# scenarios/VAE-2

Hardware: AMD Instinct MI355X
Metric: training frames/sec on 128x256 8-frame Cityscapes clips, 1/2/4/8 MI355X (higher is better)
Workload: dtype fp32; 1 GPU; VAE2 ELBO step (encz + encoder + 2 decoders fwd/bwd + Adam), HRNet-W18-small-v2, 128x256, 8 clips/GPU x 9 frames (CLIP_LENGTH=3); yaml=vae-2_amd/experiments/vae2_w18_small_v2_128x256.yaml, global_batch=8, frames_per_clip=9, parallelism=dp1, sync_bn=False, launch=hip_graph, mfma_operands=fp32

## Files before the change

### include/vae2_hip.h

```cpp
#ifndef VAE2_HIP_H
#define VAE2_HIP_H

#include <stdint.h>

#ifdef __cplusplus
extern "C" {
#endif

typedef struct vae2_act {
  int64_t n, h, w, c;
  int64_t ps;
} vae2_act;

#define VAE2_ABI_VERSION 15

int vae2_abi_version(void);
const char* vae2_last_error(void);

int vae2_kernel_log(int enable);
int64_t vae2_kernel_log_read(char* buf, int64_t len);


int64_t vae2_conv2d_fwd_stats_rows(const float* x, const vae2_act* xd, const vae2_act* yd,
                                   int k, int stride, int pad);

int vae2_conv2d_set_algo(int algo);
int vae2_conv2d_set_mfma_bf16(int on);
int vae2_conv2d_set_tune(int key, int value);
int vae2_wgrad_defer(int on);
int vae2_wgrad_flush(void* stream);
int vae2_wgrad_flush_stream(void* stream);

typedef struct vae2_conv_job {
  int32_t kind, k, stride, pad;
  const float* x;
  vae2_act xd;
  const float* wp;
  const float* bias;
  float* y;
  vae2_act yd;
  float beta;
  float* stats;
} vae2_conv_job;
int vae2_conv2d_multi(int n, const vae2_conv_job* jobs, void* stream);
int vae2_conv2d_set_grouping(int on);

int64_t vae2_conv2d_packed_size(int64_t cout, int64_t cin, int k, int mode);
int vae2_conv2d_pack_weight(const float* w, int64_t cout, int64_t cin, int k,
                            int mode, float* out, void* stream);
int vae2_conv2d_pack_weight_ld(const float* w, int64_t cout, int64_t cin, int k,
                               int mode, int64_t ld, float* out, void* stream);

typedef struct vae2_pack_job {
  const float* w;
  float* out;
  int32_t cout, cin, k, mode;
  int32_t ld;
  int32_t pad_;
} vae2_pack_job;
int vae2_conv2d_pack_weights(const vae2_pack_job* jobs, int64_t njobs, void* stream);

int vae2_conv2d_fwd(const float* x, const vae2_act* xd, const float* wp,
                    const float* bias, float* y, const vae2_act* yd, int k,
                    int stride, int pad, float beta, float* stats,
                    void* stream);

int vae2_conv2d_bnin_ok(const float* x, const vae2_act* xd, const vae2_act* yd, int k,
                        int stride, int pad);
int vae2_conv2d_fwd_bnin(const float* x, const vae2_act* xd, const float* bn_save, int relu,
                         const float* wp, const float* bias, float* y, const vae2_act* yd,
                         int k, int stride, int pad, float beta, float* stats, void* stream);
int vae2_conv2d_bwd_weight_bnin(const float* x, const vae2_act* xd, const float* bn_save,
                                int relu, const float* dy, const vae2_act* dyd, float* dw,
                                float* dbias, int k, int stride, int pad, int accumulate,
                                float* ws, int64_t ws_size, void* stream);
int64_t vae2_conv2d_bwd_data_bnpart_rows(const float* dy, const vae2_act* dyd,
                                         const vae2_act* dxd, int k, int stride, int pad);
int vae2_conv2d_bwd_data_bnpart(const float* dy, const vae2_act* dyd, const float* wp,
                                float* dx, const vae2_act* dxd, int k, int stride, int pad,
                                const float* bn_x, const vae2_act* bn_xd, const float* bn_save,
                                int relu, float* partials, void* stream);

int vae2_conv2d_fwd_kernel_name(const vae2_act* xd, const vae2_act* yd, int k, int stride,
                                int pad, char* buf, int64_t len);

int vae2_conv2d_bwd_data(const float* dy, const vae2_act* dyd, const float* wp,
                         float* dx, const vae2_act* dxd, int k, int stride,
                         int pad, float beta, void* stream);

int64_t vae2_conv2d_bwd_weight_ws_size(const vae2_act* xd, const vae2_act* dyd,
                                       int k);

int vae2_conv2d_bwd_weight(const float* x, const vae2_act* xd, const float* dy,
                           const vae2_act* dyd, float* dw, float* dbias, int k,
                           int stride, int pad, int accumulate, float* ws,
                           int64_t ws_size, void* stream);

int vae2_conv2d_bwd_weight_ld(const float* x, const vae2_act* xd, const float* dy,
                              const vae2_act* dyd, float* dw, int64_t dw_ld, float* dbias,
                              int k, int stride, int pad, int accumulate, float* ws,
                              int64_t ws_size, void* stream);


int64_t vae2_bn_partial_rows(const vae2_act* xd);

int vae2_bn_stats(const float* x, const vae2_act* xd, float* partials,
                  void* stream);

int vae2_bn_partials_reduce(const float* partials, int64_t rows, int64_t c,
                            double* sums, int accumulate, void* stream);

int vae2_bn_finalize(const double* sums, double count, const float* gamma,
                     const float* beta, float* running_mean, float* running_var,
                     int64_t* num_batches_tracked, float momentum, float eps,
                     int64_t c, float* save, void* stream);

int vae2_bn_reduce_finalize(const float* partials, int64_t rows, int64_t c,
                            double* sums, double count, const float* gamma,
                            const float* beta, float* running_mean, float* running_var,
                            int64_t* num_batches_tracked, float momentum, float eps,
                            float* save, void* stream);

int vae2_bn_reduce_finalize_shifted(const float* partials, int64_t rows, int64_t c,
                                    double* sums, double count, const float* mean_shift,
                                    const float* gamma, const float* beta,
                                    float* running_mean, float* running_var,
                                    int64_t* num_batches_tracked, float momentum, float eps,
                                    float* save, void* stream);
int vae2_bn_finalize_shifted(const double* sums, double count, const float* mean_shift,
                             const float* gamma, const float* beta, float* running_mean,
                             float* running_var, int64_t* num_batches_tracked, float momentum,
                             float eps, int64_t c, float* save, void* stream);

int vae2_bn_bwd_reduce_param_grads(const float* partials, int64_t rows, int64_t c,
                                   double* sums, float* dgamma, float* dbeta,
                                   void* stream);

int vae2_bn_eval_coeffs(const float* gamma, const float* beta,
                        const float* running_mean, const float* running_var,
                        float eps, int64_t c, float* save, void* stream);

int vae2_bn_apply(const float* x, const vae2_act* xd, const float* save,
                  const float* res, const vae2_act* rd, float* y,
                  const vae2_act* yd, int relu, void* stream);

int vae2_bn_relu_bwd_reduce(const float* dy, const vae2_act* dyd,
                            const float* y, const vae2_act* yd, const float* x,
                            const vae2_act* xd, const float* save, int relu,
                            float* partials, void* stream);

int vae2_bn_bwd_param_grads(const double* sums, int64_t c, float* dgamma,
                            float* dbeta, void* stream);

int vae2_bn_relu_bwd_apply(const float* dy, const vae2_act* dyd, const float* y,
                           const vae2_act* yd, const float* x,
                           const vae2_act* xd, const float* save,
                           const float* gamma, const double* sums, double count,
                           int relu, float* dx, const vae2_act* dxd,
                           float* dres, const vae2_act* dresd, void* stream);

typedef struct vae2_bn_layer {
  const float* x; vae2_act xd;
  const float* a; vae2_act ad;
  float* o; vae2_act od;
  const float* dy; vae2_act dyd;
  float* dres; vae2_act dresd;
  const float* save;
  const float* gamma;
  float* partials;
  const double* sums;
  const double* countp;
  double count;
  int relu;
  int dres_acc;
  const float* rx; vae2_act rxd;
  const float* rsave;
  const float* rgamma;
  float* rpartials;
  const double* rsums;
  float* rdx; vae2_act rdxd;
  unsigned char* mask;
} vae2_bn_layer;
int vae2_bn_multi_apply(int n, const vae2_bn_layer* layers, void* stream);
int vae2_bn_multi_bwd_reduce(int n, const vae2_bn_layer* layers, void* stream);
int vae2_bn_multi_bwd_apply(int n, const vae2_bn_layer* layers, void* stream);

typedef struct vae2_bn_fin {
  const float* partials; int64_t rows; int64_t c;
  double* sums;
  const double* countp;
  double count;
  const float* gamma; const float* beta;
  float* running_mean; float* running_var; int64_t* num_batches_tracked;
  float momentum, eps;
  float* save;
  float* dgamma; float* dbeta;
} vae2_bn_fin;
int vae2_bn_multi_reduce(int n, const vae2_bn_fin* fins, int mode, void* stream);
int vae2_bn_multi_finalize(int n, const vae2_bn_fin* fins, void* stream);

int64_t vae2_conv1x1_upsum_stats_rows(const vae2_act* yd);
int vae2_conv1x1_upsum_fwd(const float* x, const vae2_act* xd, const float* wp,
                           const float* bias, int nup, const float* const* ups,
                           const vae2_act* upds, float* y, const vae2_act* yd, float* stats,
                           void* stream);

int vae2_head_out_fwd(const float* y, const vae2_act* yd, const float* save, const float* w2,
                      const float* b2, int cout2, float* out, const vae2_act* outd,
                      void* stream);
int64_t vae2_head_out_bwd_ws_size(const vae2_act* yd, int cout2);
int vae2_head_out_bwd_reduce(const float* y, const vae2_act* yd, const float* save,
                             const float* w2, int cout2, const float* dout,
                             const vae2_act* doutd, double* sums, float* dgamma, float* dbeta,
                             float* dw2, float* db2, float* ws, int64_t ws_size, void* stream);
int vae2_head_out_bwd_apply(const float* y, const vae2_act* yd, const float* save,
                            const float* gamma, const float* w2, int cout2, const float* dout,
                            const vae2_act* doutd, const double* sums, double count, float* dy,
                            const vae2_act* dyd, float* dbias, float* ws, int64_t ws_size,
                            void* stream);


int vae2_upsample_bilinear_fwd(const float* x, const vae2_act* xd, float* y,
                               const vae2_act* yd, float beta, void* stream);
int vae2_upsample_bilinear_bwd(const float* dy, const vae2_act* dyd, float* dx,
                               const vae2_act* dxd, float beta, void* stream);

int vae2_fuse_sum_relu(int n, const float* const* xs, const vae2_act* xds,
                       float* y, const vae2_act* yd, void* stream);
int vae2_fuse_sum_relu_bn(int n, const float* const* xs, const vae2_act* xds,
                          const float* const* saves, float* y, const vae2_act* yd,
                          void* stream);

int vae2_heads_set_algo(int algo);

int64_t vae2_upsample_bilinear_bwd_multi_ws_size(const vae2_act* dyd, int n,
                                                 const vae2_act* dxds);
int vae2_upsample_bilinear_bwd_multi(const float* dy, const vae2_act* dyd, int n,
                                     float* const* dxs, const vae2_act* dxds, float* ws,
                                     int64_t ws_size, void* stream);

int64_t vae2_upsample_bilinear_bwd_pow2_ws_size(const vae2_act* dyd, int n,
                                                const vae2_act* dxds);
int vae2_upsample_bilinear_bwd_pow2(const float* dy, const vae2_act* dyd, int n,
                                    float* const* dxs, const vae2_act* dxds,
                                    const float* betas, float* ws, int64_t ws_size,
                                    void* stream);

int vae2_relu_bwd(const float* dy, const vae2_act* dyd, const float* y,
                  const vae2_act* yd, float* g, const vae2_act* gd,
                  void* stream);

int vae2_relu_bwd_dual(const float* dy, const vae2_act* dyd, const float* y,
                       const vae2_act* yd, float* g, const vae2_act* gd, float* g2,
                       const vae2_act* g2d, float beta2, void* stream);

int vae2_copy_act(const float* x, const vae2_act* xd, float* y,
                  const vae2_act* yd, float beta, void* stream);

int vae2_codemap_tile_fwd(const float* v, int64_t vs, float* y,
                          const vae2_act* yd, void* stream);
int64_t vae2_spatial_ws_size(const vae2_act* xd);
int vae2_codemap_tile_bwd(const float* dy, const vae2_act* dyd, float* dv,
                          int64_t vs, int accumulate, float* ws, int64_t ws_size,
                          void* stream);

int vae2_nchw_to_nhwc(const float* x, float* y, const vae2_act* yd,
                      float beta, void* stream);
int vae2_nhwc_to_nchw(const float* x, const vae2_act* xd, float* y,
                      float beta, void* stream);

int vae2_global_avgpool_fwd(const float* x, const vae2_act* xd, float* y,
                            const vae2_act* yd, float* ws, int64_t ws_size,
                            void* stream);
int vae2_global_avgpool_bwd(const float* dy, const vae2_act* dyd, float* dx,
                            const vae2_act* dxd, float beta, void* stream);
int vae2_weighted_avgpool_fwd(const float* x, const vae2_act* xd, const float* wr,
                              const float* wc, float scale, float* y, const vae2_act* yd,
                              float* ws, int64_t ws_size, void* stream);
int vae2_weighted_avgpool_bwd(const float* dy, const vae2_act* dyd, const float* wr,
                              const float* wc, float scale, float* dx, const vae2_act* dxd,
                              float beta, void* stream);


int64_t vae2_reduce_ws_size(int64_t n);
int vae2_l1_fwd(const float* p, const vae2_act* pd, const float* t,
                const vae2_act* td, float scale, float* ws, float* out,
                void* stream);
int vae2_l1_bwd(const float* p, const vae2_act* pd, const float* t,
                const vae2_act* td, const float* gout, float scale, float* dp,
                const vae2_act* dpd, float beta, void* stream);

int vae2_lsgan_fwd(const float* x, const vae2_act* xd, float target, float scale, float* ws,
                   float* out, void* stream);
int vae2_lsgan_bwd(const float* x, const vae2_act* xd, float target, const float* gout,
                   float scale, float* dx, const vae2_act* dxd, float beta, void* stream);

int64_t vae2_ssim_loss_ws_size(const vae2_act* pd);
int vae2_ssim_loss_fwd(const float* p, const vae2_act* pd, const float* t, const vae2_act* td,
                       const float* a, const float* b, float c1, float c2, float scale,
                       double* ws, float* out, void* stream);
int vae2_ssim_loss_bwd(const float* p, const vae2_act* pd, const float* t, const vae2_act* td,
                       const float* a, const float* b, float c1, float c2, const float* gout,
                       float scale, float* dp, const vae2_act* dpd, float beta, void* stream);

int vae2_reparam_kl_fwd(const float* muvar, const vae2_act* md,
                        const float* eps, const vae2_act* ed, float* z,
                        const vae2_act* zd, int prior, float scale,
                        float* kl_out, int accumulate, float* ws, void* stream);
int vae2_reparam_kl_bwd(const float* muvar, const vae2_act* md,
                        const float* eps, const vae2_act* ed, const float* dz,
                        const vae2_act* dzd, const float* gkl, float scale,
                        float* dmuvar, const vae2_act* dmd, void* stream);

int vae2_weighted_sum(int n, const float* const* terms, const float* lambdas,
                      float* total, void* stream);

int vae2_nonfinite_check(const float* x, int64_t n, int32_t* flag,
                         void* stream);


int vae2_clip_normalize_u8(const uint8_t* frames, int64_t n, int64_t nframes, int64_t h,
                           int64_t w, const float* lut, int nseg, float* const* outs,
                           void* stream);


int vae2_to_image(const float* x, float* y, int64_t n, int64_t c, int64_t h, int64_t w,
                  const double* mean3, const double* std3, void* stream);
int64_t vae2_metrics_ws_size(int64_t planes, int64_t h, int64_t w);
int vae2_absdiff_sqdiff_sum(const float* a, const float* b, int64_t n, double* ws,
                            double* out, void* stream);
int vae2_ssim(const float* x, const float* y, int64_t planes, int64_t h, int64_t w,
              const float* win, int win_size, float c1, float c2, double* ws, double* out,
              void* stream);
int vae2_avgpool2x2(const float* x, float* y, int64_t planes, int64_t h, int64_t w,
                    void* stream);


int vae2_adam_step(float* p, const float* g, float* m, float* v, int64_t n,
                   float lr, float beta1, float beta2, float eps,
                   float weight_decay, int64_t step, void* stream);

int vae2_adam_coeffs(double* state, float beta1, float beta2, float* coeffs,
                     void* stream);
int vae2_adam_step_dev(float* p, const float* g, float* m, float* v, int64_t n,
                       const float* coeffs, float beta1, float beta2, float eps,
                       float weight_decay, void* stream);

int vae2_sgd_step(float* p, const float* g, float* buf, int64_t n, float lr, float momentum,
                  float dampening, float weight_decay, int nesterov, int first_step,
                  void* stream);

int vae2_sgd_coeffs(double* state, float momentum, float dampening, int nesterov,
                    float* coeffs, void* stream);
int vae2_sgd_step_dev(float* p, const float* g, float* buf, int64_t n, const float* coeffs,
                      float momentum, float weight_decay, int nesterov, void* stream);

int64_t vae2_grad_norm_ws_size(int64_t n);
int vae2_grad_sumsq(const float* g, int64_t n, double* partials, void* stream);
int vae2_clip_coeffs(const double* partials, int64_t count, float max_norm, float* clip,
                     void* stream);
int vae2_sgd_step_dev_clip(float* p, const float* g, float* buf, int64_t n, const float* coeffs,
                           const float* clip, float momentum, float weight_decay, int nesterov,
                           void* stream);
int vae2_adam_step_dev_clip(float* p, const float* g, float* m, float* v, int64_t n,
                            const float* coeffs, const float* clip, float beta1, float beta2,
                            float eps, float weight_decay, void* stream);
int vae2_scale_dev(float* x, int64_t n, const float* clip, void* stream);

int vae2_ema_coeffs(double* state, float decay, float* coeffs, void* stream);
int vae2_ema_update_dev(float* ema, const float* p, int64_t n, const float* coeffs,
                        void* stream);
int vae2_ema_update(float* ema, const float* p, int64_t n, float decay, int first,
                    void* stream);

int vae2_scale(float* dst, const float* src, int64_t n, float scale,
               void* stream);


typedef struct vae2_syncbn_comm vae2_syncbn_comm;
int64_t vae2_syncbn_comm_bytes(int world, int64_t max_elems);
int vae2_syncbn_comm_init(int rank, int world, int64_t max_elems, void* handle_out,
                          vae2_syncbn_comm** out);
int vae2_syncbn_comm_connect(vae2_syncbn_comm* comm, const void* handles);
int vae2_syncbn_allreduce(vae2_syncbn_comm* comm, double* buf, int64_t n, void* stream);
int vae2_syncbn_comm_error(vae2_syncbn_comm* comm, int64_t* host_out);
int vae2_syncbn_comm_set_timeout(vae2_syncbn_comm* comm, double seconds);
int vae2_syncbn_comm_destroy(vae2_syncbn_comm* comm);

#ifdef __cplusplus
}
#endif

#endif
```

### vae-2_amd/csrc/conv.h

```cpp
#pragma once

#include "common.h"

namespace vae2 {

static inline int round_up(int a, int b) { return (a + b - 1) / b * b; }

struct IGemm {
  const float* a;
  int a_ps, a_c, a_c4, a_h, a_w;
  int g_n, g_h, g_w;
  int a_step;
  int nth, ntw;
  int dh0, dhs, dw0, dws;
  int kh0, khs, kw0, kws, ksz;
  const float* w;
  uint32_t a_bytes, w_bytes;
  int n;
  const float* bias;
  float* y;
  int y_ps, y_h, y_w, y_step, y_offh, y_offw;
  float beta;
  float* stats;
  int vec_out;
  FastDiv hw_div, w_div;
  int ktab;
  const float* bx;
  int bx_ps, brelu;
  const float* bsave;
  uint32_t bx_bytes;
  struct Cls {
    int g_h, g_w, nth, ntw, dh0, dw0, kh0, kw0, y_offh, y_offw;
    FastDiv hw_div, w_div;
  } cls[4];
};

struct Tile {
  int tm, tn, nblk;
  int ks = 1;
  int nr = 0;
};

struct IGemmPlan {
  Tile t;
  int64_t M;
  int max_taps;
  dim3 grid;
};
IGemmPlan igemm_plan(const IGemm& p, int ncls);

extern int g_wide_tiles, g_ksplit, g_bf16, g_conv_algo, g_dconv_nr, g_gemm1, g_vec_out,
    g_dconv_nr_wide, g_igemm_minblk, g_wgrad_cols, g_dconv_nw8, g_wgrad_nw8, g_gemm1_tn,
    g_gemm1_tm, g_igemm_nr, g_wgrad_narrow, g_igemm_tab, g_dconv_n16, g_dconv_split72,
    g_dconv_ksp, g_wgrad_wgs;
extern int g_dconv_stream, g_dconv_stream_wpc, g_dconv_stream_bl, g_dconv_stream_spb;
extern int g_wgrad_narrow_tps;
extern int g_bn_v2, g_bn_blocks, g_bn_apply_res;
extern int g_fuse_quad;

inline uint32_t packed_bytes(int64_t cout, int64_t cin, int k, int mode) {
  return (uint32_t)(vae2_conv2d_packed_size(cout, cin, k, mode) * 4);
}

inline bool vec_ok(const float* a, int ps) {
  return ((uintptr_t)a % 16 == 0) && (ps % 4 == 0);
}

inline bool conv_shapes_ok(const vae2_act* xd, const vae2_act* yd, int k, int stride, int pad) {
  if (!act_ok(xd) || !act_ok(yd)) return false;
  if (xd->n != yd->n) return false;
  if (k < 1 || stride < 1 || pad < 0) return false;
  int64_t oh = (xd->h + 2 * pad - k) / stride + 1;
  int64_t ow = (xd->w + 2 * pad - k) / stride + 1;
  return oh == yd->h && ow == yd->w;
}

inline bool fits32(const vae2_act* d) {
  return d->n * d->h * d->w * d->ps < (int64_t(1) << 29);
}

inline uint32_t act_bytes(const vae2_act* d) {
  int64_t tail = (d->ps % 4 == 0) ? ((d->c + 3) / 4 * 4) : d->c;
  int64_t last = ((d->n * d->h * d->w) - 1) * d->ps + tail;
  return (uint32_t)(last * 4);
}

struct G1Tile {
  int tm = 2, tn, nblk, grid_x;
  size_t lds;
};
int launch_igemm(IGemm& p, int role, hipStream_t s, const char* fn, int ncls = 1);
int launch_gemm1(const float* a, const vae2_act* ad, const float* wp, uint32_t w_bytes,
                 const float* bias, float* y, const vae2_act* yd, float beta, float* stats,
                 const G1Tile& t, hipStream_t s, const char* fn, const float* bx = nullptr,
                 int bx_ps = 0, int brelu = 0, const float* bsave = nullptr,
                 uint32_t bx_bytes = 0);

struct DTile {
  int tm, tn, nblk, cs4, tiles_h, tiles_w;
  int nr = 0;
  int nw = 4;
  int ks = 1;
};

struct BnSide {
  const float* isave = nullptr;
  int irelu = 0;
  const float* bx = nullptr;
  int bx_ps = 0, brelu = 0;
  const float* bsave = nullptr;
  uint32_t bx_bytes = 0;
};

int launch_dconv(const float* a, const vae2_act* ad, const float* wp, uint32_t w_bytes,
                 const float* bias, float* y, const vae2_act* yd, float beta,
                 float* stats, bool flip, hipStream_t s, const char* fn,
                 const BnSide& bn = BnSide{});

Tile pick_tile(int64_t M, int N, bool wide = false);
bool gemm1_pick(const vae2_act* ad, const vae2_act* yd, int k, int stride, int pad,
                const float* a, G1Tile* out);
DTile pick_dtile(const vae2_act* ad, const vae2_act* yd, bool remainder = true);
bool stream_use(const vae2_act* ad, const vae2_act* yd);
bool dconv_use(const vae2_act* ad, const vae2_act* yd, int k, int stride, int pad,
               const float* a);
int64_t dconv_rows(const vae2_act* ad, const vae2_act* yd);
bool wgrad3_shape_ok(const vae2_act* xd, const vae2_act* dyd, int k, int stride, int pad);

}
```

### vae-2_amd/csrc/conv_wgrad.hip

```cpp
#include <algorithm>
#include <mutex>
#include <vector>

#include "conv.h"

namespace vae2 {

struct WGrad {
  const float* x;
  int x_ps, cin, cin4, x_h, x_w;
  const float* dy;
  int dy_ps, cout, o_n, o_h, o_w;
  int k, stride, pad;
  int P, px_split;
  uint32_t x_bytes, dy_bytes;
  float* part;
  FastDiv ohw_div, ow_div, cin4_div;
};

template <int TM, int TN, bool BF = false, bool V4 = false>
__global__ __launch_bounds__(256, 2) void wgrad_kernel(WGrad p) {
  extern __shared__ __attribute__((aligned(16))) float wred[];
  const int lane = threadIdx.x & 63, wave = threadIdx.x >> 6;
  const int g = lane >> 4, r = lane & 15;
  const int ncol4 = p.k * p.k * p.cin4;
  const int co0 = blockIdx.y * 16 * TM;
  const int col0 = blockIdx.x * 16 * TN;
  const int pbeg = blockIdx.z * p.px_split;
  const int pend = min(pbeg + p.px_split, p.P);
  const __amdgpu_buffer_rsrc_t xr = make_rsrc(p.x, p.x_bytes);
  const __amdgpu_buffer_rsrc_t dr = make_rsrc(p.dy, p.dy_bytes);

  int aco[TM];
#pragma unroll
  for (int i = 0; i < TM; ++i) {
    const int co = co0 + i * 16 + r;
    aco[i] = co < p.cout ? co : -1;
  }
  int bkh[TN], bkw[TN], boff[TN];
  bool bok[TN];
  const int kq = r & 3;
#pragma unroll
  for (int j = 0; j < TN; ++j) {
    const int col = col0 + j * 16 + (V4 ? 4 * (r >> 2) : r);
    const int t = (int)p.cin4_div.div((uint32_t)col);
    const int ci = col - t * p.cin4;
    bkh[j] = t / p.k;
    bkw[j] = t - bkh[j] * p.k;
    bok[j] = col < ncol4 && ci < p.cin;
    boff[j] = (bkh[j] * p.x_w + bkw[j]) * p.x_ps + ci;
  }
  f4 acc[TM][TN];
#pragma unroll
  for (int i = 0; i < TM; ++i)
#pragma unroll
    for (int j = 0; j < TN; ++j) acc[i][j] = f4{0.f, 0.f, 0.f, 0.f};

  const int ohw = p.o_h * p.o_w;
  auto load = [&](int pc, f4* fa, f4* fb) {
    if constexpr (V4) {
      const int pix = pc + 4 * g + kq;
      const bool pv = pix < pend;
      const int pp = pv ? pix : pbeg;
      const int n = (int)p.ohw_div.div((uint32_t)pp);
      const int rem = pp - n * ohw;
      const int oh = (int)p.ow_div.div((uint32_t)rem);
      const int ow = rem - oh * p.o_w;
      const uint32_t drow = (uint32_t)(pp * p.dy_ps);
#pragma unroll
      for (int i = 0; i < TM; ++i) {
        const int co = co0 + i * 16 + 4 * (r >> 2);
        fa[i] = load4(dr, (pv && co < p.cout) ? (drow + co) * 4u : kOOB);
      }
      const int ih0 = oh * p.stride - p.pad, iw0 = ow * p.stride - p.pad;
      const int xc = ((n * p.x_h + ih0) * p.x_w + iw0) * p.x_ps;
#pragma unroll
      for (int j = 0; j < TN; ++j) {
        const int ih = ih0 + bkh[j], iw = iw0 + bkw[j];
        const bool ok = pv && bok[j] && (unsigned)ih < (unsigned)p.x_h &&
                        (unsigned)iw < (unsigned)p.x_w;
        fb[j] = load4(xr, ok ? (uint32_t)(xc + boff[j]) * 4u : kOOB);
      }
      return;
    }
#pragma unroll
    for (int s = 0; s < 4; ++s) {
      const int pix = pc + 4 * g + s;
      const bool pv = pix < pend;
      const int pp = pv ? pix : pbeg;
      const int n = (int)p.ohw_div.div((uint32_t)pp);
      const int rem = pp - n * ohw;
      const int oh = (int)p.ow_div.div((uint32_t)rem);
      const int ow = rem - oh * p.o_w;
      const uint32_t drow = (uint32_t)(pp * p.dy_ps);
#pragma unroll
      for (int i = 0; i < TM; ++i)
        fa[i][s] = load1(dr, (pv && aco[i] >= 0) ? (drow + aco[i]) * 4u : kOOB);
      const int ih0 = oh * p.stride - p.pad, iw0 = ow * p.stride - p.pad;
      const int xc = ((n * p.x_h + ih0) * p.x_w + iw0) * p.x_ps;
#pragma unroll
      for (int j = 0; j < TN; ++j) {
        const int ih = ih0 + bkh[j], iw = iw0 + bkw[j];
        const bool ok = pv && bok[j] && (unsigned)ih < (unsigned)p.x_h &&
                        (unsigned)iw < (unsigned)p.x_w;
        fb[j][s] = load1(xr, ok ? (uint32_t)(xc + boff[j]) * 4u : kOOB);
      }
    }
  };
  auto quads = [&](f4* fa, f4* fb) {
    if constexpr (V4) {
#pragma unroll
      for (int i = 0; i < TM; ++i) quad_transpose(fa[i], kq);
#pragma unroll
      for (int j = 0; j < TN; ++j) quad_transpose(fb[j], kq);
    }
  };
  auto mma = [&](f4* fa, f4* fb) {
    quads(fa, fb);
#pragma unroll
    for (int s = 0; s < 4; ++s)
#pragma unroll
      for (int i = 0; i < TM; ++i)
#pragma unroll
        for (int j = 0; j < TN; ++j)
          acc[i][j] = __builtin_amdgcn_mfma_f32_16x16x4f32(fa[i][s], fb[j][s], acc[i][j], 0, 0, 0);
  };
  {
    f4 fa0[TM], fb0[TN], fa1[TM], fb1[TN];
    int pc = pbeg + 16 * wave;
    if (!BF) {
      if (pc < pend) load(pc, fa0, fb0);
      for (; pc < pend; pc += 128) {
        load(pc + 64, fa1, fb1);
        mma(fa0, fb0);
        load(pc + 128, fa0, fb0);
        mma(fa1, fb1);
      }
    } else if (pc < pend) {
      load(pc, fa0, fb0);
      load(pc + 64, fa1, fb1);
      for (; pc < pend; pc += 128) {
        bf16x8 A[TM], B[TN];
        quads(fa0, fb0);
        quads(fa1, fb1);
#pragma unroll
        for (int i = 0; i < TM; ++i) A[i] = pack_bf16(fa0[i], fa1[i]);
#pragma unroll
        for (int j = 0; j < TN; ++j) B[j] = pack_bf16(fb0[j], fb1[j]);
        load(pc + 128, fa0, fb0);
        load(pc + 192, fa1, fb1);
#pragma unroll
        for (int i = 0; i < TM; ++i)
#pragma unroll
          for (int j = 0; j < TN; ++j)
            acc[i][j] = __builtin_amdgcn_mfma_f32_16x16x32_bf16(A[i], B[j], acc[i][j], 0, 0, 0);
      }
    }
  }

  constexpr int NV = TM * TN * 4;
  if (wave > 0) {
#pragma unroll
    for (int i = 0; i < TM; ++i)
#pragma unroll
      for (int j = 0; j < TN; ++j)
#pragma unroll
        for (int e = 0; e < 4; ++e)
          wred[((wave - 1) * NV + (i * TN + j) * 4 + e) * 64 + lane] = acc[i][j][e];
  }
  __syncthreads();
  if (wave != 0) return;
#pragma unroll
  for (int w = 0; w < 3; ++w)
#pragma unroll
    for (int i = 0; i < TM; ++i)
#pragma unroll
      for (int j = 0; j < TN; ++j)
#pragma unroll
        for (int e = 0; e < 4; ++e)
          acc[i][j][e] += wred[(w * NV + (i * TN + j) * 4 + e) * 64 + lane];

  float* out = p.part + (int64_t)blockIdx.z * p.cout * ncol4;
#pragma unroll
  for (int i = 0; i < TM; ++i)
#pragma unroll
    for (int e = 0; e < 4; ++e) {
      const int co = co0 + i * 16 + g * 4 + e;
      if (co >= p.cout) continue;
#pragma unroll
      for (int j = 0; j < TN; ++j) {
        const int col = col0 + j * 16 + r;
        if (col < ncol4) out[(int64_t)co * ncol4 + col] = acc[i][j][e];
      }
    }
}

struct WGrad3 {
  const float* x;
  int x_ps, cin, cin4, h, w;
  const float* dy;
  int dy_ps, cout;
  int tiles_h, tiles_w, ntiles, tiles_per_split;
  int csw, n_ci_slabs;
  uint32_t x_bytes, dy_bytes;
  float* part;
  const float* isave;
  int irelu;
};

template <int TM, int TN, int BH, bool PF, int KS, bool BF = false, int NR = 0, int NW = 4>
__global__ __launch_bounds__(64 * NW) void wgrad3_kernel(WGrad3 p) {
  constexpr int NT = 64 * NW;
  constexpr int HALO = KS / 2, TAPS = KS * KS;
  constexpr int LH = BH + KS - 1, LW = 32 + KS - 1, NPX = BH * 32, LPX = LH * LW;
  constexpr int QMAX = KS == 1 ? 16 : 9;
  constexpr int DYS = NPX + 4;
  constexpr int NRQ = (NR + 3) / 4;
  constexpr int NQ = 4 * TM + NRQ;
  static_assert(NR == 0 || (!BF && NR <= 4), "remainder shape");
  extern __shared__ __attribute__((aligned(16))) float sm[];
  float* dyt = sm;
  float* xt = sm + NQ * 4 * DYS;
  const int lane = threadIdx.x & 63, wave = threadIdx.x >> 6;
  const int g = lane >> 4, r = lane & 15;
  const int cis = blockIdx.y % p.n_ci_slabs, cos = blockIdx.y / p.n_ci_slabs;
  const int co0 = cos * (16 * TM + NR), c0 = cis * p.csw;
  const int csw_real = p.cin4 - c0 < p.csw ? p.cin4 - c0 : p.csw;
  const __amdgpu_buffer_rsrc_t xr = make_rsrc(p.x, p.x_bytes);
  const __amdgpu_buffer_rsrc_t dr = make_rsrc(p.dy, p.dy_bytes);

  int bbase[TN];
#pragma unroll
  for (int j = 0; j < TN; ++j) {
    const int n = (wave * TN + j) * 16 + r;
    const int t = n / p.csw;
    const int cl = n - t * p.csw;
    const bool ok = t < TAPS && cl < csw_real;
    bbase[j] = ok ? cl * LPX + (t / KS) * LW + (t % KS) : p.csw * LPX;
  }
  for (int i = threadIdx.x; i < LPX; i += NT) xt[p.csw * LPX + i] = 0.f;
  __shared__ float ibn[2][QMAX * 4];
  if (p.isave && threadIdx.x < QMAX * 4) {
    const int ch = c0 + (int)threadIdx.x < p.cin ? c0 + (int)threadIdx.x : p.cin - 1;
    ibn[0][threadIdx.x] = p.isave[2 * p.cin + ch];
    ibn[1][threadIdx.x] = p.isave[3 * p.cin + ch];
  }
  auto ibn_apply = [&](f4& v, int q) {
#pragma unroll
    for (int k = 0; k < 4; ++k) {
      const float t = __builtin_fmaf(v[k], ibn[0][4 * q + k], ibn[1][4 * q + k]);
      v[k] = (p.irelu && t < 0.f) ? 0.f : t;
    }
  };

  f4 acc[TM][TN];
#pragma unroll
  for (int i = 0; i < TM; ++i)
#pragma unroll
    for (int j = 0; j < TN; ++j) acc[i][j] = f4{0.f, 0.f, 0.f, 0.f};
  float racc[TN][NR > 0 ? NR : 1];
#pragma unroll
  for (int j = 0; j < TN; ++j)
#pragma unroll
    for (int q = 0; q < NR; ++q) racc[j][q] = 0.f;

  const int per_img = p.tiles_h * p.tiles_w;
  const int tb = blockIdx.x * p.tiles_per_split;
  const int te = tb + p.tiles_per_split < p.ntiles ? tb + p.tiles_per_split : p.ntiles;
  constexpr int NDY = NPX * NQ;
  constexpr int NI = (NDY + NT - 1) / NT;
  constexpr int NX = (LPX * QMAX + NT - 1) / NT;
  const int xtotal = LPX * (csw_real >> 2);
  f4 pdy[NI], pxx[NX];
  static_assert(NX <= 32, "x item mask");
  uint32_t xok = 0;
  auto fetch = [&](int tile) {
    const int img = tile / per_img;
    const int trem = tile - img * per_img;
    const int th = trem / p.tiles_w;
    const int oh0 = th * BH, ow0 = (trem - th * p.tiles_w) * 32;
    const int ibase = img * p.h;
#pragma unroll
    for (int u = 0; u < NI; ++u) {
      const int i = threadIdx.x + u * NT;
      const int q = i / NPX, px = i - q * NPX;
      const int oh = oh0 + px / 32, ow = ow0 + (px & 31);
      const int co = co0 + 4 * q;
      const bool ok = i < NDY && oh < p.h && ow < p.w && co < p.cout;
      pdy[u] = load4(dr, ok ? (uint32_t)(((ibase + oh) * p.w + ow) * p.dy_ps + co) * 4u : kOOB);
    }
#pragma unroll
    for (int u = 0; u < NX; ++u) {
      const int i = threadIdx.x + u * NT;
      const int q = i / LPX, hp = i - q * LPX;
      const int lr = hp / LW, lc = hp - lr * LW;
      const int ih = oh0 - HALO + lr, iw = ow0 - HALO + lc;
      const int c = c0 + 4 * q;
      const bool ok = i < xtotal && (unsigned)ih < (unsigned)p.h && (unsigned)iw < (unsigned)p.w;
      pxx[u] = load4(xr, ok ? (uint32_t)(((ibase + ih) * p.w + iw) * p.x_ps + c) * 4u : kOOB);
      xok = u == 0 ? (uint32_t)ok : (xok | ((uint32_t)ok << u));
    }
  };
  auto store = [&]() {
#pragma unroll
    for (int u = 0; u < NI; ++u) {
      const int i = threadIdx.x + u * NT;
      if (NDY % NT != 0 && i >= NDY) break;
      const int q = i / NPX, px = i - q * NPX;
      const int co = co0 + 4 * q;
#pragma unroll
      for (int k = 0; k < 4; ++k) dyt[(4 * q + k) * DYS + px] = co + k < p.cout ? pdy[u][k] : 0.f;
    }
#pragma unroll
    for (int u = 0; u < NX; ++u) {
      const int i = threadIdx.x + u * NT;
      if (i < xtotal) {
        const int q = i / LPX, hp = i - q * LPX;
        const int c = c0 + 4 * q;
        if (p.isave && ((xok >> u) & 1u)) ibn_apply(pxx[u], q);
#pragma unroll
        for (int k = 0; k < 4; ++k) xt[(4 * q + k) * LPX + hp] = c + k < p.cin ? pxx[u][k] : 0.f;
      }
    }
  };
  if (PF && tb < te) fetch(tb);
  for (int tile = tb; tile < te; ++tile) {
    __syncthreads();
    if (PF) {
      store();
    } else {
      const int img = tile / per_img;
      const int trem = tile - img * per_img;
      const int th = trem / p.tiles_w;
      const int oh0 = th * BH, ow0 = (trem - th * p.tiles_w) * 32;
      const int ibase = img * p.h;
      {
        f4 v[NI];
#pragma unroll
        for (int u = 0; u < NI; ++u) {
          const int i = threadIdx.x + u * NT;
          const int q = i / NPX, px = i - q * NPX;
          const int oh = oh0 + px / 32, ow = ow0 + (px & 31);
          const int co = co0 + 4 * q;
          const bool ok = i < NDY && oh < p.h && ow < p.w && co < p.cout;
          v[u] = load4(dr, ok ? (uint32_t)(((ibase + oh) * p.w + ow) * p.dy_ps + co) * 4u : kOOB);
        }
#pragma unroll
        for (int u = 0; u < NI; ++u) {
          const int i = threadIdx.x + u * NT;
          if (NDY % NT != 0 && i >= NDY) break;
          const int q = i / NPX, px = i - q * NPX;
          const int co = co0 + 4 * q;
#pragma unroll
          for (int k = 0; k < 4; ++k)
            dyt[(4 * q + k) * DYS + px] = co + k < p.cout ? v[u][k] : 0.f;
        }
      }
      for (int i0 = threadIdx.x; i0 < xtotal; i0 += 4 * NT) {
        f4 v[4];
        bool okv[4];
#pragma unroll
        for (int u = 0; u < 4; ++u) {
          const int i = i0 + u * NT;
          const int q = i / LPX, hp = i - q * LPX;
          const int lr = hp / LW, lc = hp - lr * LW;
          const int ih = oh0 - HALO + lr, iw = ow0 - HALO + lc;
          const int c = c0 + 4 * q;
          const bool ok =
              i < xtotal && (unsigned)ih < (unsigned)p.h && (unsigned)iw < (unsigned)p.w;
          okv[u] = ok;
          v[u] = load4(xr, ok ? (uint32_t)(((ibase + ih) * p.w + iw) * p.x_ps + c) * 4u : kOOB);
        }
#pragma unroll
        for (int u = 0; u < 4; ++u) {
          const int i = i0 + u * NT;
          if (i >= xtotal) break;
          const int q = i / LPX, hp = i - q * LPX;
          const int c = c0 + 4 * q;
          if (p.isave && okv[u]) ibn_apply(v[u], q);
#pragma unroll
          for (int k = 0; k < 4; ++k) xt[(4 * q + k) * LPX + hp] = c + k < p.cin ? v[u][k] : 0.f;
        }
      }
    }
    __syncthreads();
    if (PF && tile + 1 < te) fetch(tile + 1);
    auto frag = [&](int ch, f4* fa, f4* fb) {
      const int px0 = ch * 16 + 4 * g;
      const int poff = (px0 >> 5) * LW + (px0 & 31);
#pragma unroll
      for (int i = 0; i < TM; ++i)
        fa[i] = *reinterpret_cast<const f4*>(&dyt[(i * 16 + r) * DYS + px0]);
#pragma unroll
      for (int j = 0; j < TN; ++j) {
        const float* b = &xt[bbase[j] + poff];
        if (KS == 1) fb[j] = *reinterpret_cast<const f4*>(b);
        else fb[j] = f4{b[0], b[1], b[2], b[3]};
      }
    };
    if (!BF) {
#pragma unroll 2
      for (int ch = 0; ch < NPX / 16; ++ch) {
        f4 fa[TM], fb[TN];
        frag(ch, fa, fb);
#pragma unroll
        for (int s2 = 0; s2 < 4; ++s2)
#pragma unroll
          for (int i = 0; i < TM; ++i)
#pragma unroll
            for (int j = 0; j < TN; ++j)
              acc[i][j] = __builtin_amdgcn_mfma_f32_16x16x4f32(fa[i][s2], fb[j][s2], acc[i][j], 0, 0, 0);
        if constexpr (NR > 0) {
          const int px0 = ch * 16 + 4 * g;
#pragma unroll
          for (int q = 0; q < NR; ++q) {
            const f4 d = *reinterpret_cast<const f4*>(&dyt[(16 * TM + q) * DYS + px0]);
#pragma unroll
            for (int j = 0; j < TN; ++j) {
              racc[j][q] = __builtin_fmaf(d[0], fb[j][0], racc[j][q]);
              racc[j][q] = __builtin_fmaf(d[1], fb[j][1], racc[j][q]);
              racc[j][q] = __builtin_fmaf(d[2], fb[j][2], racc[j][q]);
              racc[j][q] = __builtin_fmaf(d[3], fb[j][3], racc[j][q]);
            }
          }
        }
      }
    } else {
#pragma unroll 2
      for (int ch = 0; ch < NPX / 16; ch += 2) {
        f4 fa0[TM], fb0[TN], fa1[TM], fb1[TN];
        frag(ch, fa0, fb0);
        frag(ch + 1, fa1, fb1);
#pragma unroll
        for (int i = 0; i < TM; ++i)
#pragma unroll
          for (int j = 0; j < TN; ++j)
            acc[i][j] = __builtin_amdgcn_mfma_f32_16x16x32_bf16(
                pack_bf16(fa0[i], fa1[i]), pack_bf16(fb0[j], fb1[j]), acc[i][j], 0, 0, 0);
      }
    }
  }

  const int ncol4 = TAPS * p.cin4;
  float* out = p.part + (int64_t)blockIdx.x * p.cout * ncol4;
#pragma unroll
  for (int j = 0; j < TN; ++j) {
    const int n = (wave * TN + j) * 16 + r;
    const int t = n / p.csw;
    const int cl = n - t * p.csw;
    if (t >= TAPS || cl >= csw_real) continue;
    const int col = t * p.cin4 + c0 + cl;
#pragma unroll
    for (int i = 0; i < TM; ++i)
#pragma unroll
      for (int e = 0; e < 4; ++e) {
        const int co = co0 + i * 16 + g * 4 + e;
        if (co < p.cout) out[(int64_t)co * ncol4 + col] = acc[i][j][e];
      }
  }
  if constexpr (NR > 0) {
#pragma unroll
    for (int j = 0; j < TN; ++j) {
      const int n = (wave * TN + j) * 16 + r;
      const int t = n / p.csw;
      const int cl = n - t * p.csw;
#pragma unroll
      for (int q = 0; q < NR; ++q) {
        float v = racc[j][q];
        v += __shfl_xor(v, 16, 64);
        v += __shfl_xor(v, 32, 64);
        if (g == 0 && t < TAPS && cl < csw_real)
          out[(int64_t)(co0 + 16 * TM + q) * ncol4 + t * p.cin4 + c0 + cl] = v;
      }
    }
  }
}

__global__ __launch_bounds__(256) void wgrad_reduce_kernel(const float* __restrict__ part,
                                                           int splits, int cout, int cin,
                                                           int cin4, int k,
                                                           float* __restrict__ dw, int64_t ld,
                                                           int accumulate) {
  __shared__ float red[8][32];
  const int kk = k * k;
  const int ncol4 = kk * cin4;
  const int total = cout * ncol4;
  const int cl = threadIdx.x & 31, sg = threadIdx.x >> 5;
  const int idx = blockIdx.x * 32 + cl;
  float s = 0.f;
  if (idx < total) {
    const float* src = part + idx;
    const int64_t stride = (int64_t)total;
#pragma unroll 8
    for (int sp = sg; sp < splits; sp += 8) s += src[sp * stride];
  }
  red[sg][cl] = s;
  __syncthreads();
  if (sg != 0 || idx >= total) return;
  s = red[0][cl];
#pragma unroll
  for (int j = 1; j < 8; ++j) s += red[j][cl];
  const int co = idx / ncol4;
  const int col = idx - co * ncol4;
  const int t = col / cin4;
  const int ci = col - t * cin4;
  if (ci >= cin) return;
  const int64_t o = (int64_t)co * ld + ci * kk + t;
  dw[o] = accumulate ? dw[o] + s : s;
}

struct WRJob {
  const float* part;
  float* dw;
  int64_t ld;
  int splits, cout, cin, cin4, k, accumulate, blk0;
};
constexpr int kWrMaxJobs = 32;
struct WRMulti {
  WRJob j[kWrMaxJobs];
  int n;
};

__global__ __launch_bounds__(256) void wgrad_reduce_multi_kernel(WRMulti m) {
  int i = 0;
  while (i + 1 < m.n && (int)blockIdx.x >= m.j[i + 1].blk0) ++i;
  const WRJob& J = m.j[i];
  __shared__ float red[8][32];
  const int kk = J.k * J.k;
  const int ncol4 = kk * J.cin4;
  const int total = J.cout * ncol4;
  const int cl = threadIdx.x & 31, sg = threadIdx.x >> 5;
  const int idx = ((int)blockIdx.x - J.blk0) * 32 + cl;
  float s = 0.f;
  if (idx < total) {
    const float* src = J.part + idx;
    const int64_t stride = (int64_t)total;
#pragma unroll 8
    for (int sp = sg; sp < J.splits; sp += 8) s += src[sp * stride];
  }
  red[sg][cl] = s;
  __syncthreads();
  if (sg != 0 || idx >= total) return;
  s = red[0][cl];
#pragma unroll
  for (int q = 1; q < 8; ++q) s += red[q][cl];
  const int co = idx / ncol4;
  const int col = idx - co * ncol4;
  const int t = col / J.cin4;
  const int ci = col - t * J.cin4;
  if (ci >= J.cin) return;
  const int64_t o = (int64_t)co * J.ld + ci * kk + t;
  J.dw[o] = J.accumulate ? J.dw[o] + s : s;
}


struct WRQueued {
  WRJob job;
  hipStream_t stream;
};
static thread_local bool g_wr_defer = false;
static std::vector<WRQueued> g_wr_queue;
static std::mutex g_wr_mu;

struct WTile {
  int tm, tn, gx, gy, splits, px_split;
};

static WTile pick_wtile(int64_t P, int cout, int ncol4) {
  WTile t;
  int mt = (cout + 15) / 16;
  t.tm = mt <= 4 ? mt : 4;
  t.gy = (int)ceil_div(cout, 16 * t.tm);
  int ct = (ncol4 + 15) / 16;
  if (g_wgrad_cols && t.tm == 4 && ct == 4) {
    t.tm = 2;
    t.gy = (int)ceil_div(cout, 32);
  }
  const int tn_max = t.tm == 4 ? 3 : 4;
  t.tn = ct <= tn_max ? ct : tn_max;
  t.gx = (int)ceil_div(ncol4, 16 * t.tn);
  int64_t tiles = (int64_t)t.gx * t.gy;
  int64_t want = ceil_div(g_wgrad_wgs, tiles);
  int64_t maxs = ceil_div(P, 256);
  int64_t s = want < maxs ? want : maxs;
  if (s < 1) s = 1;
  t.px_split = (int)(ceil_div(ceil_div(P, s), 64) * 64);
  t.splits = (int)ceil_div(P, t.px_split);
  return t;
}

template <int TM, bool V4>
static void launch_wgrad_tn_v(const WGrad& p, int tn, dim3 grid, hipStream_t s) {
  const size_t lds = (size_t)3 * TM * 4 * 4 * 64 * sizeof(float) / 4 * tn;
  switch (tn) {
#define CASE(T) \
  case T: \
    if (g_bf16) VAE2_LAUNCH((wgrad_kernel<TM, T, true, V4>), grid, dim3(256), lds, s, p); \
    else VAE2_LAUNCH((wgrad_kernel<TM, T, false, V4>), grid, dim3(256), lds, s, p); \
    break;
    CASE(1) CASE(2) CASE(3)
    default: CASE(4)
#undef CASE
  }
}

template <int TM>
static void launch_wgrad_tn(const WGrad& p, int tn, dim3 grid, hipStream_t s, bool v4) {
  if (v4) launch_wgrad_tn_v<TM, true>(p, tn, grid, s);
  else launch_wgrad_tn_v<TM, false>(p, tn, grid, s);
}


struct W3Tile {
  int ks, tm, tn, bh, csw, n_ci_slabs, n_co_slabs, tiles_h, tiles_w, ntiles, tps, splits;
  bool pf;
  int nr = 0;
  int nw = 4;
};

int wgrad3_blocks_per_cu(const W3Tile& t, size_t lds);
static size_t wgrad3_lds(const W3Tile& t);

bool wgrad3_shape_ok(const vae2_act* xd, const vae2_act* dyd, int k, int stride, int pad) {
  return k == 3 && pad == 1 && stride == 1 && xd->h == dyd->h &&
         xd->w == dyd->w && xd->ps % 4 == 0 && dyd->ps % 4 == 0 && dyd->w >= 16;
}

static W3Tile pick_w3tile(const vae2_act* xd, const vae2_act* dyd, int k) {
  W3Tile t;
  t.ks = k;
  const int cin4 = round_up((int)xd->c, 4);
  const int maxc = k == 1 ? 64 : 36;
  int nsl = (cin4 + maxc - 1) / maxc;
  t.csw = round_up((int)ceil_div(cin4, nsl), 4);
  t.n_ci_slabs = (int)ceil_div(cin4, t.csw);
  const int nt = (k * k * t.csw + 15) / 16;
  t.tn = (nt + 3) / 4;
  const int mt = (int)((dyd->c + 15) / 16);
  t.n_co_slabs = (mt + 3) / 4;
  t.tm = (mt + t.n_co_slabs - 1) / t.n_co_slabs;
  if (k == 3 && g_dconv_nr && !g_bf16 && (dyd->c == 18 || dyd->c == 36 || dyd->c == 72)) {
    t.tm = dyd->c == 18 ? 1 : 2;
    t.nr = dyd->c == 18 ? 2 : 4;
    t.n_co_slabs = (int)(dyd->c / (16 * t.tm + t.nr));
  }
  if (g_wgrad_nw8 && t.nr && !g_bf16) {
    const int tn2 = (nt + 7) / 8;
    if ((t.tm == 1 && tn2 == 2) || (t.tm == 2 && tn2 == 3)) {
      t.tn = tn2;
      t.nw = 8;
    }
  }
  t.bh = (t.tm <= 2 && t.csw <= 24 && k == 3) ? 8 : 4;
  t.tiles_h = (int)ceil_div(dyd->h, t.bh);
  t.tiles_w = (int)ceil_div(dyd->w, 32);
  t.ntiles = (int)(dyd->n * t.tiles_h * t.tiles_w);
  const int gy = t.n_ci_slabs * t.n_co_slabs;
  int64_t want = ceil_div(1024, gy);
  const int64_t slab = (int64_t)dyd->c * k * k * cin4 * 4;
  const int64_t cap = 48ll << 20;
  if (want * slab > cap) want = cap / slab > 0 ? cap / slab : 1;
  if (want > t.ntiles) want = t.ntiles;
  t.tps = (int)ceil_div(t.ntiles, want);
  t.pf = (int64_t)t.ntiles * gy >= 1024;
  if (t.pf) {
    const int64_t resident = 256 * (int64_t)wgrad3_blocks_per_cu(t, wgrad3_lds(t));
    int64_t w2 = resident / gy > 0 ? resident / gy : 1;
    if (w2 * slab > cap) w2 = cap / slab > 0 ? cap / slab : 1;
    t.tps = (int)ceil_div(t.ntiles, w2);
    if (t.tps < 2) t.tps = 2;
  }
  if (t.tps < 2) t.tps = 2;
  t.splits = (int)ceil_div(t.ntiles, t.tps);
  return t;
}

static size_t wgrad3_lds(const W3Tile& t) {
  const int npx = t.bh * 32, lpx = (t.bh + t.ks - 1) * (32 + t.ks - 1);
  const int rows = 16 * t.tm + 4 * ((t.nr + 3) / 4);
  return ((size_t)rows * (npx + 4) + (size_t)(t.csw + 1) * lpx) * sizeof(float);
}

struct W3Probe {
  bool on = false;
  const void* fn = nullptr;
  unsigned threads = 0;
};
static thread_local W3Probe g_w3probe;
#define W3_LAUNCH(K, GRID, BLOCK, SHM, S, ...)                         \
  do {                                                                \
    if (g_w3probe.on) {                                               \
      g_w3probe.fn = reinterpret_cast<const void*>(K);                \
      g_w3probe.threads = dim3(BLOCK).x;                              \
    } else {                                                          \
      VAE2_LAUNCH(K, GRID, BLOCK, SHM, S, __VA_ARGS__);               \
    }                                                                 \
  } while (0)

template <int TM, int BH, bool PF>
static void wgrad3_launch_tn(const WGrad3& p, int tn, int ks, dim3 grid, size_t shm,
                             hipStream_t s, int nr = 0, int nw = 4) {
  if constexpr (TM == 1 || TM == 2) {
    if (nr && nw == 8) {
      constexpr int R = TM == 1 ? 2 : 4, T8 = TM == 1 ? 2 : 3;
      W3_LAUNCH((wgrad3_kernel<TM, T8, BH, PF, 3, false, R, 8>), grid, dim3(512), shm, s, p);
      return;
    }
    if (nr) {
      constexpr int R = TM == 1 ? 2 : 4;
      switch (tn) {
#define CASE(T) \
  case T: W3_LAUNCH((wgrad3_kernel<TM, T, BH, PF, 3, false, R>), grid, dim3(256), shm, s, p); break;
        CASE(1) CASE(2) CASE(3) CASE(4) CASE(5) CASE(6)
#undef CASE
      }
      return;
    }
  }
  if (ks == 1) {
    if (g_bf16) W3_LAUNCH((wgrad3_kernel<TM, 1, BH, PF, 1, true>), grid, dim3(256), shm, s, p);
    else W3_LAUNCH((wgrad3_kernel<TM, 1, BH, PF, 1>), grid, dim3(256), shm, s, p);
    return;
  }
  switch (tn) {
#define CASE(T) \
  case T:                                                                         \
    if (g_bf16) W3_LAUNCH((wgrad3_kernel<TM, T, BH, PF, 3, true>), grid, dim3(256), shm, s, p); \
    else W3_LAUNCH((wgrad3_kernel<TM, T, BH, PF, 3>), grid, dim3(256), shm, s, p);   \
    break;
    CASE(1) CASE(2) CASE(3) CASE(4) CASE(5) CASE(6)
#undef CASE
  }
}

template <int BH, bool PF>
static void wgrad3_launch_tm(const WGrad3& p, const W3Tile& t, dim3 grid, size_t shm,
                             hipStream_t s) {
  switch (t.tm) {
    case 1: wgrad3_launch_tn<1, BH, PF>(p, t.tn, t.ks, grid, shm, s, t.nr, t.nw); break;
    case 2: wgrad3_launch_tn<2, BH, PF>(p, t.tn, t.ks, grid, shm, s, t.nr, t.nw); break;
    case 3: wgrad3_launch_tn<3, BH, PF>(p, t.tn, t.ks, grid, shm, s); break;
    default: wgrad3_launch_tn<4, BH, PF>(p, t.tn, t.ks, grid, shm, s); break;
  }
}

template <int BH>
static void wgrad3_launch(const WGrad3& p, const W3Tile& t, dim3 grid, size_t shm,
                          hipStream_t s) {
  if (t.pf) wgrad3_launch_tm<BH, true>(p, t, grid, shm, s);
  else wgrad3_launch_tm<BH, false>(p, t, grid, shm, s);
}

int wgrad3_blocks_per_cu(const W3Tile& t, size_t lds) {
  struct Key {
    int tm, tn, bh, ks, nr, nw, pf, bf;
    size_t lds;
    int n;
  };
  static Key cache[32];
  static int ncache = 0;
  const int bf = g_bf16;
  for (int i = 0; i < ncache; ++i) {
    const Key& k = cache[i];
    if (k.tm == t.tm && k.tn == t.tn && k.bh == t.bh && k.ks == t.ks && k.nr == t.nr &&
        k.nw == t.nw && k.pf == (int)t.pf && k.bf == bf && k.lds == lds)
      return k.n;
  }
  WGrad3 p{};
  g_w3probe = W3Probe{};
  g_w3probe.on = true;
  if (t.bh == 8) wgrad3_launch<8>(p, t, dim3(1), lds, nullptr);
  else wgrad3_launch<4>(p, t, dim3(1), lds, nullptr);
  g_w3probe.on = false;
  int n = 0;
  if (!g_w3probe.fn || hipOccupancyMaxActiveBlocksPerMultiprocessor(
                           &n, g_w3probe.fn, (int)g_w3probe.threads, lds) != hipSuccess ||
      n < 1) {
    (void)hipGetLastError();
    n = 1;
  }
  if (ncache < 32) cache[ncache++] = Key{t.tm, t.tn, t.bh, t.ks, t.nr, t.nw, (int)t.pf, bf, lds, n};
  return n;
}

}

using namespace vae2;

extern "C" {

int vae2_wgrad_defer(int on) {
  const int prev = g_wr_defer ? 1 : 0;
  g_wr_defer = on != 0;
  return prev;
}

static int wgrad_flush_impl(void* stream, bool own_only) {
  const char* fn = "vae2_wgrad_flush";
  hipStream_t want = as_stream(stream);
  std::vector<WRQueued> q;
  {
    std::lock_guard<std::mutex> lk(g_wr_mu);
    if (own_only) {
      std::vector<WRQueued> keep;
      for (const WRQueued& j : g_wr_queue) (j.stream == want ? q : keep).push_back(j);
      g_wr_queue.swap(keep);
    } else {
      q.swap(g_wr_queue);
    }
  }
  size_t i = 0;
  while (i < q.size()) {
    WRMulti m{};
    hipStream_t st = want;
    int blocks = 0;
    while (i < q.size() && m.n < kWrMaxJobs) {
      WRJob j = q[i].job;
      const float* lo = j.dw;
      const float* hi = j.dw + (int64_t)(j.cout - 1) * j.ld + (int64_t)j.cin * j.k * j.k;
      bool clash = false;
      for (int u = 0; u < m.n; ++u) {
        const float* lo2 = m.j[u].dw;
        const float* hi2 = m.j[u].dw + (int64_t)(m.j[u].cout - 1) * m.j[u].ld +
                           (int64_t)m.j[u].cin * m.j[u].k * m.j[u].k;
        if (lo < hi2 && lo2 < hi) clash = true;
      }
      if (clash) break;
      j.blk0 = blocks;
      blocks += (int)ceil_div((int64_t)j.cout * j.k * j.k * j.cin4, 32);
      m.j[m.n++] = j;
      ++i;
    }
    VAE2_LAUNCH(wgrad_reduce_multi_kernel, dim3((unsigned)blocks), dim3(256), 0, st, m);
    const int rc = check_launch(fn);
    if (rc) return rc;
  }
  return 0;
}

int vae2_wgrad_flush(void* stream) { return wgrad_flush_impl(stream, false); }

int vae2_wgrad_flush_stream(void* stream) { return wgrad_flush_impl(stream, true); }


struct WgradWs {
  int64_t part, total;
};
static WgradWs wgrad_ws(const vae2_act* xd, const vae2_act* dyd, int k) {
  const int ncol4 = k * k * round_up((int)xd->c, 4);
  const WTile t = pick_wtile(act_pixels(dyd), (int)dyd->c, ncol4);
  int64_t splits = t.splits;
  if ((k == 3 || k == 1) && xd->h == dyd->h && xd->w == dyd->w) {
    splits = std::max<int64_t>(splits, pick_w3tile(xd, dyd, k).splits);
    splits = std::max<int64_t>(splits, wgrad3n_splits(xd, dyd));
  }
  const int64_t part = splits * dyd->c * ncol4;
  return WgradWs{part, part + 2 * vae2_bn_partial_rows(dyd) * dyd->c + 4};
}

int64_t vae2_conv2d_bwd_weight_ws_size(const vae2_act* xd, const vae2_act* dyd, int k) {
  if (!act_ok(xd) || !act_ok(dyd)) return 0;
  return wgrad_ws(xd, dyd, k).total;
}

static int bwd_weight_impl(const float* x, const vae2_act* xd, const float* dy,
                           const vae2_act* dyd, float* dw, int64_t dw_ld, float* dbias,
                           int k, int stride, int pad, int accumulate, float* ws,
                           int64_t ws_size, void* stream, const float* isave, int irelu,
                           const char* fn) {
  VAE2_REQUIRE(xd && dw_ld >= xd->c * k * k, fn, "bad dW row stride");
  VAE2_REQUIRE(x && dy && dw && ws, fn, "null pointer");
  VAE2_REQUIRE(conv_shapes_ok(xd, dyd, k, stride, pad), fn, "inconsistent conv shapes");
  VAE2_REQUIRE(fits32(xd) && fits32(dyd), fn, "tensor too large for 32-bit indexing");
  const WgradWs wsl = wgrad_ws(xd, dyd, k);
  VAE2_REQUIRE(ws_size >= wsl.total, fn, "workspace too small");
  hipStream_t s = as_stream(stream);
  const int cin4 = round_up((int)xd->c, 4);
  const int ncol4 = k * k * cin4;
  int splits = 0;
  const bool direct = g_conv_algo != 1 && wgrad3_shape_ok(xd, dyd, k, stride, pad) &&
                      vec_ok(x, (int)xd->ps) && vec_ok(dy, (int)dyd->ps);
  VAE2_REQUIRE(direct || !isave, fn,
               "input BatchNorm needs the direct 3x3 weight-gradient kernel (vae2_conv2d_bnin_ok)");
  if (direct && k == 3) {
    splits = wgrad3n_launch(x, xd, dy, dyd, ws, isave, irelu, act_bytes(xd), act_bytes(dyd), s);
    if (splits < 0) return check_launch(fn);
  }
  if (direct && !splits) {
    W3Tile t3 = pick_w3tile(xd, dyd, k);
    WGrad3 q{};
    q.x = x; q.x_ps = (int)xd->ps; q.cin = (int)xd->c; q.cin4 = cin4;
    q.h = (int)xd->h; q.w = (int)xd->w;
    q.dy = dy; q.dy_ps = (int)dyd->ps; q.cout = (int)dyd->c;
    q.tiles_h = t3.tiles_h; q.tiles_w = t3.tiles_w; q.ntiles = t3.ntiles;
    q.tiles_per_split = t3.tps;
    q.csw = t3.csw; q.n_ci_slabs = t3.n_ci_slabs;
    q.x_bytes = act_bytes(xd); q.dy_bytes = act_bytes(dyd);
    q.part = ws;
    q.isave = isave;
    q.irelu = irelu ? 1 : 0;
    dim3 grid((unsigned)t3.splits, (unsigned)(t3.n_ci_slabs * t3.n_co_slabs));
    const size_t shm = wgrad3_lds(t3);
    if (t3.bh == 8) wgrad3_launch<8>(q, t3, grid, shm, s);
    else wgrad3_launch<4>(q, t3, grid, shm, s);
    int rc = check_launch(fn);
    if (rc) return rc;
    splits = t3.splits;
  }
  WTile t = pick_wtile(act_pixels(dyd), (int)dyd->c, ncol4);
  if (splits) goto reduce;
  {
  WGrad p{};
  p.x = x; p.x_ps = (int)xd->ps; p.cin = (int)xd->c; p.cin4 = cin4;
  p.x_h = (int)xd->h; p.x_w = (int)xd->w;
  p.dy = dy; p.dy_ps = (int)dyd->ps; p.cout = (int)dyd->c;
  p.o_n = (int)dyd->n; p.o_h = (int)dyd->h; p.o_w = (int)dyd->w;
  p.k = k; p.stride = stride; p.pad = pad;
  p.P = (int)act_pixels(dyd);
  p.px_split = t.px_split;
  p.part = ws;
  p.x_bytes = act_bytes(xd);
  p.dy_bytes = act_bytes(dyd);
  p.ohw_div = FastDiv((uint32_t)(dyd->h * dyd->w));
  p.ow_div = FastDiv((uint32_t)dyd->w);
  p.cin4_div = FastDiv((uint32_t)cin4);
  dim3 grid(t.gx, t.gy, (unsigned)t.splits);
  const bool v4 = g_vec_out && vec_ok(x, (int)xd->ps) && vec_ok(dy, (int)dyd->ps);
  switch (t.tm) {
    case 1: launch_wgrad_tn<1>(p, t.tn, grid, s, v4); break;
    case 2: launch_wgrad_tn<2>(p, t.tn, grid, s, v4); break;
    case 3: launch_wgrad_tn<3>(p, t.tn, grid, s, v4); break;
    default: launch_wgrad_tn<4>(p, t.tn, grid, s, v4); break;
  }
  int rc = check_launch(fn);
  if (rc) return rc;
  splits = t.splits;
  }
reduce:
  int64_t slab = dyd->c * (int64_t)ncol4;
  int rc = 0;
  if (g_wr_defer) {
    WRJob j{ws, dw, dw_ld, splits, (int)dyd->c, (int)xd->c, cin4, k, accumulate, 0};
    std::lock_guard<std::mutex> lk(g_wr_mu);
    g_wr_queue.push_back(WRQueued{j, s});
  } else {
    VAE2_LAUNCH(wgrad_reduce_kernel, dim3((unsigned)ceil_div(slab, 32)), dim3(256), 0, s,
                (const float*)ws, splits, (int)dyd->c, (int)xd->c, cin4, k, dw, dw_ld,
                accumulate);
    rc = check_launch(fn);
    if (rc) return rc;
  }
  if (dbias) {
    float* bp = ws + wsl.part;
    rc = vae2_bn_stats(dy, dyd, bp, stream);
    if (rc) return rc;
    rc = bias_grad_from_partials(bp, vae2_bn_partial_rows(dyd), dyd->c, dbias, accumulate,
                                 stream);
    if (rc) return rc;
  }
  return 0;
}

int vae2_conv2d_bwd_weight_ld(const float* x, const vae2_act* xd, const float* dy,
                              const vae2_act* dyd, float* dw, int64_t dw_ld, float* dbias,
                              int k, int stride, int pad, int accumulate, float* ws,
                              int64_t ws_size, void* stream) {
  return bwd_weight_impl(x, xd, dy, dyd, dw, dw_ld, dbias, k, stride, pad, accumulate, ws,
                         ws_size, stream, nullptr, 0, "vae2_conv2d_bwd_weight");
}

int vae2_conv2d_bwd_weight_bnin(const float* x, const vae2_act* xd, const float* bn_save,
                                int relu, const float* dy, const vae2_act* dyd, float* dw,
                                float* dbias, int k, int stride, int pad, int accumulate,
                                float* ws, int64_t ws_size, void* stream) {
  const char* fn = "vae2_conv2d_bwd_weight_bnin";
  if (!xd || !bn_save) return fail(fn, "null pointer");
  return bwd_weight_impl(x, xd, dy, dyd, dw, xd->c * k * k, dbias, k, stride, pad, accumulate,
                         ws, ws_size, stream, bn_save, relu, fn);
}

int vae2_conv2d_bwd_weight(const float* x, const vae2_act* xd, const float* dy,
                           const vae2_act* dyd, float* dw, float* dbias, int k,
                           int stride, int pad, int accumulate, float* ws,
                           int64_t ws_size, void* stream) {
  if (!xd) return fail("vae2_conv2d_bwd_weight", "null descriptor");
  return vae2_conv2d_bwd_weight_ld(x, xd, dy, dyd, dw, xd->c * k * k, dbias, k, stride, pad,
                                   accumulate, ws, ws_size, stream);
}

}
```

### vae-2_amd/csrc/wgrad_narrow.hip

```cpp
#include "conv.h"

namespace vae2 {

int g_wgrad_narrow_tps = 2;

constexpr int kTH = 4;
constexpr int kTW = 32;
constexpr int kLW = kTW + 2;
constexpr int kNPX = kTH * kTW;

struct WGN {
  const float* x;
  int x_ps, cin, cin4, h, w;
  const float* dy;
  int dy_ps, cout;
  int tiles_h, tiles_w, ntiles, tps;
  int n_ci_slabs;
  FastDiv per_img_div, tiles_w_div;
  uint32_t x_bytes, dy_bytes;
  float* part;
  const float* isave;
  int irelu;
};

template <int CQ, int TM, int NR, int WPIX, bool PF, int NW = 4>
__global__ __launch_bounds__(64 * NW) void wgrad3n_kernel(WGN p) {
  constexpr int CSW = 4 * CQ;
  constexpr int CO = 16 * TM + NR;
  constexpr int COQ = (CO + 3) / 4;
  constexpr int DP = 4 * COQ;
  constexpr int XP = CSW;
  constexpr int LPX = (kTH + 2) * kLW;
  constexpr int RS = kLW * XP + ((CSW - kLW * XP) % 16 + 16) % 16;
  constexpr int G = (3 * CSW + 15) / 16;
  constexpr int WCOL = NW / WPIX;
  constexpr int NT = 64 * NW;
  constexpr int GW = (G + WCOL - 1) / WCOL;
  static_assert(NR <= 4 && (NR == 0 || COQ == 4 * TM + 1), "one remainder quad");
  static_assert(WCOL * WPIX == NW && (WCOL == 1 || WCOL == 2 || WCOL == 4), "waves per tile");
  extern __shared__ __attribute__((aligned(16))) float sm[];
  float* xs = sm;
  float* ds = sm + (kTH + 2) * RS;

  const int lane = threadIdx.x & 63, wave = threadIdx.x >> 6;
  const int g = lane >> 4, r = lane & 15;
  const int wc = wave % WCOL, wp = wave / WCOL;
  const int cis = blockIdx.y % p.n_ci_slabs, cos = blockIdx.y / p.n_ci_slabs;
  const int c0 = cis * CSW, co0 = cos * CO;
  const __amdgpu_buffer_rsrc_t xr = make_rsrc(p.x, p.x_bytes);
  const __amdgpu_buffer_rsrc_t dr = make_rsrc(p.dy, p.dy_bytes);

  int xoff[GW];
  bool colok[GW];
#pragma unroll
  for (int j = 0; j < GW; ++j) {
    const int n = (wc * GW + j) * 16 + r;
    const int nc = n < 3 * CSW ? n : 3 * CSW - 1;
    const int dh = nc / CSW, ci = nc - dh * CSW;
    colok[j] = wc * GW + j < G && n < 3 * CSW && c0 + ci < p.cin;
    xoff[j] = dh * RS + ci;
  }
  __shared__ f4 ibn_tab[2][CQ];
  if (p.isave && threadIdx.x < 2 * CSW) {
    const int k = threadIdx.x % CSW, which = threadIdx.x / CSW;
    const int ch = c0 + k < p.cin ? c0 + k : p.cin - 1;
    reinterpret_cast<float*>(&ibn_tab[which][0])[k] = p.isave[(2 + which) * p.cin + ch];
  }
  auto ibn = [&](f4& v, int q) {
    const f4 sc = ibn_tab[0][q], sh = ibn_tab[1][q];
#pragma unroll
    for (int k = 0; k < 4; ++k) {
      const float t = __builtin_fmaf(v[k], sc[k], sh[k]);
      v[k] = (p.irelu && t < 0.f) ? 0.f : t;
    }
  };

  f4 acc[TM][GW][3];
#pragma unroll
  for (int i = 0; i < TM; ++i)
#pragma unroll
    for (int j = 0; j < GW; ++j)
#pragma unroll
      for (int d = 0; d < 3; ++d) acc[i][j][d] = f4{0.f, 0.f, 0.f, 0.f};
  float racc[GW][3][NR > 0 ? NR : 1];
#pragma unroll
  for (int j = 0; j < GW; ++j)
#pragma unroll
    for (int d = 0; d < 3; ++d)
#pragma unroll
      for (int q = 0; q < NR; ++q) racc[j][d][q] = 0.f;

  const int per_img = p.tiles_h * p.tiles_w;
  const int tb = blockIdx.x * p.tps;
  const int te = tb + p.tps < p.ntiles ? tb + p.tps : p.ntiles;
  constexpr int XPU = NT / CQ, DPU = NT / COQ;
  constexpr int NXI = (LPX + XPU - 1) / XPU, NDI = (kNPX + DPU - 1) / DPU;
  const int xq = threadIdx.x % CQ, xb = threadIdx.x / CQ;
  const int dq = threadIdx.x % COQ, db = threadIdx.x / COQ;
  const bool xact = xb < XPU, dact = db < DPU;
  const int xc = c0 + 4 * xq;
  const bool xcok = xc < p.cin4;
  const bool dcok = co0 + 4 * dq < p.cout;
  f4 px[NXI], pd[NDI];
  uint32_t xin = 0;
  auto fetch = [&](int tile) {
    const int img = (int)p.per_img_div.div((uint32_t)tile);
    const int trem = tile - img * per_img;
    const int th = (int)p.tiles_w_div.div((uint32_t)trem);
    const int oh0 = th * kTH, ow0 = (trem - th * p.tiles_w) * kTW;
    const int ibase = img * p.h;
#pragma unroll
    for (int u = 0; u < NXI; ++u) {
      const int hp = xb + u * XPU;
      const int lr = hp / kLW, lc = hp - lr * kLW;
      const int ih = oh0 - 1 + lr, iw = ow0 - 1 + lc;
      const bool ok = xact && hp < LPX && xcok && (unsigned)ih < (unsigned)p.h &&
                      (unsigned)iw < (unsigned)p.w;
      px[u] = load4(xr, ok ? (uint32_t)(((ibase + ih) * p.w + iw) * p.x_ps + xc) * 4u : kOOB);
      xin = u == 0 ? (uint32_t)ok : (xin | ((uint32_t)ok << u));
    }
#pragma unroll
    for (int u = 0; u < NDI; ++u) {
      const int pp = db + u * DPU;
      const int oh = oh0 + pp / kTW, ow = ow0 + (pp & (kTW - 1));
      const bool ok = dact && pp < kNPX && dcok && oh < p.h && ow < p.w;
      pd[u] = load4(dr, ok ? (uint32_t)(((ibase + oh) * p.w + ow) * p.dy_ps + co0 + 4 * dq) * 4u : kOOB);
    }
  };
  auto store = [&]() {
#pragma unroll
    for (int u = 0; u < NXI; ++u) {
      const int hp = xb + u * XPU;
      if (!xact || hp >= LPX) break;
      f4 v = px[u];
      if (p.isave && ((xin >> u) & 1u)) ibn(v, xq);
#pragma unroll
      for (int k = 0; k < 4; ++k) v[k] = xc + k < p.cin ? v[k] : 0.f;
      const int lr = hp / kLW, lc = hp - lr * kLW;
      *reinterpret_cast<f4*>(&xs[lr * RS + lc * XP + 4 * xq]) = v;
    }
#pragma unroll
    for (int u = 0; u < NDI; ++u) {
      const int pp = db + u * DPU;
      if (!dact || pp >= kNPX) break;
      f4 v = pd[u];
#pragma unroll
      for (int k = 0; k < 4; ++k) v[k] = (co0 + 4 * dq + k < p.cout && 4 * dq + k < CO) ? v[k] : 0.f;
      *reinterpret_cast<f4*>(&ds[pp * DP + 4 * dq]) = v;
    }
  };

  if (PF && tb < te) fetch(tb);
  for (int tile = tb; tile < te; ++tile) {
    __syncthreads();
    if (!PF) fetch(tile);
    store();
    __syncthreads();
    if (PF && tile + 1 < te) fetch(tile + 1);
#pragma unroll 1
    for (int ch = wp; ch < kTH * 2; ch += WPIX) {
      const int orow = ch >> 1, cb = (ch & 1) * 16;
      const int dpx = orow * kTW + cb + 4 * g;
      float a[TM][4];
#pragma unroll
      for (int i = 0; i < TM; ++i)
#pragma unroll
        for (int s = 0; s < 4; ++s) a[i][s] = ds[(dpx + s) * DP + 16 * i + r];
      f4 rq[4];
      if constexpr (NR > 0) {
#pragma unroll
        for (int s = 0; s < 4; ++s) rq[s] = *reinterpret_cast<const f4*>(&ds[(dpx + s) * DP + 16 * TM]);
      }
      const int xb = orow * RS + (cb + 4 * g) * XP;
#pragma unroll
      for (int j = 0; j < GW; ++j) {
        float xv[6];
#pragma unroll
        for (int t = 0; t < 6; ++t) xv[t] = xs[xb + xoff[j] + t * XP];
#pragma unroll
        for (int d = 0; d < 3; ++d) {
#pragma unroll
          for (int s = 0; s < 4; ++s)
#pragma unroll
            for (int i = 0; i < TM; ++i)
              acc[i][j][d] = __builtin_amdgcn_mfma_f32_16x16x4f32(a[i][s], xv[d + s], acc[i][j][d], 0, 0, 0);
          if constexpr (NR > 0) {
#pragma unroll
            for (int q = 0; q < NR; ++q)
#pragma unroll
              for (int s = 0; s < 4; ++s) racc[j][d][q] = __builtin_fmaf(rq[s][q], xv[d + s], racc[j][d][q]);
          }
        }
      }
    }
  }

#pragma unroll
  for (int j = 0; j < GW; ++j)
#pragma unroll
    for (int d = 0; d < 3; ++d)
#pragma unroll
      for (int q = 0; q < NR; ++q) {
        float v = racc[j][d][q];
        v += __shfl_xor(v, 16, 64);
        v += __shfl_xor(v, 32, 64);
        racc[j][d][q] = v;
      }
  const int ncol4 = 9 * p.cin4;
  const uint32_t slab = (uint32_t)(p.cout * ncol4);
  const __amdgpu_buffer_rsrc_t orr = make_rsrc(p.part + (int64_t)blockIdx.x * slab, slab * 4u);
  int colb[GW];
#pragma unroll
  for (int j = 0; j < GW; ++j) {
    const int n = (wc * GW + j) * 16 + r;
    const int dh = n / CSW, ci = n - dh * CSW;
    colb[j] = colok[j] ? dh * 3 * p.cin4 + c0 + ci : -1;
  }
  auto write = [&](int j, int d, int i, int e, float v) {
    const int co = co0 + 16 * i + 4 * g + e;
    const bool ok = colb[j] >= 0 && co < p.cout;
    store1(orr, ok ? (uint32_t)(co * ncol4 + colb[j] + d * p.cin4) * 4u : kOOB, v);
  };
  auto write_r = [&](int j, int d, int q, float v) {
    const int co = co0 + 16 * TM + q;
    const bool ok = g == 0 && colb[j] >= 0 && co < p.cout;
    store1(orr, ok ? (uint32_t)(co * ncol4 + colb[j] + d * p.cin4) * 4u : kOOB, v);
  };
  if constexpr (WPIX == 1) {
#pragma unroll
    for (int j = 0; j < GW; ++j)
#pragma unroll
      for (int d = 0; d < 3; ++d) {
#pragma unroll
        for (int i = 0; i < TM; ++i)
#pragma unroll
          for (int e = 0; e < 4; ++e) write(j, d, i, e, acc[i][j][d][e]);
#pragma unroll
        for (int q = 0; q < NR; ++q) write_r(j, d, q, racc[j][d][q]);
      }
  } else {
    constexpr int NV = TM * GW * 3 * 4 + GW * 3 * NR;
    __syncthreads();
    float* red = sm;
    if (wp > 0) {
      float* o = red + ((wp - 1) * WCOL + wc) * NV * 64 + lane;
      int k = 0;
#pragma unroll
      for (int i = 0; i < TM; ++i)
#pragma unroll
        for (int j = 0; j < GW; ++j)
#pragma unroll
          for (int d = 0; d < 3; ++d)
#pragma unroll
            for (int e = 0; e < 4; ++e) o[64 * k++] = acc[i][j][d][e];
#pragma unroll
      for (int j = 0; j < GW; ++j)
#pragma unroll
        for (int d = 0; d < 3; ++d)
#pragma unroll
          for (int q = 0; q < NR; ++q) o[64 * k++] = racc[j][d][q];
    }
    __syncthreads();
    if (wp == 0) {
#pragma unroll 1
      for (int w = 1; w < WPIX; ++w) {
        const float* o = red + ((w - 1) * WCOL + wc) * NV * 64 + lane;
        int k = 0;
#pragma unroll
        for (int i = 0; i < TM; ++i)
#pragma unroll
          for (int j = 0; j < GW; ++j)
#pragma unroll
            for (int d = 0; d < 3; ++d)
#pragma unroll
              for (int e = 0; e < 4; ++e) acc[i][j][d][e] += o[64 * k++];
#pragma unroll
        for (int j = 0; j < GW; ++j)
#pragma unroll
          for (int d = 0; d < 3; ++d)
#pragma unroll
            for (int q = 0; q < NR; ++q) racc[j][d][q] += o[64 * k++];
      }
#pragma unroll
      for (int j = 0; j < GW; ++j)
#pragma unroll
        for (int d = 0; d < 3; ++d) {
#pragma unroll
          for (int i = 0; i < TM; ++i)
#pragma unroll
            for (int e = 0; e < 4; ++e) write(j, d, i, e, acc[i][j][d][e]);
#pragma unroll
          for (int q = 0; q < NR; ++q) write_r(j, d, q, racc[j][d][q]);
        }
    }
  }
}

namespace {

struct Cfg {
  int cq, tm, nr, wpix, ci_slabs, co_slabs;
  int pf = 0;
  int nw = 4;
};

bool pick(const vae2_act* xd, const vae2_act* dyd, Cfg& c) {
  if (xd->c != dyd->c) return false;
  if (dyd->c == 18) c = Cfg{5, 1, 2, 2, 1, 1};
  else if (dyd->c == 36) c = Cfg{9, 2, 4, 1, 1, 1};
  else if (dyd->c == 72) c = Cfg{9, 2, 4, 1, 2, 2};
  else return false;
  c.pf = g_wgrad_narrow == 2;
  if (g_wgrad_narrow == 3) {
    c.nw = 8;
    c.wpix *= 2;
  }
  return true;
}

size_t lds_bytes(const Cfg& c) {
  const int CO = 16 * c.tm + c.nr, DP = 4 * ((CO + 3) / 4);
  const int csw = 4 * c.cq, rs = kLW * csw + ((csw - kLW * csw) % 16 + 16) % 16;
  const size_t stage = ((size_t)(kTH + 2) * rs + (size_t)kNPX * DP) * sizeof(float);
  const int G = (3 * 4 * c.cq + 15) / 16, wcol = c.nw / c.wpix, gw = (G + wcol - 1) / wcol;
  const size_t nv = (size_t)c.tm * gw * 12 + (size_t)gw * 3 * c.nr;
  const size_t red = c.wpix > 1 ? (size_t)(c.wpix - 1) * wcol * nv * 64 * sizeof(float) : 0;
  return stage > red ? stage : red;
}

const void* kernel_of(const Cfg& c) {
  if (c.nw == 8)
    return c.cq == 5 ? reinterpret_cast<const void*>(wgrad3n_kernel<5, 1, 2, 4, false, 8>)
                     : reinterpret_cast<const void*>(wgrad3n_kernel<9, 2, 4, 2, false, 8>);
  if (c.cq == 5) return c.pf ? reinterpret_cast<const void*>(wgrad3n_kernel<5, 1, 2, 2, true>)
                             : reinterpret_cast<const void*>(wgrad3n_kernel<5, 1, 2, 2, false>);
  return c.pf ? reinterpret_cast<const void*>(wgrad3n_kernel<9, 2, 4, 1, true>)
              : reinterpret_cast<const void*>(wgrad3n_kernel<9, 2, 4, 1, false>);
}

int resident_per_cu(const Cfg& c) {
  static int cache[6] = {0, 0, 0, 0, 0, 0};
  const int k = (c.cq == 5 ? 0 : 1) + (c.nw == 8 ? 4 : 2 * c.pf);
  if (!cache[k]) {
    int n = 0;
    if (hipOccupancyMaxActiveBlocksPerMultiprocessor(&n, kernel_of(c), 64 * c.nw, lds_bytes(c)) !=
            hipSuccess || n < 1) {
      (void)hipGetLastError();
      n = 1;
    }
    cache[k] = n;
  }
  return cache[k];
}

struct Plan {
  Cfg c;
  int tiles_h, tiles_w, ntiles, tps, splits;
};

bool plan(const vae2_act* xd, const vae2_act* dyd, Plan& pl) {
  if (g_bf16 || !g_wgrad_narrow || !pick(xd, dyd, pl.c)) return false;
  pl.tiles_h = (int)ceil_div(dyd->h, kTH);
  pl.tiles_w = (int)ceil_div(dyd->w, kTW);
  pl.ntiles = (int)(dyd->n * pl.tiles_h * pl.tiles_w);
  const int gy = pl.c.ci_slabs * pl.c.co_slabs;
  int64_t want = (int64_t)256 * resident_per_cu(pl.c) / gy;
  if (want < 1) want = 1;
  pl.tps = (int)ceil_div(pl.ntiles, want);
  if (pl.tps < g_wgrad_narrow_tps) pl.tps = g_wgrad_narrow_tps;
  pl.splits = (int)ceil_div(pl.ntiles, pl.tps);
  return true;
}

}

int64_t wgrad3n_splits(const vae2_act* xd, const vae2_act* dyd) {
  Plan pl;
  return plan(xd, dyd, pl) ? pl.splits : 0;
}

int wgrad3n_launch(const float* x, const vae2_act* xd, const float* dy, const vae2_act* dyd,
                   float* part, const float* isave, int irelu, uint32_t x_bytes,
                   uint32_t dy_bytes, hipStream_t s) {
  Plan pl;
  if (!plan(xd, dyd, pl)) return 0;
  WGN p{};
  p.x = x; p.x_ps = (int)xd->ps; p.cin = (int)xd->c; p.cin4 = (int)((xd->c + 3) / 4 * 4);
  p.h = (int)xd->h; p.w = (int)xd->w;
  p.dy = dy; p.dy_ps = (int)dyd->ps; p.cout = (int)dyd->c;
  p.tiles_h = pl.tiles_h; p.tiles_w = pl.tiles_w; p.ntiles = pl.ntiles; p.tps = pl.tps;
  p.n_ci_slabs = pl.c.ci_slabs;
  p.per_img_div = FastDiv((uint32_t)(pl.tiles_h * pl.tiles_w));
  p.tiles_w_div = FastDiv((uint32_t)pl.tiles_w);
  p.x_bytes = x_bytes; p.dy_bytes = dy_bytes;
  p.part = part;
  p.isave = isave; p.irelu = irelu ? 1 : 0;
  dim3 grid((unsigned)pl.splits, (unsigned)(pl.c.ci_slabs * pl.c.co_slabs));
  const size_t shm = lds_bytes(pl.c);
  if (pl.c.cq == 5) {
    if (pl.c.nw == 8) VAE2_LAUNCH((wgrad3n_kernel<5, 1, 2, 4, false, 8>), grid, dim3(512), shm, s, p);
    else if (pl.c.pf) VAE2_LAUNCH((wgrad3n_kernel<5, 1, 2, 2, true>), grid, dim3(256), shm, s, p);
    else VAE2_LAUNCH((wgrad3n_kernel<5, 1, 2, 2, false>), grid, dim3(256), shm, s, p);
  } else {
    if (pl.c.nw == 8) VAE2_LAUNCH((wgrad3n_kernel<9, 2, 4, 2, false, 8>), grid, dim3(512), shm, s, p);
    else if (pl.c.pf) VAE2_LAUNCH((wgrad3n_kernel<9, 2, 4, 1, true>), grid, dim3(256), shm, s, p);
    else VAE2_LAUNCH((wgrad3n_kernel<9, 2, 4, 1, false>), grid, dim3(256), shm, s, p);
  }
  const hipError_t e = hipGetLastError();
  return e == hipSuccess ? pl.splits : -(int)e;
}

}
```

### vae-2_amd/vae2/_lib.py

```python
import ctypes
import os

import torch

_HERE = os.path.dirname(os.path.abspath(__file__))
LIB_PATH = os.environ.get("VAE2_LIB", os.path.join(_HERE, "libvae2_hip.so"))

c_i64 = ctypes.c_int64
c_int = ctypes.c_int
c_f32 = ctypes.c_float
c_f64 = ctypes.c_double
c_vp = ctypes.c_void_p


class Act(ctypes.Structure):

    _fields_ = [("n", c_i64), ("h", c_i64), ("w", c_i64), ("c", c_i64), ("ps", c_i64)]


P_ACT = ctypes.POINTER(Act)


class BnLayer(ctypes.Structure):
    _fields_ = [("x", c_vp), ("xd", Act), ("a", c_vp), ("ad", Act), ("o", c_vp), ("od", Act),
                ("dy", c_vp), ("dyd", Act), ("dres", c_vp), ("dresd", Act),
                ("save", c_vp), ("gamma", c_vp), ("partials", c_vp), ("sums", c_vp),
                ("countp", c_vp), ("count", c_f64), ("relu", c_int), ("dres_acc", c_int),
                ("rx", c_vp), ("rxd", Act), ("rsave", c_vp), ("rgamma", c_vp),
                ("rpartials", c_vp), ("rsums", c_vp), ("rdx", c_vp), ("rdxd", Act),
                ("mask", c_vp)]


class BnFin(ctypes.Structure):
    _fields_ = [("partials", c_vp), ("rows", c_i64), ("c", c_i64), ("sums", c_vp),
                ("countp", c_vp), ("count", c_f64), ("gamma", c_vp), ("beta", c_vp),
                ("running_mean", c_vp), ("running_var", c_vp), ("num_batches_tracked", c_vp),
                ("momentum", c_f32), ("eps", c_f32), ("save", c_vp), ("dgamma", c_vp),
                ("dbeta", c_vp)]

_SIGS = {
    "vae2_abi_version": (c_int, []),
    "vae2_last_error": (ctypes.c_char_p, []),
    "vae2_kernel_log": (c_int, [c_int]),
    "vae2_kernel_log_read": (c_i64, [ctypes.c_char_p, c_i64]),
    "vae2_conv2d_packed_size": (c_i64, [c_i64, c_i64, c_int, c_int]),
    "vae2_conv2d_pack_weight": (c_int, [c_vp, c_i64, c_i64, c_int, c_int, c_vp, c_vp]),
    "vae2_conv2d_pack_weight_ld": (c_int, [c_vp, c_i64, c_i64, c_int, c_int, c_i64, c_vp, c_vp]),
    "vae2_conv2d_pack_weights": (c_int, [c_vp, c_i64, c_vp]),
    "vae2_conv2d_fwd_stats_rows": (c_i64, [c_vp, P_ACT, P_ACT, c_int, c_int, c_int]),
    "vae2_conv2d_set_mfma_bf16": (c_int, [c_int]),
    "vae2_conv2d_set_tune": (c_int, [c_int, c_int]),
    "vae2_wgrad_defer": (c_int, [c_int]),
    "vae2_wgrad_flush": (c_int, [c_vp]),
    "vae2_wgrad_flush_stream": (c_int, [c_vp]),
    "vae2_conv2d_set_algo": (c_int, [c_int]),
    "vae2_conv2d_fwd": (c_int, [c_vp, P_ACT, c_vp, c_vp, c_vp, P_ACT, c_int, c_int, c_int,
                                c_f32, c_vp, c_vp]),
    "vae2_conv2d_fwd_kernel_name": (c_int, [P_ACT, P_ACT, c_int, c_int, c_int, ctypes.c_char_p,
                                            c_i64]),
    "vae2_conv2d_bwd_data": (c_int, [c_vp, P_ACT, c_vp, c_vp, P_ACT, c_int, c_int, c_int,
                                     c_f32, c_vp]),
    "vae2_conv2d_bnin_ok": (c_int, [c_vp, P_ACT, P_ACT, c_int, c_int, c_int]),
    "vae2_conv2d_fwd_bnin": (c_int, [c_vp, P_ACT, c_vp, c_int, c_vp, c_vp, c_vp, P_ACT, c_int,
                                     c_int, c_int, c_f32, c_vp, c_vp]),
    "vae2_conv2d_bwd_weight_bnin": (c_int, [c_vp, P_ACT, c_vp, c_int, c_vp, P_ACT, c_vp, c_vp,
                                            c_int, c_int, c_int, c_int, c_vp, c_i64, c_vp]),
    "vae2_conv2d_bwd_data_bnpart_rows": (c_i64, [c_vp, P_ACT, P_ACT, c_int, c_int, c_int]),
    "vae2_conv2d_bwd_data_bnpart": (c_int, [c_vp, P_ACT, c_vp, c_vp, P_ACT, c_int, c_int, c_int,
                                            c_vp, P_ACT, c_vp, c_int, c_vp, c_vp]),
    "vae2_conv2d_bwd_weight_ws_size": (c_i64, [P_ACT, P_ACT, c_int]),
    "vae2_conv2d_bwd_weight": (c_int, [c_vp, P_ACT, c_vp, P_ACT, c_vp, c_vp, c_int, c_int,
                                       c_int, c_int, c_vp, c_i64, c_vp]),
    "vae2_conv2d_bwd_weight_ld": (c_int, [c_vp, P_ACT, c_vp, P_ACT, c_vp, c_i64, c_vp, c_int,
                                          c_int, c_int, c_int, c_vp, c_i64, c_vp]),
    "vae2_conv1x1_upsum_stats_rows": (c_i64, [P_ACT]),
    "vae2_conv1x1_upsum_fwd": (c_int, [c_vp, P_ACT, c_vp, c_vp, c_int, ctypes.POINTER(c_vp), P_ACT,
                                       c_vp, P_ACT, c_vp, c_vp]),
    "vae2_upsample_bilinear_bwd_multi_ws_size": (c_i64, [P_ACT, c_int, P_ACT]),
    "vae2_upsample_bilinear_bwd_multi": (c_int, [c_vp, P_ACT, c_int, ctypes.POINTER(c_vp), P_ACT,
                                                 c_vp, c_i64, c_vp]),
    "vae2_upsample_bilinear_bwd_pow2_ws_size": (c_i64, [P_ACT, c_int, P_ACT]),
    "vae2_upsample_bilinear_bwd_pow2": (c_int, [c_vp, P_ACT, c_int, ctypes.POINTER(c_vp), P_ACT,
                                                c_vp, c_vp, c_i64, c_vp]),
    "vae2_head_out_fwd":(c_int, [c_vp, P_ACT, c_vp, c_vp, c_vp, c_int, c_vp, P_ACT, c_vp]),
    "vae2_head_out_bwd_ws_size": (c_i64, [P_ACT, c_int]),
    "vae2_head_out_bwd_reduce": (c_int, [c_vp, P_ACT, c_vp, c_vp, c_int, c_vp, P_ACT, c_vp, c_vp,
                                         c_vp, c_vp, c_vp, c_vp, c_i64, c_vp]),
    "vae2_head_out_bwd_apply": (c_int, [c_vp, P_ACT, c_vp, c_vp, c_vp, c_int, c_vp, P_ACT, c_vp,
                                        c_f64, c_vp, P_ACT, c_vp, c_vp, c_i64, c_vp]),
    "vae2_bn_reduce_finalize_shifted": (c_int, [c_vp, c_i64, c_i64, c_vp, c_f64, c_vp, c_vp, c_vp,
                                                c_vp, c_vp, c_vp, c_f32, c_f32, c_vp, c_vp]),
    "vae2_bn_finalize_shifted": (c_int, [c_vp, c_f64, c_vp, c_vp, c_vp, c_vp, c_vp, c_vp,
                                         c_f32, c_f32, c_i64, c_vp, c_vp]),
    "vae2_bn_partial_rows": (c_i64, [P_ACT]),
    "vae2_bn_stats": (c_int, [c_vp, P_ACT, c_vp, c_vp]),
    "vae2_bn_partials_reduce": (c_int, [c_vp, c_i64, c_i64, c_vp, c_int, c_vp]),
    "vae2_bn_finalize": (c_int, [c_vp, c_f64, c_vp, c_vp, c_vp, c_vp, c_vp, c_f32, c_f32,
                                 c_i64, c_vp, c_vp]),
    "vae2_bn_reduce_finalize": (c_int, [c_vp, c_i64, c_i64, c_vp, c_f64, c_vp, c_vp, c_vp, c_vp,
                                        c_vp, c_f32, c_f32, c_vp, c_vp]),
    "vae2_bn_bwd_reduce_param_grads": (c_int, [c_vp, c_i64, c_i64, c_vp, c_vp, c_vp, c_vp]),
    "vae2_bn_eval_coeffs": (c_int, [c_vp, c_vp, c_vp, c_vp, c_f32, c_i64, c_vp, c_vp]),
    "vae2_bn_apply": (c_int, [c_vp, P_ACT, c_vp, c_vp, P_ACT, c_vp, P_ACT, c_int, c_vp]),
    "vae2_bn_relu_bwd_reduce": (c_int, [c_vp, P_ACT, c_vp, P_ACT, c_vp, P_ACT, c_vp, c_int,
                                        c_vp, c_vp]),
    "vae2_bn_bwd_param_grads": (c_int, [c_vp, c_i64, c_vp, c_vp, c_vp]),
    "vae2_bn_relu_bwd_apply": (c_int, [c_vp, P_ACT, c_vp, P_ACT, c_vp, P_ACT, c_vp, c_vp,
                                       c_vp, c_f64, c_int, c_vp, P_ACT, c_vp, P_ACT, c_vp]),
    "vae2_upsample_bilinear_fwd": (c_int, [c_vp, P_ACT, c_vp, P_ACT, c_f32, c_vp]),
    "vae2_upsample_bilinear_bwd": (c_int, [c_vp, P_ACT, c_vp, P_ACT, c_f32, c_vp]),
    "vae2_fuse_sum_relu": (c_int, [c_int, ctypes.POINTER(c_vp), P_ACT, c_vp, P_ACT, c_vp]),
    "vae2_fuse_sum_relu_bn": (c_int, [c_int, ctypes.POINTER(c_vp), P_ACT, ctypes.POINTER(c_vp),
                                      c_vp, P_ACT, c_vp]),
    "vae2_relu_bwd_dual": (c_int, [c_vp, P_ACT, c_vp, P_ACT, c_vp, P_ACT, c_vp, P_ACT, c_f32,
                                   c_vp]),
    "vae2_relu_bwd": (c_int, [c_vp, P_ACT, c_vp, P_ACT, c_vp, P_ACT, c_vp]),
    "vae2_copy_act": (c_int, [c_vp, P_ACT, c_vp, P_ACT, c_f32, c_vp]),
    "vae2_codemap_tile_fwd": (c_int, [c_vp, c_i64, c_vp, P_ACT, c_vp]),
    "vae2_spatial_ws_size": (c_i64, [P_ACT]),
    "vae2_codemap_tile_bwd": (c_int, [c_vp, P_ACT, c_vp, c_i64, c_int, c_vp, c_i64, c_vp]),
    "vae2_nchw_to_nhwc": (c_int, [c_vp, c_vp, P_ACT, c_f32, c_vp]),
    "vae2_nhwc_to_nchw": (c_int, [c_vp, P_ACT, c_vp, c_f32, c_vp]),
    "vae2_global_avgpool_fwd": (c_int, [c_vp, P_ACT, c_vp, P_ACT, c_vp, c_i64, c_vp]),
    "vae2_global_avgpool_bwd": (c_int, [c_vp, P_ACT, c_vp, P_ACT, c_f32, c_vp]),
    "vae2_reduce_ws_size": (c_i64, [c_i64]),
    "vae2_l1_fwd": (c_int, [c_vp, P_ACT, c_vp, P_ACT, c_f32, c_vp, c_vp, c_vp]),
    "vae2_l1_bwd": (c_int, [c_vp, P_ACT, c_vp, P_ACT, c_vp, c_f32, c_vp, P_ACT, c_f32, c_vp]),
    "vae2_ssim_loss_ws_size": (c_i64, [P_ACT]),
    "vae2_ssim_loss_fwd": (c_int, [c_vp, P_ACT, c_vp, P_ACT, c_vp, c_vp, c_f32, c_f32, c_f32,
                                   c_vp, c_vp, c_vp]),
    "vae2_ssim_loss_bwd": (c_int, [c_vp, P_ACT, c_vp, P_ACT, c_vp, c_vp, c_f32, c_f32, c_vp,
                                   c_f32, c_vp, P_ACT, c_f32, c_vp]),
    "vae2_bn_multi_apply": (c_int, [c_int, c_vp, c_vp]),
    "vae2_bn_multi_bwd_reduce": (c_int, [c_int, c_vp, c_vp]),
    "vae2_bn_multi_bwd_apply": (c_int, [c_int, c_vp, c_vp]),
    "vae2_bn_multi_reduce": (c_int, [c_int, c_vp, c_int, c_vp]),
    "vae2_bn_multi_finalize": (c_int, [c_int, c_vp, c_vp]),
    "vae2_lsgan_fwd": (c_int, [c_vp, P_ACT, c_f32, c_f32, c_vp, c_vp, c_vp]),
    "vae2_lsgan_bwd": (c_int, [c_vp, P_ACT, c_f32, c_vp, c_f32, c_vp, P_ACT, c_f32, c_vp]),
    "vae2_reparam_kl_fwd": (c_int, [c_vp, P_ACT, c_vp, P_ACT, c_vp, P_ACT, c_int, c_f32, c_vp,
                                    c_int, c_vp, c_vp]),
    "vae2_reparam_kl_bwd": (c_int, [c_vp, P_ACT, c_vp, P_ACT, c_vp, P_ACT, c_vp, c_f32, c_vp,
                                    P_ACT, c_vp]),
    "vae2_weighted_sum": (c_int, [c_int, ctypes.POINTER(c_vp), ctypes.POINTER(c_f32), c_vp,
                                  c_vp]),
    "vae2_nonfinite_check": (c_int, [c_vp, c_i64, c_vp, c_vp]),
    "vae2_adam_coeffs": (c_int, [c_vp, c_f32, c_f32, c_vp, c_vp]),
    "vae2_adam_step_dev": (c_int, [c_vp, c_vp, c_vp, c_vp, c_i64, c_vp, c_f32, c_f32, c_f32,
                                   c_f32, c_vp]),
    "vae2_adam_step": (c_int, [c_vp, c_vp, c_vp, c_vp, c_i64, c_f32, c_f32, c_f32, c_f32, c_f32,
                               c_i64, c_vp]),
    "vae2_sgd_coeffs": (c_int, [c_vp, c_f32, c_f32, c_int, c_vp, c_vp]),
    "vae2_sgd_step_dev": (c_int, [c_vp, c_vp, c_vp, c_i64, c_vp, c_f32, c_f32, c_int, c_vp]),
    "vae2_sgd_step": (c_int, [c_vp, c_vp, c_vp, c_i64, c_f32, c_f32, c_f32, c_f32, c_int, c_int,
                              c_vp]),
    "vae2_grad_norm_ws_size": (c_i64, [c_i64]),
    "vae2_grad_sumsq": (c_int, [c_vp, c_i64, c_vp, c_vp]),
    "vae2_clip_coeffs": (c_int, [c_vp, c_i64, c_f32, c_vp, c_vp]),
    "vae2_sgd_step_dev_clip": (c_int, [c_vp, c_vp, c_vp, c_i64, c_vp, c_vp, c_f32, c_f32, c_int,
                                       c_vp]),
    "vae2_adam_step_dev_clip": (c_int, [c_vp, c_vp, c_vp, c_vp, c_i64, c_vp, c_vp, c_f32, c_f32,
                                        c_f32, c_f32, c_vp]),
    "vae2_scale_dev": (c_int, [c_vp, c_i64, c_vp, c_vp]),
    "vae2_ema_coeffs": (c_int, [c_vp, c_f32, c_vp, c_vp]),
    "vae2_ema_update_dev": (c_int, [c_vp, c_vp, c_i64, c_vp, c_vp]),
    "vae2_ema_update": (c_int, [c_vp, c_vp, c_i64, c_f32, c_int, c_vp]),
    "vae2_scale": (c_int, [c_vp, c_vp, c_i64, c_f32, c_vp]),
    "vae2_syncbn_comm_bytes": (c_i64, [c_int, c_i64]),
    "vae2_syncbn_comm_init": (c_int, [c_int, c_int, c_i64, c_vp, ctypes.POINTER(c_vp)]),
    "vae2_syncbn_comm_connect": (c_int, [c_vp, c_vp]),
    "vae2_syncbn_allreduce": (c_int, [c_vp, c_vp, c_i64, c_vp]),
    "vae2_syncbn_comm_error": (c_int, [c_vp, ctypes.POINTER(c_i64)]),
    "vae2_syncbn_comm_set_timeout": (c_int, [c_vp, ctypes.c_double]),
    "vae2_syncbn_comm_destroy": (c_int, [c_vp]),
    "vae2_clip_normalize_u8": (c_int, [c_vp, c_i64, c_i64, c_i64, c_i64, c_vp, c_int,
                                       ctypes.POINTER(c_vp), c_vp]),
    "vae2_to_image": (c_int, [c_vp, c_vp, c_i64, c_i64, c_i64, c_i64,
                              ctypes.POINTER(c_f64), ctypes.POINTER(c_f64), c_vp]),
    "vae2_metrics_ws_size": (c_i64, [c_i64, c_i64, c_i64]),
    "vae2_absdiff_sqdiff_sum": (c_int, [c_vp, c_vp, c_i64, c_vp, c_vp, c_vp]),
    "vae2_ssim": (c_int, [c_vp, c_vp, c_i64, c_i64, c_i64, c_vp, c_int, c_f32, c_f32, c_vp,
                          c_vp, c_vp]),
    "vae2_avgpool2x2": (c_int, [c_vp, c_vp, c_i64, c_i64, c_i64, c_vp]),
    "vae2_heads_set_algo": (c_int, [c_int]),
    "vae2_conv2d_multi": (c_int, [c_int, c_vp, c_vp]),
    "vae2_weighted_avgpool_fwd": (c_int, [c_vp, P_ACT, c_vp, c_vp, c_f32, c_vp, P_ACT, c_vp,
                                          c_i64, c_vp]),
    "vae2_weighted_avgpool_bwd": (c_int, [c_vp, P_ACT, c_vp, c_vp, c_f32, c_vp, P_ACT, c_f32,
                                          c_vp]),
    "vae2_conv2d_set_grouping": (c_int, [c_int]),
}

ABI_VERSION = 15
_lib = None


def load():
    global _lib
    if _lib is not None:
        return _lib
    if not os.path.exists(LIB_PATH):
        raise RuntimeError(
            f"libvae2_hip.so not found at {LIB_PATH}: build it with "
            "`python -c 'import __graft_entry__ as g; g.build()'` "
            "(there is no fallback compute path)")
    lib = ctypes.CDLL(LIB_PATH)
    for name, (res, args) in _SIGS.items():
        fn = getattr(lib, name)
        fn.restype = res
        fn.argtypes = args
    if lib.vae2_abi_version() != ABI_VERSION:
        raise RuntimeError("libvae2_hip.so ABI version mismatch; rebuild it")
    _lib = lib
    return lib


def exported_symbols():
    return sorted(_SIGS)


class PackJob(ctypes.Structure):
    _fields_ = [("w", c_vp), ("out", c_vp), ("cout", ctypes.c_int32), ("cin", ctypes.c_int32),
                ("k", ctypes.c_int32), ("mode", ctypes.c_int32), ("ld", ctypes.c_int32),
                ("pad_", ctypes.c_int32)]


class ConvJob(ctypes.Structure):
    _fields_ = [("kind", ctypes.c_int32), ("k", ctypes.c_int32), ("stride", ctypes.c_int32),
                ("pad", ctypes.c_int32), ("x", c_vp), ("xd", Act), ("wp", c_vp), ("bias", c_vp),
                ("y", c_vp), ("yd", Act), ("beta", c_f32), ("stats", c_vp)]


class HipError(RuntimeError):
    pass


def check(rc):
    if rc != 0:
        msg = load().vae2_last_error()
        raise HipError(f"libvae2_hip error {rc}: {msg.decode() if msg else ''}")


CALL_HOOK = None


def call(name, *args):
    fn = getattr(load(), name)
    if CALL_HOOK is not None:
        check(CALL_HOOK(name, fn, args))
    else:
        check(fn(*args))
```

### vae-2_amd/vae2/ops.py

```python
import collections
import ctypes
import functools
import itertools

import torch
import torch.distributed as dist

from . import _lib, prof, streams
from ._lib import Act, call

_F32 = torch.float32


def stream_ptr():
    return ctypes.c_void_p(torch.cuda.current_stream().cuda_stream)


def act_of(t):
    if t.dim() != 4 or t.dtype != _F32 or not t.is_cuda:
        raise ValueError(f"expected a 4-D float32 device tensor (N,H,W,C), got {tuple(t.shape)} "
                         f"{t.dtype} on {t.device}")
    n, h, w, c = t.shape
    s0, s1, s2, s3 = t.stride()
    if c > 1 and s3 != 1:
        raise ValueError("channel axis must be contiguous")
    if w > 1:
        ps = s2
    elif h > 1:
        ps = s1
    elif n > 1:
        ps = s0
    else:
        ps = c
    if (w > 1 and s2 != ps) or (h > 1 and s1 != w * ps) or (n > 1 and s0 != h * w * ps) or ps < c:
        raise ValueError(f"not a uniform NHWC view: shape {tuple(t.shape)} strides {t.stride()}")
    return ctypes.c_void_p(t.data_ptr()), Act(n, h, w, c, ps)


def as_act(t):
    try:
        act_of(t)
        return t
    except ValueError:
        return t.contiguous()


def ptr(t):
    return ctypes.c_void_p(t.data_ptr()) if t is not None else None


def _empty(shape, like, dtype=_F32):
    return torch.empty(shape, dtype=dtype, device=like.device)


def new_act(shape, like):
    n, h, w, c = shape
    cp = (c + 3) // 4 * 4
    buf = torch.empty((n, h, w, cp), dtype=_F32, device=like.device)
    return buf if cp == c else buf[..., :c]


def _grad_sink(p, need=True):
    if p is None or not need or not p.requires_grad:
        return None, None
    mg = getattr(p, "main_grad", None)
    if mg is not None:
        return mg, None
    g = torch.zeros_like(p)
    return g, g


def _bn_group():
    from . import dist as vdist
    return vdist.sync_bn_group()


def _all_reduce_sums(sums, count, group):
    if group is None:
        return sums, count
    from . import dist as vdist
    vdist.syncbn_all_reduce_(sums, group=group)
    return sums, count * dist.get_world_size(group)


class GradLink:

    __slots__ = ("n", "buf", "done")

    def __init__(self, n=2):
        self.n, self.buf, self.done = n, None, 0

    def finish(self):
        self.done += 1
        if self.done < self.n:
            return None
        buf, self.buf = self.buf, None
        return buf

    def hand_over(self, g, before_add=None):
        if self.buf is None:
            self.buf = g
        elif self.buf is not g:
            if before_add is not None:
                before_add(self.buf)
            self.buf.add_(g)
        return self.finish()


class _BNMarker:

    __slots__ = ("save", "relu", "part", "rows", "r", "claimed")

    def __init__(self):
        self.claimed = False
        self.publish(None, False)

    def claim(self):
        if self.claimed:
            raise RuntimeError("one consumer per marked BatchNorm output: already claimed")
        self.claimed = True

    def publish(self, save, relu, r=None):
        self.save, self.relu, self.r, self.part, self.rows = save, relu, r, None, 0

    def put_partials(self, part, rows):
        self.part, self.rows = part, rows

    def take_partials(self):
        part, self.part = self.part, None
        return part, self.rows


def _claim(markers):
    for m in markers or ():
        if isinstance(m, _BNMarker):
            m.claim()


class LazyBN(_BNMarker):
    __slots__ = ()


LAZY_BN = True


class PartBN(_BNMarker):
    __slots__ = ()


PART_BN = True


class ResBN:
    __slots__ = ()


RES_BN = True
MASK_BYTES = True
FUSE_LAZY = True


def lazy_bn_ok(shape, conv):
    if not LAZY_BN or not torch.cuda.is_available():
        return False
    n, h, w, c = shape
    k, st, pad = conv.kernel_size[0], conv.stride[0], conv.padding[0]
    if conv.in_channels != c:
        return False
    oh, ow = (h + 2 * pad - k) // st + 1, (w + 2 * pad - k) // st + 1
    xa = Act(n, h, w, c, (c + 3) // 4 * 4)
    ya = Act(n, oh, ow, conv.out_channels, (conv.out_channels + 3) // 4 * 4)
    return bool(_lib.load().vae2_conv2d_bnin_ok(ctypes.c_void_p(256), ctypes.byref(xa),
                                                ctypes.byref(ya), k, st, pad))


class ConvSpec:

    __slots__ = ("k", "stride", "pad", "relu", "bn", "momentum", "eps", "training", "x_link",
                 "res_link", "bn_in", "bn_out", "res_bn", "bn_part")

    def __init__(self, conv, bn=None, relu=False):
        kh, kw = conv.kernel_size
        if kh != kw or conv.stride[0] != conv.stride[1] or conv.padding[0] != conv.padding[1]:
            raise ValueError("only square kernels / strides / paddings are used by the model")
        if conv.groups != 1 or conv.dilation != (1, 1):
            raise ValueError("grouped / dilated convs are not used by the model")
        self.k, self.stride, self.pad = kh, conv.stride[0], conv.padding[0]
        self.relu = relu
        self.bn = bn
        self.x_link = self.res_link = None
        self.bn_in = self.bn_out = None
        self.bn_part = None
        self.res_bn = None
        if bn is not None:
            if bn.momentum is None:
                raise ValueError("cumulative-average BatchNorm (momentum=None) is not supported")
            self.momentum = float(bn.momentum)
            self.eps = float(bn.eps)
            self.training = bn.training or not bn.track_running_stats
        else:
            self.momentum = self.eps = 0.0
            self.training = False

    def out_hw(self, h, w):
        return ((h + 2 * self.pad - self.k) // self.stride + 1,
                (w + 2 * self.pad - self.k) // self.stride + 1)


class PackPlan:

    def __init__(self, module):
        lib = _lib.load()
        seen, self.weights, self.splits = set(), [], []
        for m in module.modules():
            if isinstance(m, torch.nn.Conv2d) and id(m.weight) not in seen:
                seen.add(id(m.weight))
                self.weights.append(m.weight)
                self.splits.append(getattr(m, "_vae2_col_split", None))
        self._blocks, total = [], 0
        for w, split in zip(self.weights, self.splits):
            cout, cin, k, _ = w.shape
            blocks, c0 = [], 0
            for cb in (split if split is not None else (cin,)):
                sizes = [lib.vae2_conv2d_packed_size(cout, cb, k, mode) for mode in (0, 1)]
                blocks.append((c0, cb, total, sizes[0], total + sizes[0], sizes[1]))
                total += sizes[0] + sizes[1]
                c0 += cb
            if c0 != cin:
                raise ValueError(f"column split {split} does not cover {cin} input channels")
            self._blocks.append(blocks)
        self.buf = torch.empty((total,), dtype=_F32,
                               device=self.weights[0].device if self.weights else None)
        self._views = [[(self.buf[a:a + na], self.buf[b:b + nb]) for _, _, a, na, b, nb in bl]
                       for bl in self._blocks]
        self._build_jobs()
        self.run()

    def _build_jobs(self):
        if not self.weights:
            self.njobs = 0
            return
        self._ptrs = [w.data_ptr() for w in self.weights]
        jobs = []
        for w, split, blocks, views in zip(self.weights, self.splits, self._blocks, self._views):
            cout, cin, k, _ = w.shape
            ld = cin * k * k if split is not None else 0
            for (c0, cb, *_), vv in zip(blocks, views):
                for mode in (0, 1):
                    jobs.append(_lib.PackJob(w.data_ptr() + 4 * c0 * k * k, vv[mode].data_ptr(),
                                             cout, cb, k, mode, ld, 0))
        arr = (_lib.PackJob * len(jobs))(*jobs)
        host = torch.frombuffer(bytearray(bytes(arr)), dtype=torch.uint8)
        self.jobs = host.to(self.buf.device)
        self.njobs = len(jobs)

    @torch.no_grad()
    def run(self):
        if not self.weights:
            return
        if any(w.data_ptr() != p for w, p in zip(self.weights, self._ptrs)):
            self._build_jobs()
        call("vae2_conv2d_pack_weights", ptr(self.jobs), self.njobs, stream_ptr())
        for w, split, views in zip(self.weights, self.splits, self._views):
            if split is None:
                w._vae2_packed = (views[0][0], views[0][1], w._version, w.data_ptr())
            else:
                w._vae2_packed_cols = (tuple(split), views, w._version, w.data_ptr())

    def bump_versions(self):
        torch.autograd.graph.increment_version(self.weights)
        self.run()


def packed_weight(weight, mode):
    cached = getattr(weight, "_vae2_packed", None)
    if cached is not None and cached[2] == weight._version and cached[3] == weight.data_ptr():
        return cached[mode]
    cout, cin, k, _ = weight.shape
    out = torch.empty((_lib.load().vae2_conv2d_packed_size(cout, cin, k, mode),),
                      dtype=_F32, device=weight.device)
    call("vae2_conv2d_pack_weight", ptr(weight), cout, cin, k, mode, ptr(out), stream_ptr())
    return out


def packed_weight_cols(weight, split, j, mode):
    split = tuple(split)
    cached = getattr(weight, "_vae2_packed_cols", None)
    if (cached is not None and cached[0] == split and cached[2] == weight._version and
            cached[3] == weight.data_ptr()):
        return cached[1][j][mode]
    cout, cin, k, _ = weight.shape
    c0, cb = sum(split[:j]), split[j]
    out = torch.empty((_lib.load().vae2_conv2d_packed_size(cout, cb, k, mode),),
                      dtype=_F32, device=weight.device)
    call("vae2_conv2d_pack_weight_ld", ctypes.c_void_p(weight.data_ptr() + 4 * c0 * k * k),
         cout, cb, k, mode, cin * k * k, ptr(out), stream_ptr())
    return out


def _conv_work(kind, xa, yshape, k, stride):
    n, oh, ow, cout = yshape
    prof.note(2.0 * n * oh * ow * cout * xa.c * k * k,
              4.0 * (xa.n * xa.h * xa.w * xa.c + n * oh * ow * cout + cout * xa.c * k * k),
              prof.conv_label(kind, xa.c, cout, k, stride, xa.h, xa.w))


class ConvGroup:

    def __init__(self):
        self.jobs, self.hold, self.outs, self.notes = [], [], set(), []

    def add(self, kind, x, xa, wp, bias, y, ya, spec, beta=0.0, stats=None):
        self.jobs.append(_lib.ConvJob(kind, spec.k, spec.stride, spec.pad, x, xa, ptr(wp),
                                      ptr(bias), y, ya, beta, ptr(stats)))
        self.hold.append((wp, bias, stats))
        self.outs.add(y.value if isinstance(y, ctypes.c_void_p) else int(y))
        self.notes.append(prof.take())

    def pending(self, t):
        return t is not None and t.data_ptr() in self.outs

    def flush(self):
        if not self.jobs:
            return
        if prof.active() and not _lib.load().vae2_conv2d_set_grouping(0):
            for job, work in zip(self.jobs, self.notes):
                prof.put(work)
                call("vae2_conv2d_multi", 1, (_lib.ConvJob * 1)(job), stream_ptr())
        else:
            if prof.active():
                _lib.load().vae2_conv2d_set_grouping(1)
                prof.put(_merge(self.notes))
            arr = (_lib.ConvJob * len(self.jobs))(*self.jobs)
            call("vae2_conv2d_multi", len(self.jobs), arr, stream_ptr())
        self.jobs, self.hold, self.outs, self.notes = [], [], set(), []


def _merge(notes):
    notes = [n for n in notes if n is not None]
    if not notes:
        return None
    return (sum(n[0] for n in notes), sum(n[1] for n in notes),
            " + ".join(n[2] for n in notes if n[2]))


def _conv_fwd(x, weight, bias, spec, stats=None, group=None, sp=None):
    sp = stream_ptr() if sp is None else sp
    xp, xa = act_of(x)
    n, h, w, _ = x.shape
    oh, ow = spec.out_hw(h, w)
    cout = weight.shape[0]
    y = new_act((n, oh, ow, cout), x)
    yp, ya = act_of(y)
    wp, lz = packed_weight(weight, 0), spec.bn_in
    if prof.active():
        _conv_work("fwd", xa, (n, oh, ow, cout), spec.k, spec.stride)
    if lz is not None:
        call("vae2_conv2d_fwd_bnin", xp, ctypes.byref(xa), ptr(lz.save), int(lz.relu), ptr(wp),
             ptr(bias), yp, ctypes.byref(ya), spec.k, spec.stride, spec.pad, 0.0, ptr(stats), sp)
    elif group is None:
        call("vae2_conv2d_fwd", xp, ctypes.byref(xa), ptr(wp), ptr(bias), yp, ctypes.byref(ya),
             spec.k, spec.stride, spec.pad, 0.0, ptr(stats), sp)
    else:
        group.add(0, xp, xa, wp, bias, yp, ya, spec, 0.0, stats)
    return y


_WGRAD_BATCH = [0]
_WS_HOLD = []
_WGRAD_CB = [False, -1]


def flush_wgrad(own_stream=False):
    cur = torch.cuda.current_stream() if torch.cuda.is_available() else None
    if own_stream:
        key = cur.cuda_stream if cur is not None else None
        if _FLUSH_EV[0] is not None and cur is not None:
            cur.wait_event(_FLUSH_EV[0])
        call("vae2_wgrad_flush_stream", stream_ptr())
        keep = [(k, t_) for k, t_ in _WS_HOLD if k != key]
        _WS_HOLD[:] = keep
        return
    streams.join_all()
    try:
        call("vae2_wgrad_flush", stream_ptr())
    finally:
        if cur is not None:
            for _, t_ in _WS_HOLD:
                if t_.is_cuda:
                    t_.record_stream(cur)
            ev = torch.cuda.Event()
            ev.record(cur)
            _FLUSH_EV[0] = ev
        _WS_HOLD.clear()


_FLUSH_EV = [None]


def _end_of_backward():
    _WGRAD_CB[0] = False
    flush_wgrad()
    _FLUSH_EV[0] = None


def _graph_task():
    try:
        return torch._C._current_graph_task_id()
    except (AttributeError, RuntimeError):
        return -1


class wgrad_batch:

    def __enter__(self):
        if _WGRAD_BATCH[0] == 0 and _WGRAD_CB[0] and _WGRAD_CB[1] != _graph_task():
            _end_of_backward()
        _lib.load().vae2_wgrad_defer(1)
        _WGRAD_BATCH[0] += 1
        return self

    def __exit__(self, *exc):
        _WGRAD_BATCH[0] -= 1
        if _WGRAD_BATCH[0] == 0:
            _lib.load().vae2_wgrad_defer(0)
            if not _WGRAD_CB[0]:
                try:
                    torch.autograd.Variable._execution_engine.queue_callback(_end_of_backward)
                    _WGRAD_CB[0], _WGRAD_CB[1] = True, _graph_task()
                except RuntimeError:
                    flush_wgrad()
        return False


class _defer_off:

    __slots__ = ("on", "prev")

    def __init__(self, on=True):
        self.on = on

    def __enter__(self):
        if self.on:
            self.prev = _lib.load().vae2_wgrad_defer(0)
        return self

    def __exit__(self, *exc):
        if self.on:
            _lib.load().vae2_wgrad_defer(self.prev)
        return False


def _conv_bwd(x, weight, bias, dy, spec, need_dx, need_w=True, need_b=True, group=None,
              sp=None, hold=None):
    s = stream_ptr() if sp is None else sp
    xv, dyv = act_of(x), act_of(dy)
    wret, bret, ws = _conv_wgrad(x, xv, weight, bias, dy, dyv, spec, need_w, need_b, s=s,
                                 lane=sp is not None, hold=hold)
    if not need_dx or getattr(x, "_vae2_no_dx", False):
        return None, wret, bret
    return _conv_dgrad(x, xv, weight, dy, dyv, spec, group=group, s=s, hold=hold), wret, bret


def _conv_wgrad(x, xv, weight, bias, dy, dyv, spec, need_w, need_b, *, s, lane, hold):
    (xp, xa), (dyp, dya) = xv, dyv
    wsink, wret = _grad_sink(weight, need_w)
    bsink, bret = _grad_sink(bias, need_b)
    if wsink is None and bsink is None:
        return wret, bret, None
    tmp_w = wsink is None
    if tmp_w:
        wsink = torch.zeros_like(weight)
    size = _lib.load().vae2_conv2d_bwd_weight_ws_size(ctypes.byref(xa), ctypes.byref(dya), spec.k)
    ws = _empty((max(size, 1),), x)
    if prof.active():
        _conv_work("wgrad", xa, tuple(dy.shape), spec.k, spec.stride)
    lz = spec.bn_in
    now = wret is not None or tmp_w or lane
    if lane and hold is not None:
        hold.append(ws)
    with _defer_off(now and _WGRAD_BATCH[0] > 0):
        if lz is not None:
            call("vae2_conv2d_bwd_weight_bnin", xp, ctypes.byref(xa), ptr(lz.save),
                 int(lz.relu), dyp, ctypes.byref(dya), ptr(wsink), ptr(bsink), spec.k,
                 spec.stride, spec.pad, 1, ptr(ws), size, s)
        else:
            call("vae2_conv2d_bwd_weight", xp, ctypes.byref(xa), dyp, ctypes.byref(dya),
                 ptr(wsink), ptr(bsink), spec.k, spec.stride, spec.pad, 1, ptr(ws), size, s)
    if _WGRAD_BATCH[0] and not now:
        _WS_HOLD.append((torch.cuda.current_stream().cuda_stream, ws))
    return wret, bret, ws


def _conv_dgrad(x, xv, weight, dy, dyv, spec, *, group, s, hold):
    (xp, xa), (dyp, dya) = xv, dyv
    link, beta = spec.x_link, 0.0
    if link is not None and link.buf is not None:
        dx, beta = link.buf, 1.0
    else:
        dx = new_act(tuple(x.shape), x)
        if link is not None:
            link.buf = dx
    (dxp, dxa), wp = act_of(dx), packed_weight(weight, 1)
    if prof.active():
        _conv_work("dgrad", xa, tuple(dy.shape), spec.k, spec.stride)
    lz, src = spec.bn_in, spec.bn_in if spec.bn_in is not None else spec.bn_part
    if lz is None and src is not None and (src.r is None or src.save is None or
                                           link is not None):
        src = None
    rows = 0
    if src is not None and beta == 0.0:
        rows = _lib.load().vae2_conv2d_bwd_data_bnpart_rows(
            dyp, ctypes.byref(dya), ctypes.byref(dxa), spec.k, spec.stride, spec.pad)
    if rows > 0:
        part = _empty((2 * rows * xa.c,), x)
        if hold is not None:
            hold.append(part)
        bxp, bxa = (xp, xa) if lz is not None else act_of(src.r)
        call("vae2_conv2d_bwd_data_bnpart", dyp, ctypes.byref(dya), ptr(wp), dxp,
             ctypes.byref(dxa), spec.k, spec.stride, spec.pad, bxp, ctypes.byref(bxa),
             ptr(src.save), int(src.relu), ptr(part), s)
        src.put_partials(part, rows)
    elif group is not None:
        group.add(1, dyp, dya, wp, None, dxp, dxa, spec, beta)
    else:
        call("vae2_conv2d_bwd_data", dyp, ctypes.byref(dya), ptr(wp), dxp,
             ctypes.byref(dxa), spec.k, spec.stride, spec.pad, beta, s)
    return link.finish() if link is not None else dx


_In = collections.namedtuple("_In", "x weight bias gamma beta residual")


def _layer_needs(need, i):
    k = len(_In._fields)
    return _In(*need[1 + k * i:1 + k * (i + 1)])


def _level_grads(per_layer):
    return (None, *itertools.chain.from_iterable(per_layer))


def _running_ptrs(bn):
    if bn.track_running_stats and bn.running_mean is not None:
        return ptr(bn.running_mean), ptr(bn.running_var), ptr(bn.num_batches_tracked)
    return None, None, None


class _ConvBN(torch.autograd.Function):

    @staticmethod
    def forward(ctx, x, weight, bias, gamma, beta, residual, spec):
        s = stream_ptr()
        bn, group = spec.bn, None
        L = _Layer(spec, _In(x, weight, bias, gamma, beta, residual))
        r, stats, cout, count, rows = L.conv(stats=spec.training), L.stats, L.cout, L.count, L.rows
        if spec.training:
            sums = _empty((2 * cout,), x, torch.float64)
            group = _bn_group()
            save = _empty((4 * cout,), x)
            stat_ptrs = _running_ptrs(bn)
            if group is None:
                if count <= 1:
                    raise ValueError("Expected more than 1 value per channel when training, "
                                     f"got input size {(x.shape[0], cout, *r.shape[1:3])}")
                call("vae2_bn_reduce_finalize", ptr(stats), rows, cout, ptr(sums), count,
                     ptr(gamma), ptr(beta), *stat_ptrs, spec.momentum, spec.eps, ptr(save), s)
            else:
                call("vae2_bn_partials_reduce", ptr(stats), rows, cout, ptr(sums), 0, s)
                sums, count = _all_reduce_sums(sums, count, group)
                if count <= 1:
                    raise ValueError("Expected more than 1 value per channel when training")
                call("vae2_bn_finalize", ptr(sums), count, ptr(gamma), ptr(beta), *stat_ptrs,
                     spec.momentum, spec.eps, cout, ptr(save), s)
        else:
            save = _empty((4 * cout,), x)
            call("vae2_bn_eval_coeffs", ptr(gamma), ptr(beta), ptr(bn.running_mean),
                 ptr(bn.running_var), spec.eps, cout, ptr(save), s)
        y = new_act(tuple(r.shape), x)
        rp, ra = act_of(r)
        yp, ya = act_of(y)
        resp, resa = act_of(residual) if residual is not None else (None, ya)
        if prof.active():
            prof.note(0, 4.0 * r.numel() * (3 if residual is not None else 2))
        call("vae2_bn_apply", rp, ctypes.byref(ra), ptr(save), resp, ctypes.byref(resa), yp,
             ctypes.byref(ya), int(spec.relu), s)
        ctx.spec, ctx.count, ctx.group, ctx.has_res = spec, count, group, residual is not None
        ctx.params = (weight, bias, gamma, beta)
        ctx.save_for_backward(x, r, y, save)
        return y

    @staticmethod
    def backward(ctx, dy):
        if not ctx.spec.training:
            raise RuntimeError("backward through an eval-mode BatchNorm is not supported")
        s = stream_ptr()
        x, r, y, save = ctx.saved_tensors
        (weight, bias, gamma, beta), spec = ctx.params, ctx.spec
        need = _In(*ctx.needs_input_grad[:len(_In._fields)])
        dy, cout = as_act(dy), r.shape[3]
        (dyp, dya), (rp, ra), (yp, ya) = act_of(dy), act_of(r), act_of(y)
        if not ctx.has_res:
            yp = None
        rows = _lib.load().vae2_bn_partial_rows(ctypes.byref(ra))
        part = _empty((2 * rows * cout,), r)
        if prof.active():
            prof.note(0, 4.0 * r.numel() * (3 if yp is not None else 2))
        call("vae2_bn_relu_bwd_reduce", dyp, ctypes.byref(dya), yp, ctypes.byref(ya), rp,
             ctypes.byref(ra), ptr(save), int(spec.relu), ptr(part), s)
        lsums = _empty((2 * cout,), r, torch.float64)
        gsink, gret = _grad_sink(gamma, need.gamma)
        bsink, bret = _grad_sink(beta, need.beta)
        call("vae2_bn_bwd_reduce_param_grads", ptr(part), rows, cout, ptr(lsums), ptr(gsink),
             ptr(bsink), s)
        gsums, _ = _all_reduce_sums(lsums, ctx.count, ctx.group)
        dr = new_act(tuple(r.shape), r)
        drp, dra = act_of(dr)
        dres = new_act(tuple(r.shape), r) if ctx.has_res and need.residual else None
        dresp, dresa = act_of(dres) if dres is not None else (None, dra)
        if prof.active():
            prof.note(0, 4.0 * r.numel() * (3 + (1 if yp is not None else 0) +
                                             (1 if dres is not None else 0)))
        call("vae2_bn_relu_bwd_apply", dyp, ctypes.byref(dya), yp, ctypes.byref(ya), rp,
             ctypes.byref(ra), ptr(save), ptr(gamma), ptr(gsums), ctx.count, int(spec.relu), drp,
             ctypes.byref(dra), dresp, ctypes.byref(dresa), s)
        if dres is not None and spec.res_link is not None:
            dres = spec.res_link.hand_over(dres)
        dx, wret, bret_conv = _conv_bwd(x, weight, bias, dr, spec, need.x, need.weight, need.bias)
        return (*_In(dx, wret, bret_conv, gret, bret, dres), None)


def conv_bn(x, conv, bn, relu, residual=None, x_link=None, res_link=None, bn_part=None):
    _claim((bn_part,))
    spec = ConvSpec(conv, bn, relu)
    spec.x_link, spec.res_link = x_link, res_link
    spec.bn_part = bn_part if PART_BN else None
    if spec.training and (residual is None or _bn_quad_ok(residual)):
        return _ConvBNMulti.apply((spec,), x, conv.weight, conv.bias, bn.weight, bn.bias,
                                  residual)[0]
    return _ConvBN.apply(x, conv.weight, conv.bias, bn.weight, bn.bias, residual, spec)


def _bn_quad_ok(t):
    p_, a = act_of(t)
    return p_.value % 16 == 0 and a.ps % 4 == 0 and a.c <= 1024


@functools.lru_cache(maxsize=None)
def _counts_dev(counts, device):
    return torch.tensor(counts, dtype=torch.float64).to(device)


LEVEL_LANES = 0
LEVEL_LANES_BWD = True


class _Lanes:

    def __init__(self, specs, enabled=True):
        self.on = False
        self.lane = [0] * len(specs)
        if (not enabled or LEVEL_LANES <= 1 or len(specs) < 2 or not torch.cuda.is_available()
                or prof.active()):
            return
        keys = []
        for i, sp in enumerate(specs):
            key = id(sp.x_link) if sp.x_link is not None else ("solo", i)
            if key not in keys:
                keys.append(key)
            self.lane[i] = keys.index(key) % LEVEL_LANES
        if max(self.lane) == 0:
            return
        self.parent = torch.cuda.current_stream()
        if streams.role_of(self.parent) != "main":
            return
        self.streams = {k: streams.side_stream(self.parent.device, ("lane", "main", k))
                        for k in sorted(set(self.lane) - {0})}
        self.on = torch.cuda.is_current_stream_capturing()
        if not self.on:
            return
        for st in self.streams.values():
            st.wait_stream(self.parent)
            streams._FORKED.add(st)

    def ptr(self, i):
        if not self.on or self.lane[i] == 0:
            return None
        return ctypes.c_void_p(self.streams[self.lane[i]].cuda_stream)

    def join(self):
        if self.on:
            for st in self.streams.values():
                self.parent.wait_stream(st)

    def sync(self):
        if self.on:
            self.join()
            for st in self.streams.values():
                st.wait_stream(self.parent)


class _Layer:
    __slots__ = _In._fields + ("spec", "has_res", "cout", "count", "rows", "stats", "r", "save",
                               "y", "mask", "dy", "dr", "dres", "acc", "gret", "bret")

    def __init__(self, spec, ins):
        self.cout = self.count = self.rows = self.stats = self.r = self.save = self.y = None
        self.mask = self.dy = self.dr = self.dres = self.acc = self.gret = self.bret = None
        self.spec, self.has_res = spec, ins.residual is not None
        self.x, self.weight, self.bias, self.gamma, self.beta, self.residual = ins

    def conv(self, group=None, sp=None, stats=True):
        x, spec = self.x, self.spec
        n, h, w, _ = x.shape
        oh, ow = spec.out_hw(h, w)
        cout, self.count = self.weight.shape[0], float(n * oh * ow)
        self.cout = cout
        if stats:
            xp, xa = act_of(x)
            self.rows = _lib.load().vae2_conv2d_fwd_stats_rows(
                xp, ctypes.byref(xa), ctypes.byref(Act(n, oh, ow, cout, cout)), spec.k,
                spec.stride, spec.pad)
            self.stats = _empty((2 * self.rows * cout,), x)
        self.r = _conv_fwd(x, self.weight, self.bias, spec, self.stats, group, sp)
        return self.r


def _sums_layout(layers, group):
    n, tot = len(layers), 2 * sum(L.cout for L in layers)
    buf = _empty((tot + n,), layers[0].r, torch.float64)
    if group is not None:
        buf[tot:].copy_(_counts_dev(tuple(L.count for L in layers), buf.device))
    base, off, ptrs = buf.data_ptr(), 0, []
    for i, L in enumerate(layers):
        ptrs.append((base + 8 * off, base + 8 * (tot + i) if group is not None else None))
        off += 2 * L.cout
    return buf, ptrs


def _bn_fin(L, sums_p, countp=None, gamma=None, beta=None, running=(None, None, None),
            momentum=0.0, eps=0.0, save=None, dgamma=None, dbeta=None):
    return _lib.BnFin(L.stats.data_ptr(), L.rows, L.cout, sums_p, countp, L.count, ptr(gamma),
                      ptr(beta), *running, momentum, eps, ptr(save), ptr(dgamma), ptr(dbeta))


def _ride_shortcut(layer, S, rsums_p=None):
    layer.rx, layer.rxd, layer.rsave = S.r.data_ptr(), act_of(S.r)[1], S.save.data_ptr()
    if rsums_p is not None:
        layer.rgamma, layer.rpartials, layer.rsums = ptr(S.gamma), S.stats.data_ptr(), rsums_p
        layer.rdx, layer.rdxd = S.dr.data_ptr(), act_of(S.dr)[1]


def _bn_note(kind, Ls, passes):
    if prof.active():
        prof.note(0, sum(4.0 * L.r.numel() * passes(L) for L in Ls),
                  f"{kind} " + " + ".join("%d@%dx%d" % (L.r.shape[3], *L.r.shape[1:3]) for L in Ls))


def _level_convs(layers):
    lanes = _Lanes([L.spec for L in layers])
    cg = None if lanes.on else ConvGroup()
    for i, L in enumerate(layers):
        L.conv(cg, lanes.ptr(i))
        L.save = _empty((4 * L.cout,), L.x)
    if cg is not None:
        cg.flush()
    lanes.join()


def _level_stats(layers, group, s):
    n = len(layers)
    buf, sp = _sums_layout(layers, group)
    world = dist.get_world_size(group) if group is not None else 1
    arr = (_lib.BnFin * n)()
    for i, L in enumerate(layers):
        if L.count * world <= 1:
            raise ValueError("Expected more than 1 value per channel when training, "
                             f"got input size {(L.count, L.cout)}")
        arr[i] = _bn_fin(L, *sp[i], L.gamma, L.beta, _running_ptrs(L.spec.bn), L.spec.momentum,
                         L.spec.eps, L.save)
    if group is None:
        call("vae2_bn_multi_reduce", n, arr, 0, s)
    else:
        call("vae2_bn_multi_reduce", n, arr, 2, s)
        from . import dist as vdist
        vdist.syncbn_all_reduce_(buf, group=group)
        call("vae2_bn_multi_finalize", n, arr, s)
    return buf


def _level_apply(layers, s):
    lay = []
    for L in layers:
        spec, lz, res = L.spec, L.spec.bn_out, L.residual
        if isinstance(lz, PartBN):
            lz.publish(L.save, spec.relu, L.r if res is None and spec.res_bn is None else None)
        elif lz is not None:
            if not isinstance(lz, ResBN):
                lz.publish(L.save, spec.relu)
            L.y = L.r
            continue
        L.y = new_act(tuple(L.r.shape), L.r)
        layer = _bn_layer(L.r, res, L.y, None, None, L.save, None, None, None, None, 0.0,
                          spec.relu)
        if MASK_BYTES and spec.relu and (res is not None or spec.res_bn is not None):
            _, ya_ = act_of(L.y)
            L.mask = torch.empty((ya_.n * ya_.h * ya_.w * ((ya_.c + 3) // 4),),
                                 dtype=torch.uint8, device=L.y.device)
            layer.mask = L.mask.data_ptr()
        if spec.res_bn is not None:
            _ride_shortcut(layer, layers[spec.res_bn])
        lay.append(layer)
    if lay:
        _bn_note("bn apply", [L for L in layers if L.spec.bn_out is None],
                 lambda L: 3 if L.has_res or L.spec.res_bn is not None else 2)
        call("vae2_bn_multi_apply", len(lay), (_lib.BnLayer * len(lay))(*lay), s)


def _resbn_buffers(layers):
    for L in layers:
        if isinstance(L.spec.bn_out, ResBN):
            L.rows = _lib.load().vae2_bn_partial_rows(ctypes.byref(act_of(L.r)[1]))
            L.stats = _empty((2 * L.rows * L.cout,), L.r)
            L.dr = new_act(tuple(L.r.shape), L.r)


def _bn_bwd_descs(ctx, layers, dys, sp):
    n = len(layers)
    lay, fins, red, act = (_lib.BnLayer * n)(), (_lib.BnFin * n)(), [], []
    for i, L in enumerate(layers):
        spec, r, lz, need = L.spec, L.r, L.spec.bn_out, _layer_needs(ctx.needs_input_grad, i)
        own = not isinstance(lz, ResBN)
        if own:
            act.append(i)
            dy = as_act(dys[i]) if dys[i] is not None else torch.zeros_like(L.y)
            L.dy = dy if _bn_quad_ok(dy) else _aligned_copy(dy)
            L.stats, L.rows = (lz.take_partials() if lz is not None and dys[i] is not None
                               else (None, 0))
            if L.stats is None:
                L.rows = _lib.load().vae2_bn_partial_rows(ctypes.byref(act_of(r)[1]))
                L.stats = _empty((2 * L.rows * L.cout,), r)
                red.append(i)
            L.dr, L.acc, link = new_act(tuple(r.shape), r), 0, spec.res_link
            if L.has_res and need.residual:
                if (link is not None and link.buf is not None and
                        tuple(link.buf.shape) == tuple(r.shape) and _bn_quad_ok(link.buf)):
                    L.dres, L.acc = link.buf, 1
                else:
                    L.dres = new_act(tuple(r.shape), r)
        gsink, L.gret = _grad_sink(L.gamma, need.gamma)
        bsink, L.bret = _grad_sink(L.beta, need.beta)
        fins[i] = _bn_fin(L, sp[i][0], dgamma=gsink, dbeta=bsink)
        if own:
            y = L.y if (L.has_res or spec.res_bn is not None) and L.mask is None else None
            layer = _bn_layer(r, y, L.dr, L.dy, L.dres, L.save, L.gamma, L.stats, *sp[i],
                              L.count, spec.relu, L.acc)
            if L.mask is not None:
                layer.mask = L.mask.data_ptr()
            if spec.res_bn is not None:
                _ride_shortcut(layer, layers[spec.res_bn], sp[spec.res_bn][0])
            lay[i] = layer
    return lay, fins, red, act


def _bn_bwd_launch(layers, descs, buf, group, s):
    lay, fins, red, act = descs
    if red:
        _bn_note("bn bwd reduce", [layers[i] for i in red],
                 lambda L: 2 + _y_reads(L) + (1 if L.spec.res_bn is not None else 0))
        call("vae2_bn_multi_bwd_reduce", len(red),
             (_lib.BnLayer * len(red))(*[lay[i] for i in red]), s)
    call("vae2_bn_multi_reduce", len(layers), fins, 1, s)
    if group is not None:
        from . import dist as vdist
        vdist.syncbn_all_reduce_(buf, group=group)
    _bn_note("bn bwd apply", [layers[i] for i in act],
             lambda L: (3 + _y_reads(L) + (1 if L.dres is not None else 0) +
                        (2 if L.spec.res_bn is not None else 0)))
    call("vae2_bn_multi_bwd_apply", len(act), (_lib.BnLayer * len(act))(*[lay[i] for i in act]),
         s)


def _level_conv_grads(ctx, layers):
    grads, hold = [], []
    lanes = _Lanes([L.spec for L in layers], LEVEL_LANES_BWD)
    cg = None if lanes.on else ConvGroup()

    def settle(buf):
        if cg is not None and cg.pending(buf):
            cg.flush()
        lanes.sync()

    with wgrad_batch():
        for i, L in enumerate(layers):
            need, dres = _layer_needs(ctx.needs_input_grad, i), L.dres
            if dres is not None and L.spec.res_link is not None:
                dres = L.spec.res_link.hand_over(dres, settle)
            dx, wret, bret_conv = _conv_bwd(L.x, L.weight, L.bias, L.dr, L.spec, need.x,
                                            need.weight, need.bias, group=cg, sp=lanes.ptr(i),
                                            hold=hold)
            grads.append(_In(dx, wret, bret_conv, L.gret, L.bret, dres))
        if cg is not None:
            cg.flush()
        lanes.join()
    del hold
    return _level_grads(grads)


class _ConvBNMulti(torch.autograd.Function):

    @staticmethod
    def forward(ctx, specs, *flat):
        s = stream_ptr()
        ctx.group = _bn_group()
        ins = map(_In._make, zip(*[iter(flat)] * len(_In._fields)))
        layers = [_Layer(spec, i_) for spec, i_ in zip(specs, ins)]
        _level_convs(layers)
        sums = _level_stats(layers, ctx.group, s)
        _level_apply(layers, s)
        ys = tuple(L.y for L in layers)
        ctx.save_for_backward(*[t for L in layers for t in (L.x, L.r, L.y, L.save)])
        for L in layers:
            L.x = L.r = L.y = L.save = L.residual = L.stats = None
        ctx.layers = layers
        del sums
        return ys

    @staticmethod
    def backward(ctx, *dys):
        s = stream_ptr()
        layers = ctx.layers
        for L, saved in zip(layers, zip(*[iter(ctx.saved_tensors)] * 4)):
            L.x, L.r, L.y, L.save = saved
        buf, sp = _sums_layout(layers, ctx.group)
        _resbn_buffers(layers)
        descs = _bn_bwd_descs(ctx, layers, dys, sp)
        _bn_bwd_launch(layers, descs, buf, ctx.group, s)
        grads = _level_conv_grads(ctx, layers)
        for L in layers:
            L.x = L.r = L.y = L.save = L.stats = L.dy = L.dr = L.dres = L.gret = L.bret = None
        return grads


def _y_reads(L):
    if L.mask is not None:
        return 1.0 / 16.0
    return 1 if L.has_res or L.spec.res_bn is not None else 0


def _aligned_copy(t):
    out = new_act(tuple(t.shape), t)
    (tp, ta), (op, oa) = act_of(t), act_of(out)
    call("vae2_copy_act", tp, ctypes.byref(ta), op, ctypes.byref(oa), 0.0, stream_ptr())
    return out


def _bn_layer(x, a, o, dy, dres, save, gamma, part, sums_p, countp, count, relu, dres_acc=0):
    def d(t):
        return act_of(t)[1] if t is not None else Act(0, 0, 0, 0, 0)
    return _lib.BnLayer(ptr(x), d(x), ptr(a), d(a), ptr(o), d(o), ptr(dy), d(dy), ptr(dres),
                        d(dres), ptr(save), ptr(gamma), ptr(part), sums_p, countp, float(count),
                        int(relu), int(dres_acc))


BN_BATCH = True


def _check_res_bns(res_bns, xs, convs, specs, residuals, bn_outs):
    for i, j in enumerate(res_bns):
        if j is None:
            continue
        if (residuals[i] is not None or residuals[j] is not None or specs[j].relu or
                res_bns[j] is not None or bn_outs[i] is not None or bn_outs[j] is not None):
            raise ValueError("res_bns: the shortcut layer must be a plain conv + BN")
        shp = [(xs[k].shape[0], *specs[k].out_hw(xs[k].shape[1], xs[k].shape[2]),
                convs[k].out_channels) for k in (i, j)]
        if shp[0] != shp[1]:
            raise ValueError(f"res_bns: shortcut output {shp[1]} != layer output {shp[0]}")
        specs[i].res_bn = j
        specs[j].bn_out = ResBN()


def conv_bn_multi(xs, convs, bns, relu, residuals=None, x_links=None, res_links=None,
                  bn_outs=None, bn_ins=None, res_bns=None):
    n = len(xs)
    nones = [None] * n
    residuals, x_links, res_links = residuals or nones, x_links or nones, res_links or nones
    outs_, ins_, res_bns = bn_outs or nones, bn_ins or nones, res_bns or nones
    relus = relu if isinstance(relu, (list, tuple)) else [relu] * n
    _claim(ins_)
    specs = []
    for i in range(n):
        spec = ConvSpec(convs[i], bns[i], relus[i])
        spec.x_link, spec.res_link, spec.bn_out = x_links[i], res_links[i], outs_[i]
        if isinstance(ins_[i], PartBN):
            spec.bn_part = ins_[i] if PART_BN else None
        else:
            spec.bn_in = ins_[i]
        specs.append(spec)
    _check_res_bns(res_bns, xs, convs, specs, residuals, outs_)
    if (not BN_BATCH or not RES_BN and any(j is not None for j in res_bns)
            or not all(sp.training for sp in specs) or
            not all(r is None or _bn_quad_ok(r) for r in residuals)):
        if any(sp.bn_in is not None for sp in specs):
            raise RuntimeError("a LazyBN input needs the batched training path")
        if bn_outs is not None:
            bn_outs[:] = nones
        outs = [None] * n
        order = [j for j in range(n) if j in res_bns]
        order += [i for i in range(n) if i not in order]
        for i in order:
            res = outs[res_bns[i]] if res_bns[i] is not None else residuals[i]
            outs[i] = conv_bn(xs[i], convs[i], bns[i], relus[i], res, x_links[i], res_links[i])
        return outs
    flat = [t for i in range(n) for t in _In(xs[i], convs[i].weight, convs[i].bias,
                                             bns[i].weight, bns[i].bias, residuals[i])]
    return list(_ConvBNMulti.apply(tuple(specs), *flat))


class _Conv(torch.autograd.Function):
    @staticmethod
    def forward(ctx, x, weight, bias, spec):
        y = _conv_fwd(x, weight, bias, spec)
        ctx.spec, ctx.params = spec, (weight, bias)
        ctx.save_for_backward(x)
        return y

    @staticmethod
    def backward(ctx, dy):
        (x,) = ctx.saved_tensors
        weight, bias = ctx.params
        dx, wret, bret = _conv_bwd(x, weight, bias, as_act(dy), ctx.spec, ctx.needs_input_grad[0],
                                   ctx.needs_input_grad[1], ctx.needs_input_grad[2])
        return dx, wret, bret, None


def conv(x, conv_mod):
    return _Conv.apply(x, conv_mod.weight, conv_mod.bias, ConvSpec(conv_mod))


def _up_bwd(g, shape):
    dx = new_act(shape, g)
    gp, ga = act_of(g)
    dxp, dxa = act_of(dx)
    call("vae2_upsample_bilinear_bwd", gp, ctypes.byref(ga), dxp, ctypes.byref(dxa), 0.0,
         stream_ptr())
    return dx


UP_POW2 = True


def _up_bwd_pow2(g, shapes):
    if not UP_POW2 or len(shapes) > 3:
        return None
    lib = _lib.load()
    gp, ga = act_of(g)
    dxs = [new_act(shp, g) for shp in shapes]
    views = [act_of(d) for d in dxs]
    acts = (Act * len(dxs))(*[a for _, a in views])
    wsz = lib.vae2_upsample_bilinear_bwd_pow2_ws_size(ctypes.byref(ga), len(dxs), acts)
    if wsz < 0 or ga.ps % 4 or g.data_ptr() % 16:
        return None
    ptrs = (ctypes.c_void_p * len(dxs))(*[p for p, _ in views])
    ws = _empty((max(wsz, 1),), g)
    call("vae2_upsample_bilinear_bwd_pow2", gp, ctypes.byref(ga), len(dxs), ptrs, acts, None,
         ptr(ws), wsz, stream_ptr())
    return dxs


class _FuseSum(torch.autograd.Function):
    @staticmethod
    def forward(ctx, out_hw, links, lazies, *terms):
        ref = terms[0]
        n, c = ref.shape[0], ref.shape[3]
        y = new_act((n, out_hw[0], out_hw[1], c), ref)
        ptrs = (ctypes.c_void_p * len(terms))()
        acts = (Act * len(terms))()
        for i, t in enumerate(terms):
            p_, a_ = act_of(t)
            ptrs[i] = p_
            acts[i] = a_
        yp, ya = act_of(y)
        if lazies is not None and any(lz is not None for lz in lazies):
            sv = (ctypes.c_void_p * len(terms))(*[ptr(lz.save) if lz is not None else None
                                                  for lz in lazies])
            call("vae2_fuse_sum_relu_bn", len(terms), ptrs, acts, sv, yp, ctypes.byref(ya),
                 stream_ptr())
        else:
            call("vae2_fuse_sum_relu", len(terms), ptrs, acts, yp, ctypes.byref(ya),
                 stream_ptr())
        ctx.shapes = [tuple(t.shape) for t in terms]
        ctx.links = links
        ctx.save_for_backward(y)
        return y

    @staticmethod
    def backward(ctx, dy):
        (y,) = ctx.saved_tensors
        dy = as_act(dy)
        g = new_act(tuple(y.shape), y)
        dyp, dya = act_of(dy)
        yp, ya = act_of(y)
        gp, ga = act_of(g)
        links = ctx.links or (None,) * len(ctx.shapes)
        lk = next((i for i, l in enumerate(links) if l is not None), None)
        if lk is not None and ctx.needs_input_grad[lk + 3]:
            link = links[lk]
            beta = 0.0
            if link.buf is None:
                link.buf = new_act(tuple(y.shape), y)
            else:
                beta = 1.0
            bp, ba = act_of(link.buf)
            call("vae2_relu_bwd_dual", dyp, ctypes.byref(dya), yp, ctypes.byref(ya), gp,
                 ctypes.byref(ga), bp, ctypes.byref(ba), beta, stream_ptr())
        else:
            lk = None
            call("vae2_relu_bwd", dyp, ctypes.byref(dya), yp, ctypes.byref(ya), gp,
                 ctypes.byref(ga), stream_ptr())
        grads = []
        ups = [i for i, shp in enumerate(ctx.shapes)
               if ctx.needs_input_grad[i + 3] and i != lk and shp[1:3] != tuple(y.shape[1:3])]
        upg = _up_bwd_pow2(g, [ctx.shapes[i] for i in ups]) if ups else None
        for i, shp in enumerate(ctx.shapes):
            if not ctx.needs_input_grad[i + 3]:
                grads.append(None)
            elif i == lk:
                grads.append(links[i].finish())
            elif shp[1:3] == tuple(y.shape[1:3]):
                grads.append(g)
            elif upg is not None:
                grads.append(upg[ups.index(i)])
            else:
                grads.append(_up_bwd(g, shp))
        return (None, None, None, *grads)


def fuse_sum_relu(terms, out_hw, links=None, lazies=None):
    _claim(lazies)
    return _FuseSum.apply(tuple(out_hw), tuple(links) if links else None,
                          tuple(lazies) if lazies else None, *terms)


class _UpCat(torch.autograd.Function):

    @staticmethod
    def forward(ctx, *xs):
        x0 = xs[0]
        n, h, w, _ = x0.shape
        ctot = sum(t.shape[3] for t in xs)
        y = new_act((n, h, w, ctot), x0)
        s = stream_ptr()
        off = 0
        for t in xs:
            c = t.shape[3]
            dst = y[..., off:off + c]
            tp, ta = act_of(t)
            dp_, da = act_of(dst)
            if t.shape[1:3] == x0.shape[1:3]:
                call("vae2_copy_act", tp, ctypes.byref(ta), dp_, ctypes.byref(da), 0.0, s)
            else:
                call("vae2_upsample_bilinear_fwd", tp, ctypes.byref(ta), dp_, ctypes.byref(da), 0.0,
                     s)
            off += c
        ctx.shapes = [tuple(t.shape) for t in xs]
        return y

    @staticmethod
    def backward(ctx, dy):
        dy = as_act(dy)
        grads = []
        off = 0
        for i, shp in enumerate(ctx.shapes):
            c = shp[3]
            sl = dy[..., off:off + c]
            off += c
            if not ctx.needs_input_grad[i]:
                grads.append(None)
            elif shp[1:3] == tuple(dy.shape[1:3]):
                grads.append(sl)
            else:
                grads.append(_up_bwd(sl, shp))
        return tuple(grads)


def up_cat(xs):
    return _UpCat.apply(*xs)


class _Cat(torch.autograd.Function):

    @staticmethod
    def forward(ctx, out_hw, tiles, *parts):
        ref = parts[0]
        n = ref.shape[0]
        ctot = sum(p_.shape[3] for p_ in parts)
        y = new_act((n, out_hw[0], out_hw[1], ctot), ref)
        s = stream_ptr()
        off = 0
        for p_, tile in zip(parts, tiles):
            c = p_.shape[3]
            dst = y[..., off:off + c]
            dp_, da = act_of(dst)
            pp, pa = act_of(p_)
            if tile:
                call("vae2_codemap_tile_fwd", pp, pa.ps, dp_, ctypes.byref(da), s)
            else:
                call("vae2_copy_act", pp, ctypes.byref(pa), dp_, ctypes.byref(da), 0.0, s)
            off += c
        ctx.tiles = tiles
        ctx.shapes = [tuple(p_.shape) for p_ in parts]
        return y

    @staticmethod
    def backward(ctx, dy):
        dy = as_act(dy)
        grads = []
        off = 0
        lib = _lib.load()
        for i, (shp, tile) in enumerate(zip(ctx.shapes, ctx.tiles)):
            c = shp[3]
            sl = dy[..., off:off + c]
            off += c
            if not ctx.needs_input_grad[i + 2]:
                grads.append(None)
            elif tile:
                g = _empty(shp, dy)
                sp, sa = act_of(sl)
                wsz = lib.vae2_spatial_ws_size(ctypes.byref(sa))
                ws = _empty((max(wsz, 1),), dy)
                gp, ga = act_of(g)
                call("vae2_codemap_tile_bwd", sp, ctypes.byref(sa), gp, ga.ps, 0, ptr(ws), wsz,
                     stream_ptr())
                grads.append(g)
            else:
                grads.append(sl)
        return (None, None, *grads)


def cat(parts, out_hw, tiles=None):
    tiles = tuple(tiles) if tiles is not None else (False,) * len(parts)
    return _Cat.apply(tuple(out_hw), tiles, *parts)


class _AvgPool(torch.autograd.Function):
    @staticmethod
    def forward(ctx, x):
        n, h, w, c = x.shape
        y = _empty((n, 1, 1, c), x)
        xp, xa = act_of(x)
        yp, ya = act_of(y)
        wsz = _lib.load().vae2_spatial_ws_size(ctypes.byref(xa))
        ws = _empty((max(wsz, 1),), x)
        call("vae2_global_avgpool_fwd", xp, ctypes.byref(xa), yp, ctypes.byref(ya), ptr(ws), wsz,
             stream_ptr())
        ctx.shape = tuple(x.shape)
        return y

    @staticmethod
    def backward(ctx, dy):
        dy = as_act(dy)
        dx = new_act(ctx.shape, dy)
        dyp, dya = act_of(dy)
        dxp, dxa = act_of(dx)
        call("vae2_global_avgpool_bwd", dyp, ctypes.byref(dya), dxp, ctypes.byref(dxa), 0.0,
             stream_ptr())
        return dx


def avgpool(x):
    return _AvgPool.apply(x)


_POOLW = {}


def _pool_weights(n_in, n_out, device):
    key = (n_in, n_out, str(device))
    t = _POOLW.get(key)
    if t is None:
        import numpy as np
        w = np.zeros(n_in, dtype=np.float64)
        scale = np.float32(n_in) / np.float32(n_out)
        for o in range(n_out):
            src = max(np.float32(0.0), np.float32(scale * np.float32(o + 0.5) - np.float32(0.5)))
            i0 = int(src)
            l1 = float(src - np.float32(i0))
            i1 = i0 + 1 if i0 < n_in - 1 else i0
            w[i0] += 1.0 - l1
            w[i1] += l1
        t = torch.tensor(w, dtype=torch.float32, device=device)
        _POOLW[key] = t
    return t


class _UpAvgPool(torch.autograd.Function):

    @staticmethod
    def forward(ctx, *xs):
        x0 = xs[0]
        n, H, W, _ = x0.shape
        ctot = sum(t.shape[3] for t in xs)
        y = _empty((n, 1, 1, ctot), x0)
        s = stream_ptr()
        scale = 1.0 / (H * W)
        off = 0
        ws_keep = []
        for t in xs:
            c = t.shape[3]
            tp, ta = act_of(t)
            ya = Act(n, 1, 1, c, ctot)
            yp = ctypes.c_void_p(y.data_ptr() + 4 * off)
            wsz = _lib.load().vae2_spatial_ws_size(ctypes.byref(ta))
            ws = _empty((max(wsz, 1),), x0)
            ws_keep.append(ws)
            if t.shape[1:3] == x0.shape[1:3]:
                call("vae2_global_avgpool_fwd", tp, ctypes.byref(ta), yp, ctypes.byref(ya),
                     ptr(ws), wsz, s)
            else:
                wr = _pool_weights(t.shape[1], H, x0.device)
                wc = _pool_weights(t.shape[2], W, x0.device)
                call("vae2_weighted_avgpool_fwd", tp, ctypes.byref(ta), ptr(wr), ptr(wc),
                     scale, yp, ctypes.byref(ya), ptr(ws), wsz, s)
            off += c
        ctx.shapes = [tuple(t.shape) for t in xs]
        ctx.hw = (H, W)
        return y

    @staticmethod
    def backward(ctx, dy):
        dy = dy.contiguous()
        H, W = ctx.hw
        s = stream_ptr()
        ctot = dy.shape[3]
        grads = []
        off = 0
        for i, shp in enumerate(ctx.shapes):
            c = shp[3]
            if not ctx.needs_input_grad[i]:
                grads.append(None)
                off += c
                continue
            dx = new_act(shp, dy)
            dxp, dxa = act_of(dx)
            da = Act(shp[0], 1, 1, c, ctot)
            dp_ = ctypes.c_void_p(dy.data_ptr() + 4 * off)
            if shp[1:3] == (H, W):
                call("vae2_global_avgpool_bwd", dp_, ctypes.byref(da), dxp, ctypes.byref(dxa),
                     0.0, s)
            else:
                wr = _pool_weights(shp[1], H, dy.device)
                wc = _pool_weights(shp[2], W, dy.device)
                call("vae2_weighted_avgpool_bwd", dp_, ctypes.byref(da), ptr(wr), ptr(wc),
                     1.0 / (H * W), dxp, ctypes.byref(dxa), 0.0, s)
            grads.append(dx)
            off += c
        return tuple(grads)


UP_AVGPOOL = True


def up_avgpool(xs):
    if not UP_AVGPOOL:
        return avgpool(up_cat(xs))
    return _UpAvgPool.apply(*xs)


class _ToNHWC(torch.autograd.Function):
    @staticmethod
    def forward(ctx, x):
        x = x.contiguous()
        n, c, h, w = x.shape
        y = new_act((n, h, w, c), x)
        yp, ya = act_of(y)
        call("vae2_nchw_to_nhwc", ptr(x), yp, ctypes.byref(ya), 0.0, stream_ptr())
        return y

    @staticmethod
    def backward(ctx, dy):
        dy = as_act(dy)
        n, h, w, c = dy.shape
        dx = _empty((n, c, h, w), dy)
        dyp, dya = act_of(dy)
        call("vae2_nhwc_to_nchw", dyp, ctypes.byref(dya), ptr(dx), 0.0, stream_ptr())
        return dx


class _ToNCHW(torch.autograd.Function):
    @staticmethod
    def forward(ctx, x):
        n, h, w, c = x.shape
        y = _empty((n, c, h, w), x)
        xp, xa = act_of(x)
        call("vae2_nhwc_to_nchw", xp, ctypes.byref(xa), ptr(y), 0.0, stream_ptr())
        return y

    @staticmethod
    def backward(ctx, dy):
        dy = dy.contiguous()
        n, c, h, w = dy.shape
        dx = new_act((n, h, w, c), dy)
        dxp, dxa = act_of(dx)
        call("vae2_nchw_to_nhwc", ptr(dy), dxp, ctypes.byref(dxa), 0.0, stream_ptr())
        return dx


def to_nhwc(x):
    return _ToNHWC.apply(x)


def to_nchw(x):
    return _ToNCHW.apply(x)


def _flat_act(t):
    t = t.contiguous()
    return t, Act(1, 1, t.numel(), 1, 1)


class _L1(torch.autograd.Function):
    @staticmethod
    def forward(ctx, p, t, scale, flat):
        if flat:
            p, pa = _flat_act(p)
            t, ta = _flat_act(t)
            pp, tp = ptr(p), ptr(t)
        else:
            pp, pa = act_of(p)
            tp, ta = act_of(t)
        n = pa.n * pa.h * pa.w * pa.c
        ws = _empty((_lib.load().vae2_reduce_ws_size(n),), p)
        out = _empty((), p)
        call("vae2_l1_fwd", pp, ctypes.byref(pa), tp, ctypes.byref(ta), scale, ptr(ws), ptr(out),
             stream_ptr())
        ctx.scale = scale
        ctx.flat = flat
        ctx.save_for_backward(p, t)
        return out

    @staticmethod
    def backward(ctx, gout):
        p, t = ctx.saved_tensors
        gout = gout.contiguous()
        if ctx.flat:
            _, pa = _flat_act(p)
            _, ta = _flat_act(t)
            dp = torch.empty_like(p)
            _, da = _flat_act(dp)
            pp, tp, dpp = ptr(p), ptr(t), ptr(dp)
        else:
            pp, pa = act_of(p)
            tp, ta = act_of(t)
            dp = new_act(tuple(p.shape), p)
            dpp, da = act_of(dp)
        call("vae2_l1_bwd", pp, ctypes.byref(pa), tp, ctypes.byref(ta), ptr(gout), ctx.scale, dpp,
             ctypes.byref(da), 0.0, stream_ptr())
        return dp, None, None, None


def l1(pred, target, scale, flat=False):
    return _L1.apply(pred, target, float(scale), flat)


_SSIM_COEFFS = {}


def ssim_coeffs(device, channels):
    key = (str(device), int(channels))
    ab = _SSIM_COEFFS.get(key)
    if ab is None:
        from .metrics import MEAN, STD
        a = torch.tensor([STD[c % 3] for c in range(channels)], dtype=_F32).to(device)
        b = torch.tensor([MEAN[c % 3] for c in range(channels)], dtype=_F32).to(device)
        ab = _SSIM_COEFFS[key] = (a, b)
    return ab


class _SSIMLoss(torch.autograd.Function):
    @staticmethod
    def forward(ctx, p, t, scale, a, b, c1, c2):
        pp, pa = act_of(p)
        tp, ta = act_of(t)
        if (a is None) != (b is None):
            raise ValueError("ssim_loss: a and b must be given together")
        for coef in (a, b):
            if coef is not None and (coef.dtype != _F32 or coef.device != p.device
                                     or coef.numel() != pa.c or not coef.is_contiguous()):
                raise ValueError("ssim_loss: a, b must be dense float32 [channels] tensors on "
                                 "the predictions' device")
        ws = _empty((_lib.load().vae2_ssim_loss_ws_size(ctypes.byref(pa)),), p, torch.float64)
        out = _empty((), p)
        call("vae2_ssim_loss_fwd", pp, ctypes.byref(pa), tp, ctypes.byref(ta), ptr(a), ptr(b),
             c1, c2, scale, ptr(ws), ptr(out), stream_ptr())
        ctx.consts = (scale, c1, c2)
        ctx.save_for_backward(p, t, a, b)
        return out

    @staticmethod
    def backward(ctx, gout):
        p, t, a, b = ctx.saved_tensors
        scale, c1, c2 = ctx.consts
        gout = gout.contiguous()
        pp, pa = act_of(p)
        tp, ta = act_of(t)
        dp = new_act(tuple(p.shape), p)
        dpp, da = act_of(dp)
        call("vae2_ssim_loss_bwd", pp, ctypes.byref(pa), tp, ctypes.byref(ta), ptr(a), ptr(b),
             c1, c2, ptr(gout), scale, dpp, ctypes.byref(da), 0.0, stream_ptr())
        return dp, None, None, None, None, None, None


def ssim_loss(pred, target, scale, a=None, b=None, c1=1e-4, c2=9e-4):
    return _SSIMLoss.apply(pred, target, float(scale), a, b, float(c1), float(c2))


class _LSGAN(torch.autograd.Function):
    @staticmethod
    def forward(ctx, x, target, scale, flat):
        if flat:
            x, xa = _flat_act(x)
            xp = ptr(x)
        else:
            xp, xa = act_of(x)
        ws = _empty((_lib.load().vae2_reduce_ws_size(xa.n * xa.h * xa.w * xa.c),), x)
        out = _empty((), x)
        call("vae2_lsgan_fwd", xp, ctypes.byref(xa), target, scale, ptr(ws), ptr(out),
             stream_ptr())
        ctx.target, ctx.scale, ctx.flat = target, scale, flat
        ctx.save_for_backward(x)
        return out

    @staticmethod
    def backward(ctx, gout):
        (x,) = ctx.saved_tensors
        gout = gout.contiguous()
        if ctx.flat:
            _, xa = _flat_act(x)
            dx = torch.empty_like(x)
            xp, dxp, dxa = ptr(x), ptr(dx), xa
        else:
            xp, xa = act_of(x)
            dx = new_act(tuple(x.shape), x)
            dxp, dxa = act_of(dx)
        call("vae2_lsgan_bwd", xp, ctypes.byref(xa), ctx.target, ptr(gout), ctx.scale, dxp,
             ctypes.byref(dxa), 0.0, stream_ptr())
        return dx, None, None, None


def lsgan(sample, real, scale, flat=False):
    return _LSGAN.apply(sample, 1.0 if real else 0.0, float(scale), flat)


class _SplitFrames(torch.autograd.Function):

    @staticmethod
    def forward(ctx, x, nframes):
        n, h, w, c = x.shape
        if 3 * nframes > c:
            raise ValueError(f"{nframes} RGB frames do not fit {c} channels (the reference's "
                             "frame loop needs CLIP_LENGTH 3 or more, utils.py:116)")
        s = stream_ptr()
        outs = []
        for f in range(nframes):
            o = new_act((n, h, w, 3), x)
            sp, sa = act_of(x[..., 3 * f:3 * f + 3])
            op, oa = act_of(o)
            call("vae2_copy_act", sp, ctypes.byref(sa), op, ctypes.byref(oa), 0.0, s)
            outs.append(o)
        ctx.shape = tuple(x.shape)
        return tuple(outs)

    @staticmethod
    def backward(ctx, *gs):
        n, h, w, c = ctx.shape
        ref = next(g for g in gs if g is not None)
        dx = new_act(ctx.shape, ref)
        if 3 * len(gs) < c or any(g is None for g in gs):
            dx.zero_()
        s = stream_ptr()
        for f, g in enumerate(gs):
            if g is None:
                continue
            g = as_act(g)
            gp, ga = act_of(g)
            dp_, da = act_of(dx[..., 3 * f:3 * f + 3])
            call("vae2_copy_act", gp, ctypes.byref(ga), dp_, ctypes.byref(da), 0.0, s)
        return dx, None


def split_frames(x, nframes):
    return _SplitFrames.apply(x, int(nframes))


class _ReparamKL(torch.autograd.Function):
    @staticmethod
    def forward(ctx, muvar, eps, prior, scale):
        n, h, w, c2 = muvar.shape
        zc = c2 // 2
        z = new_act((n, h, w, zc), muvar)
        kl = _empty((), muvar)
        mp, ma = act_of(muvar)
        ep, ea = act_of(eps)
        zp, za = act_of(z)
        ws = _empty((_lib.load().vae2_reduce_ws_size(n * h * w * zc),), muvar)
        call("vae2_reparam_kl_fwd", mp, ctypes.byref(ma), ep, ctypes.byref(ea), zp, ctypes.byref(za),
             int(prior), scale, ptr(kl), 0, ptr(ws), stream_ptr())
        ctx.scale = scale
        ctx.prior = prior
        ctx.save_for_backward(muvar, eps)
        return z, kl

    @staticmethod
    def backward(ctx, dz, dkl):
        muvar, eps = ctx.saved_tensors
        dm = new_act(tuple(muvar.shape), muvar)
        mp, ma = act_of(muvar)
        ep, ea = act_of(eps)
        dmp, dma = act_of(dm)
        if dz is not None and not ctx.prior:
            dz = as_act(dz)
            dzp, dza = act_of(dz)
        else:
            dzp, dza = None, ea
        gk = dkl.contiguous() if dkl is not None else None
        call("vae2_reparam_kl_bwd", mp, ctypes.byref(ma), ep, ctypes.byref(ea), dzp, ctypes.byref(dza),
             ptr(gk), ctx.scale, dmp, ctypes.byref(dma), stream_ptr())
        return dm, None, None, None


def reparam_kl(muvar, eps, prior=False, scale=1.0):
    return _ReparamKL.apply(muvar, eps, bool(prior), float(scale))


class _WeightedSum(torch.autograd.Function):
    @staticmethod
    def forward(ctx, lambdas, *terms):
        n = len(terms)
        ptrs = (ctypes.c_void_p * n)(*[t.data_ptr() for t in terms])
        lams = (ctypes.c_float * n)(*lambdas)
        out = _empty((), terms[0])
        call("vae2_weighted_sum", n, ptrs, lams, ptr(out), stream_ptr())
        ctx.lambdas = lambdas
        return out

    @staticmethod
    def backward(ctx, g):
        g = g.contiguous()
        grads = []
        for i, lam in enumerate(ctx.lambdas):
            if not ctx.needs_input_grad[i + 1]:
                grads.append(None)
                continue
            d = torch.empty_like(g)
            call("vae2_scale", ptr(d), ptr(g), 1, float(lam), stream_ptr())
            grads.append(d)
        return (None, *grads)


def weighted_sum(terms, lambdas):
    return _WeightedSum.apply(tuple(float(x) for x in lambdas), *terms)


def nonfinite_flag(tensors, flag=None):
    if flag is None:
        flag = torch.zeros((1,), dtype=torch.int32, device=tensors[0].device)
    for t in tensors:
        t = t.detach()
        if not t.is_contiguous():
            t = t.contiguous()
        call("vae2_nonfinite_check", ptr(t), t.numel(), ptr(flag), stream_ptr())
    return flag
```

Measured before the change: 921.5 frames/s.

## Batch narrow 3x3 weight-gradient kernels of a level into one multi-job launch

Adds a grouped weight-gradient path. Eligible 3x3 direct convs in a multi-branch level (cq=9, 8-wave plan) are collected in Python and launched as a single multi-job kernel, up to four jobs, with blocks partitioned across jobs. The kernel body is also factored into a device function with a LEAN variant that hoists scalar values into SGPRs, adds register-pressure hints and moves the remainder FMA loop out of the MFMA loop. The aim is to cut launch overhead and fill the GPU better when several small wgrad kernels run back to back. The cost is a more complex host path, and a reordering in which all wgrads of a level are issued before the dgrads.

```diff
diff --git a/include/vae2_hip.h b/include/vae2_hip.h
--- a/include/vae2_hip.h
+++ b/include/vae2_hip.h
@@ -100,6 +100,26 @@
                               const vae2_act* dyd, float* dw, int64_t dw_ld, float* dbias,
                               int k, int stride, int pad, int accumulate, float* ws,
                               int64_t ws_size, void* stream);
+
+typedef struct vae2_wgrad_job {
+  const float* x;
+  vae2_act xd;
+  const float* dy;
+  vae2_act dyd;
+  float* dw;
+  int64_t dw_ld;
+  float* dbias;
+  int32_t k, stride, pad, accumulate;
+  float* ws;
+  int64_t ws_size;
+  const float* bn_save;
+  int32_t relu;
+  int32_t pad_;
+} vae2_wgrad_job;
+int vae2_conv2d_bwd_weight_multi(int n, const vae2_wgrad_job* jobs, void* stream);
+int vae2_wgrad_set_multi(int on);
+int vae2_conv2d_bwd_weight_shares(const float* x, const vae2_act* xd, const float* dy,
+                                  const vae2_act* dyd, int k, int stride, int pad);
 
 
 int64_t vae2_bn_partial_rows(const vae2_act* xd);
diff --git a/vae-2_amd/csrc/conv.h b/vae-2_amd/csrc/conv.h
--- a/vae-2_amd/csrc/conv.h
+++ b/vae-2_amd/csrc/conv.h
@@ -125,6 +125,19 @@
 bool dconv_use(const vae2_act* ad, const vae2_act* yd, int k, int stride, int pad,
                const float* a);
 int64_t dconv_rows(const vae2_act* ad, const vae2_act* yd);
+struct WgnJob {
+  const float* x;
+  const vae2_act* xd;
+  const float* dy;
+  const vae2_act* dyd;
+  float* part;
+  const float* isave;
+  int irelu;
+  uint32_t x_bytes, dy_bytes;
+};
+constexpr int kWgnMaxJobs = 4;
+bool wgrad3n_shares(const vae2_act* xd, const vae2_act* dyd);
+int wgrad3n_launch_multi(int n, const WgnJob* jobs, int* splits, hipStream_t s);
 bool wgrad3_shape_ok(const vae2_act* xd, const vae2_act* dyd, int k, int stride, int pad);
 
 }
diff --git a/vae-2_amd/csrc/conv_wgrad.hip b/vae-2_amd/csrc/conv_wgrad.hip
--- a/vae-2_amd/csrc/conv_wgrad.hip
+++ b/vae-2_amd/csrc/conv_wgrad.hip
@@ -863,25 +863,51 @@
   return wgrad_ws(xd, dyd, k).total;
 }
 
-static int bwd_weight_impl(const float* x, const vae2_act* xd, const float* dy,
-                           const vae2_act* dyd, float* dw, int64_t dw_ld, float* dbias,
-                           int k, int stride, int pad, int accumulate, float* ws,
-                           int64_t ws_size, void* stream, const float* isave, int irelu,
-                           const char* fn) {
-  VAE2_REQUIRE(xd && dw_ld >= xd->c * k * k, fn, "bad dW row stride");
-  VAE2_REQUIRE(x && dy && dw && ws, fn, "null pointer");
-  VAE2_REQUIRE(conv_shapes_ok(xd, dyd, k, stride, pad), fn, "inconsistent conv shapes");
-  VAE2_REQUIRE(fits32(xd) && fits32(dyd), fn, "tensor too large for 32-bit indexing");
-  const WgradWs wsl = wgrad_ws(xd, dyd, k);
-  VAE2_REQUIRE(ws_size >= wsl.total, fn, "workspace too small");
-  hipStream_t s = as_stream(stream);
+struct WJob {
+  const float* x;
+  const vae2_act* xd;
+  const float* dy;
+  const vae2_act* dyd;
+  float* dw;
+  int64_t dw_ld;
+  float* dbias;
+  int k, stride, pad, accumulate;
+  float* ws;
+  int64_t ws_size;
+  void* stream;
+  const float* isave;
+  int irelu;
+  const char* fn;
+};
+
+static bool wgrad_direct(const WJob& j) {
+  return g_conv_algo != 1 && wgrad3_shape_ok(j.xd, j.dyd, j.k, j.stride, j.pad) &&
+         vec_ok(j.x, (int)j.xd->ps) && vec_ok(j.dy, (int)j.dyd->ps);
+}
+
+static int wgrad_check(const WJob& j) {
+  const char* fn = j.fn;
+  VAE2_REQUIRE(j.xd && j.dw_ld >= j.xd->c * j.k * j.k, fn, "bad dW row stride");
+  VAE2_REQUIRE(j.x && j.dy && j.dw && j.ws, fn, "null pointer");
+  VAE2_REQUIRE(conv_shapes_ok(j.xd, j.dyd, j.k, j.stride, j.pad), fn, "inconsistent conv shapes");
+  VAE2_REQUIRE(fits32(j.xd) && fits32(j.dyd), fn, "tensor too large for 32-bit indexing");
+  VAE2_REQUIRE(j.ws_size >= wgrad_ws(j.xd, j.dyd, j.k).total, fn, "workspace too small");
+  VAE2_REQUIRE(wgrad_direct(j) || !j.isave, fn,
+               "input BatchNorm needs the direct 3x3 weight-gradient kernel (vae2_conv2d_bnin_ok)");
+  return 0;
+}
+
+static int wgrad_main(const WJob& j, int* splits_out) {
+  const float *x = j.x, *dy = j.dy, *isave = j.isave;
+  const vae2_act *xd = j.xd, *dyd = j.dyd;
+  const int k = j.k, stride = j.stride, pad = j.pad, irelu = j.irelu;
+  float* ws = j.ws;
+  const char* fn = j.fn;
+  hipStream_t s = as_stream(j.stream);
   const int cin4 = round_up((int)xd->c, 4);
   const int ncol4 = k * k * cin4;
   int splits = 0;
-  const bool direct = g_conv_algo != 1 && wgrad3_shape_ok(xd, dyd, k, stride, pad) &&
-                      vec_ok(x, (int)xd->ps) && vec_ok(dy, (int)dyd->ps);
-  VAE2_REQUIRE(direct || !isave, fn,
-               "input BatchNorm needs the direct 3x3 weight-gradient kernel (vae2_conv2d_bnin_ok)");
+  const bool direct = wgrad_direct(j);
   if (direct && k == 3) {
     splits = wgrad3n_launch(x, xd, dy, dyd, ws, isave, irelu, act_bytes(xd), act_bytes(dyd), s);
     if (splits < 0) return check_launch(fn);
@@ -907,36 +933,49 @@
     if (rc) return rc;
     splits = t3.splits;
   }
-  WTile t = pick_wtile(act_pixels(dyd), (int)dyd->c, ncol4);
-  if (splits) goto reduce;
-  {
-  WGrad p{};
-  p.x = x; p.x_ps = (int)xd->ps; p.cin = (int)xd->c; p.cin4 = cin4;
-  p.x_h = (int)xd->h; p.x_w = (int)xd->w;
-  p.dy = dy; p.dy_ps = (int)dyd->ps; p.cout = (int)dyd->c;
-  p.o_n = (int)dyd->n; p.o_h = (int)dyd->h; p.o_w = (int)dyd->w;
-  p.k = k; p.stride = stride; p.pad = pad;
-  p.P = (int)act_pixels(dyd);
-  p.px_split = t.px_split;
-  p.part = ws;
-  p.x_bytes = act_bytes(xd);
-  p.dy_bytes = act_bytes(dyd);
-  p.ohw_div = FastDiv((uint32_t)(dyd->h * dyd->w));
-  p.ow_div = FastDiv((uint32_t)dyd->w);
-  p.cin4_div = FastDiv((uint32_t)cin4);
-  dim3 grid(t.gx, t.gy, (unsigned)t.splits);
-  const bool v4 = g_vec_out && vec_ok(x, (int)xd->ps) && vec_ok(dy, (int)dyd->ps);
-  switch (t.tm) {
-    case 1: launch_wgrad_tn<1>(p, t.tn, grid, s, v4); break;
-    case 2: launch_wgrad_tn<2>(p, t.tn, grid, s, v4); break;
-    case 3: launch_wgrad_tn<3>(p, t.tn, grid, s, v4); break;
-    default: launch_wgrad_tn<4>(p, t.tn, grid, s, v4); break;
-  }
-  int rc = check_launch(fn);
-  if (rc) return rc;
-  splits = t.splits;
-  }
-reduce:
+  if (!splits) {
+    WTile t = pick_wtile(act_pixels(dyd), (int)dyd->c, ncol4);
+    WGrad p{};
+    p.x = x; p.x_ps = (int)xd->ps; p.cin = (int)xd->c; p.cin4 = cin4;
+    p.x_h = (int)xd->h; p.x_w = (int)xd->w;
+    p.dy = dy; p.dy_ps = (int)dyd->ps; p.cout = (int)dyd->c;
+    p.o_n = (int)dyd->n; p.o_h = (int)dyd->h; p.o_w = (int)dyd->w;
+    p.k = k; p.stride = stride; p.pad = pad;
+    p.P = (int)act_pixels(dyd);
+    p.px_split = t.px_split;
+    p.part = ws;
+    p.x_bytes = act_bytes(xd);
+    p.dy_bytes = act_bytes(dyd);
+    p.ohw_div = FastDiv((uint32_t)(dyd->h * dyd->w));
+    p.ow_div = FastDiv((uint32_t)dyd->w);
+    p.cin4_div = FastDiv((uint32_t)cin4);
+    dim3 grid(t.gx, t.gy, (unsigned)t.splits);
+    const bool v4 = g_vec_out && vec_ok(x, (int)xd->ps) && vec_ok(dy, (int)dyd->ps);
+    switch (t.tm) {
+      case 1: launch_wgrad_tn<1>(p, t.tn, grid, s, v4); break;
+      case 2: launch_wgrad_tn<2>(p, t.tn, grid, s, v4); break;
+      case 3: launch_wgrad_tn<3>(p, t.tn, grid, s, v4); break;
+      default: launch_wgrad_tn<4>(p, t.tn, grid, s, v4); break;
+    }
+    int rc = check_launch(fn);
+    if (rc) return rc;
+    splits = t.splits;
+  }
+  *splits_out = splits;
+  return 0;
+}
+
+static int wgrad_tail(const WJob& j, int splits) {
+  const vae2_act *xd = j.xd, *dyd = j.dyd;
+  const int k = j.k, accumulate = j.accumulate;
+  float *ws = j.ws, *dw = j.dw, *dbias = j.dbias;
+  const int64_t dw_ld = j.dw_ld;
+  void* stream = j.stream;
+  const char* fn = j.fn;
+  hipStream_t s = as_stream(stream);
+  const int cin4 = round_up((int)xd->c, 4);
+  const int ncol4 = k * k * cin4;
+  const WgradWs wsl = wgrad_ws(xd, dyd, k);
   int64_t slab = dyd->c * (int64_t)ncol4;
   int rc = 0;
   if (g_wr_defer) {
@@ -952,10 +991,89 @@
   }
   if (dbias) {
     float* bp = ws + wsl.part;
-    rc = vae2_bn_stats(dy, dyd, bp, stream);
+    rc = vae2_bn_stats(j.dy, dyd, bp, stream);
     if (rc) return rc;
     rc = bias_grad_from_partials(bp, vae2_bn_partial_rows(dyd), dyd->c, dbias, accumulate,
                                  stream);
+    if (rc) return rc;
+  }
+  return 0;
+}
+
+static int bwd_weight_impl(const float* x, const vae2_act* xd, const float* dy,
+                           const vae2_act* dyd, float* dw, int64_t dw_ld, float* dbias,
+                           int k, int stride, int pad, int accumulate, float* ws,
+                           int64_t ws_size, void* stream, const float* isave, int irelu,
+                           const char* fn) {
+  const WJob j{x, xd, dy, dyd, dw, dw_ld, dbias, k, stride, pad, accumulate, ws, ws_size,
+               stream, isave, irelu, fn};
+  int rc = wgrad_check(j), splits = 0;
+  if (rc) return rc;
+  rc = wgrad_main(j, &splits);
+  return rc ? rc : wgrad_tail(j, splits);
+}
+
+static int g_wgrad_multi = 1;
+
+int vae2_wgrad_set_multi(int on) {
+  const int prev = g_wgrad_multi;
+  g_wgrad_multi = on != 0;
+  return prev;
+}
+
+int vae2_conv2d_bwd_weight_shares(const float* x, const vae2_act* xd, const float* dy,
+                                  const vae2_act* dyd, int k, int stride, int pad) {
+  if (!g_wgrad_multi || !x || !dy || !conv_shapes_ok(xd, dyd, k, stride, pad)) return 0;
+  const WJob j{x, xd, dy, dyd, nullptr, 0, nullptr, k, stride, pad, 0, nullptr, 0,
+               nullptr, nullptr, 0, ""};
+  return k == 3 && wgrad_direct(j) && wgrad3n_shares(xd, dyd) ? 1 : 0;
+}
+
+int vae2_conv2d_bwd_weight_multi(int n, const vae2_wgrad_job* jobs, void* stream) {
+  const char* fn = "vae2_conv2d_bwd_weight_multi";
+  if (n <= 0) return 0;
+  VAE2_REQUIRE(jobs, fn, "null pointer");
+  std::vector<WJob> js((size_t)n);
+  for (int i = 0; i < n; ++i) {
+    const vae2_wgrad_job& q = jobs[i];
+    const bool bn = q.bn_save != nullptr;
+    js[i] = WJob{q.x, &q.xd, q.dy, &q.dyd, q.dw, q.dw_ld, q.dbias, q.k, q.stride, q.pad,
+                 q.accumulate, q.ws, q.ws_size, stream, q.bn_save, q.relu,
+                 bn ? "vae2_conv2d_bwd_weight_bnin" : "vae2_conv2d_bwd_weight"};
+    const int rc = wgrad_check(js[i]);
+    if (rc) return rc;
+  }
+  std::vector<int> share;
+  if (g_wgrad_multi)
+    for (int i = 0; i < n; ++i)
+      if (js[i].k == 3 && wgrad_direct(js[i]) && wgrad3n_shares(js[i].xd, js[i].dyd))
+        share.push_back(i);
+  for (size_t a = 0; a < share.size(); ++a)
+    for (size_t b = a + 1; b < share.size(); ++b) {
+      const WJob &A = js[share[a]], &B = js[share[b]];
+      if (A.ws < B.ws + B.ws_size && B.ws < A.ws + A.ws_size) share.clear();
+    }
+  if (share.size() < 2) share.clear();
+  std::vector<int> splits((size_t)n, -1);
+  for (size_t a = 0; a < share.size(); a += kWgnMaxJobs) {
+    const int m = (int)std::min<size_t>(kWgnMaxJobs, share.size() - a);
+    if (m < 2) break;
+    WgnJob w[kWgnMaxJobs];
+    int sp[kWgnMaxJobs];
+    for (int u = 0; u < m; ++u) {
+      const WJob& j = js[share[a + u]];
+      w[u] = WgnJob{j.x, j.xd, j.dy, j.dyd, j.ws, j.isave, j.irelu, act_bytes(j.xd),
+                    act_bytes(j.dyd)};
+    }
+    if (wgrad3n_launch_multi(m, w, sp, as_stream(stream)) < 0) {
+      const int rc = check_launch(fn);
+      return rc ? rc : fail(fn, "launch failed");
+    }
+    for (int u = 0; u < m; ++u) splits[share[a + u]] = sp[u];
+  }
+  for (int i = 0; i < n; ++i) {
+    int rc = splits[i] < 0 ? wgrad_main(js[i], &splits[i]) : 0;
+    if (!rc) rc = wgrad_tail(js[i], splits[i]);
     if (rc) return rc;
   }
   return 0;
diff --git a/vae-2_amd/csrc/wgrad_narrow.hip b/vae-2_amd/csrc/wgrad_narrow.hip
--- a/vae-2_amd/csrc/wgrad_narrow.hip
+++ b/vae-2_amd/csrc/wgrad_narrow.hip
@@ -23,8 +23,20 @@
   int irelu;
 };
 
-template <int CQ, int TM, int NR, int WPIX, bool PF, int NW = 4>
-__global__ __launch_bounds__(64 * NW) void wgrad3n_kernel(WGN p) {
+template <bool LEAN>
+__device__ __forceinline__ int cold(int v) {
+  if constexpr (LEAN) asm volatile("" : "+v"(v));
+  return v;
+}
+
+template <bool LEAN, typename T>
+__device__ __forceinline__ void hold(T& v) {
+  if constexpr (LEAN) asm volatile("" : "+v"(v));
+}
+
+template <int CQ, int TM, int NR, int WPIX, bool PF, int NW>
+__device__ __forceinline__ void wgrad3n_body(const WGN& p, const int bx, const int by) {
+  constexpr bool LEAN = CQ == 9 && NW == 8;
   constexpr int CSW = 4 * CQ;
   constexpr int CO = 16 * TM + NR;
   constexpr int COQ = (CO + 3) / 4;
@@ -42,22 +54,22 @@
   float* xs = sm;
   float* ds = sm + (kTH + 2) * RS;
 
-  const int lane = threadIdx.x & 63, wave = threadIdx.x >> 6;
+  const int lane = threadIdx.x & 63;
+  const int wave = LEAN ? __builtin_amdgcn_readfirstlane((int)(threadIdx.x >> 6))
+                        : (int)(threadIdx.x >> 6);
   const int g = lane >> 4, r = lane & 15;
   const int wc = wave % WCOL, wp = wave / WCOL;
-  const int cis = blockIdx.y % p.n_ci_slabs, cos = blockIdx.y / p.n_ci_slabs;
+  const int cis = by % p.n_ci_slabs, cos = by / p.n_ci_slabs;
   const int c0 = cis * CSW, co0 = cos * CO;
   const __amdgpu_buffer_rsrc_t xr = make_rsrc(p.x, p.x_bytes);
   const __amdgpu_buffer_rsrc_t dr = make_rsrc(p.dy, p.dy_bytes);
 
   int xoff[GW];
-  bool colok[GW];
 #pragma unroll
   for (int j = 0; j < GW; ++j) {
     const int n = (wc * GW + j) * 16 + r;
     const int nc = n < 3 * CSW ? n : 3 * CSW - 1;
     const int dh = nc / CSW, ci = nc - dh * CSW;
-    colok[j] = wc * GW + j < G && n < 3 * CSW && c0 + ci < p.cin;
     xoff[j] = dh * RS + ci;
   }
   __shared__ f4 ibn_tab[2][CQ];
@@ -91,7 +103,7 @@
       for (int q = 0; q < NR; ++q) racc[j][d][q] = 0.f;
 
   const int per_img = p.tiles_h * p.tiles_w;
-  const int tb = blockIdx.x * p.tps;
+  const int tb = bx * p.tps;
   const int te = tb + p.tps < p.ntiles ? tb + p.tps : p.ntiles;
   constexpr int XPU = NT / CQ, DPU = NT / COQ;
   constexpr int NXI = (LPX + XPU - 1) / XPU, NDI = (kNPX + DPU - 1) / DPU;
@@ -103,6 +115,7 @@
   const bool dcok = co0 + 4 * dq < p.cout;
   f4 px[NXI], pd[NDI];
   uint32_t xin = 0;
+  int xbt = xb, dbt = db;
   auto fetch = [&](int tile) {
     const int img = (int)p.per_img_div.div((uint32_t)tile);
     const int trem = tile - img * per_img;
@@ -111,7 +124,7 @@
     const int ibase = img * p.h;
 #pragma unroll
     for (int u = 0; u < NXI; ++u) {
-      const int hp = xb + u * XPU;
+      const int hp = xbt + u * XPU;
       const int lr = hp / kLW, lc = hp - lr * kLW;
       const int ih = oh0 - 1 + lr, iw = ow0 - 1 + lc;
       const bool ok = xact && hp < LPX && xcok && (unsigned)ih < (unsigned)p.h &&
@@ -121,7 +134,7 @@
     }
 #pragma unroll
     for (int u = 0; u < NDI; ++u) {
-      const int pp = db + u * DPU;
+      const int pp = dbt + u * DPU;
       const int oh = oh0 + pp / kTW, ow = ow0 + (pp & (kTW - 1));
       const bool ok = dact && pp < kNPX && dcok && oh < p.h && ow < p.w;
       pd[u] = load4(dr, ok ? (uint32_t)(((ibase + oh) * p.w + ow) * p.dy_ps + co0 + 4 * dq) * 4u : kOOB);
@@ -130,7 +143,7 @@
   auto store = [&]() {
 #pragma unroll
     for (int u = 0; u < NXI; ++u) {
-      const int hp = xb + u * XPU;
+      const int hp = xbt + u * XPU;
       if (!xact || hp >= LPX) break;
       f4 v = px[u];
       if (p.isave && ((xin >> u) & 1u)) ibn(v, xq);
@@ -141,7 +154,7 @@
     }
 #pragma unroll
     for (int u = 0; u < NDI; ++u) {
-      const int pp = db + u * DPU;
+      const int pp = dbt + u * DPU;
       if (!dact || pp >= kNPX) break;
       f4 v = pd[u];
 #pragma unroll
@@ -153,6 +166,8 @@
   if (PF && tb < te) fetch(tb);
   for (int tile = tb; tile < te; ++tile) {
     __syncthreads();
+    xbt = cold<LEAN>(xb);
+    dbt = cold<LEAN>(db);
     if (!PF) fetch(tile);
     store();
     __syncthreads();
@@ -167,7 +182,7 @@
 #pragma unroll
         for (int s = 0; s < 4; ++s) a[i][s] = ds[(dpx + s) * DP + 16 * i + r];
       f4 rq[4];
-      if constexpr (NR > 0) {
+      if constexpr (NR > 0 && !LEAN) {
 #pragma unroll
         for (int s = 0; s < 4; ++s) rq[s] = *reinterpret_cast<const f4*>(&ds[(dpx + s) * DP + 16 * TM]);
       }
@@ -184,11 +199,22 @@
 #pragma unroll
             for (int i = 0; i < TM; ++i)
               acc[i][j][d] = __builtin_amdgcn_mfma_f32_16x16x4f32(a[i][s], xv[d + s], acc[i][j][d], 0, 0, 0);
-          if constexpr (NR > 0) {
+          if constexpr (NR > 0 && !LEAN) {
 #pragma unroll
             for (int q = 0; q < NR; ++q)
 #pragma unroll
               for (int s = 0; s < 4; ++s) racc[j][d][q] = __builtin_fmaf(rq[s][q], xv[d + s], racc[j][d][q]);
+          }
+        }
+        if constexpr (NR > 0 && LEAN) {
+          const int dpo = cold<LEAN>(dpx);
+#pragma unroll
+          for (int s = 0; s < 4; ++s) {
+            const f4 rs = *reinterpret_cast<const f4*>(&ds[(dpo + s) * DP + 16 * TM]);
+#pragma unroll
+            for (int d = 0; d < 3; ++d)
+#pragma unroll
+              for (int q = 0; q < NR; ++q) racc[j][d][q] = __builtin_fmaf(rs[q], xv[d + s], racc[j][d][q]);
           }
         }
       }
@@ -206,44 +232,51 @@
         v += __shfl_xor(v, 32, 64);
         racc[j][d][q] = v;
       }
+  const int lane_e = LEAN ? (int)__lane_id() : lane;
+  const int g_e = lane_e >> 4, r_e = lane_e & 15;
+  const int wc_e = wc, wp_e = wp;
   const int ncol4 = 9 * p.cin4;
   const uint32_t slab = (uint32_t)(p.cout * ncol4);
-  const __amdgpu_buffer_rsrc_t orr = make_rsrc(p.part + (int64_t)blockIdx.x * slab, slab * 4u);
-  int colb[GW];
-#pragma unroll
-  for (int j = 0; j < GW; ++j) {
-    const int n = (wc * GW + j) * 16 + r;
-    const int dh = n / CSW, ci = n - dh * CSW;
-    colb[j] = colok[j] ? dh * 3 * p.cin4 + c0 + ci : -1;
-  }
-  auto write = [&](int j, int d, int i, int e, float v) {
-    const int co = co0 + 16 * i + 4 * g + e;
-    const bool ok = colb[j] >= 0 && co < p.cout;
-    store1(orr, ok ? (uint32_t)(co * ncol4 + colb[j] + d * p.cin4) * 4u : kOOB, v);
-  };
-  auto write_r = [&](int j, int d, int q, float v) {
-    const int co = co0 + 16 * TM + q;
-    const bool ok = g == 0 && colb[j] >= 0 && co < p.cout;
-    store1(orr, ok ? (uint32_t)(co * ncol4 + colb[j] + d * p.cin4) * 4u : kOOB, v);
+  const __amdgpu_buffer_rsrc_t orr = make_rsrc(p.part + (int64_t)bx * slab, slab * 4u);
+  auto write_all = [&]() {
+    int colb[GW];
+#pragma unroll
+    for (int j = 0; j < GW; ++j) {
+      const int n = (wc_e * GW + j) * 16 + r_e;
+      const int dh = n / CSW, ci = n - dh * CSW;
+      const bool colok = wc_e * GW + j < G && n < 3 * CSW && c0 + ci < p.cin;
+      colb[j] = colok ? dh * 3 * p.cin4 + c0 + ci : -1;
+    }
+#pragma unroll
+    for (int j = 0; j < GW; ++j)
+#pragma unroll
+      for (int d = 0; d < 3; ++d) {
+#pragma unroll
+        for (int i = 0; i < TM; ++i)
+#pragma unroll
+          for (int e = 0; e < 4; ++e) {
+            const int co = co0 + 16 * i + 4 * g_e + e;
+            const bool ok = colb[j] >= 0 && co < p.cout;
+            store1(orr, ok ? (uint32_t)(co * ncol4 + colb[j] + d * p.cin4) * 4u : kOOB,
+                   acc[i][j][d][e]);
+          }
+#pragma unroll
+        for (int q = 0; q < NR; ++q) {
+          const int co = co0 + 16 * TM + q;
+          const bool ok = g_e == 0 && colb[j] >= 0 && co < p.cout;
+          store1(orr, ok ? (uint32_t)(co * ncol4 + colb[j] + d * p.cin4) * 4u : kOOB,
+                 racc[j][d][q]);
+        }
+      }
   };
   if constexpr (WPIX == 1) {
-#pragma unroll
-    for (int j = 0; j < GW; ++j)
-#pragma unroll
-      for (int d = 0; d < 3; ++d) {
-#pragma unroll
-        for (int i = 0; i < TM; ++i)
-#pragma unroll
-          for (int e = 0; e < 4; ++e) write(j, d, i, e, acc[i][j][d][e]);
-#pragma unroll
-        for (int q = 0; q < NR; ++q) write_r(j, d, q, racc[j][d][q]);
-      }
+    write_all();
   } else {
     constexpr int NV = TM * GW * 3 * 4 + GW * 3 * NR;
     __syncthreads();
     float* red = sm;
-    if (wp > 0) {
-      float* o = red + ((wp - 1) * WCOL + wc) * NV * 64 + lane;
+    if (wp_e > 0) {
+      float* o = red + ((wp_e - 1) * WCOL + wc_e) * NV * 64 + lane_e;
       int k = 0;
 #pragma unroll
       for (int i = 0; i < TM; ++i)
@@ -264,36 +297,73 @@
     if (wp == 0) {
 #pragma unroll 1
       for (int w = 1; w < WPIX; ++w) {
-        const float* o = red + ((w - 1) * WCOL + wc) * NV * 64 + lane;
+        const float* o = red + ((w - 1) * WCOL + wc_e) * NV * 64 + lane_e;
         int k = 0;
 #pragma unroll
         for (int i = 0; i < TM; ++i)
 #pragma unroll
-          for (int j = 0; j < GW; ++j)
-#pragma unroll
-            for (int d = 0; d < 3; ++d)
+          for (int j = 0; j < GW; ++j) {
+#pragma unroll
+            for (int d = 0; d < 3; ++d) {
 #pragma unroll
               for (int e = 0; e < 4; ++e) acc[i][j][d][e] += o[64 * k++];
-#pragma unroll
-        for (int j = 0; j < GW; ++j)
+              hold<LEAN>(acc[i][j][d]);
+            }
+            if constexpr (LEAN) __builtin_amdgcn_sched_barrier(0);
+          }
+#pragma unroll
+        for (int j = 0; j < GW; ++j) {
 #pragma unroll
           for (int d = 0; d < 3; ++d)
 #pragma unroll
-            for (int q = 0; q < NR; ++q) racc[j][d][q] += o[64 * k++];
+            for (int q = 0; q < NR; ++q) {
+              racc[j][d][q] += o[64 * k++];
+              hold<LEAN>(racc[j][d][q]);
+            }
+          if constexpr (LEAN) __builtin_amdgcn_sched_barrier(0);
+        }
       }
-#pragma unroll
-      for (int j = 0; j < GW; ++j)
-#pragma unroll
-        for (int d = 0; d < 3; ++d) {
-#pragma unroll
-          for (int i = 0; i < TM; ++i)
-#pragma unroll
-            for (int e = 0; e < 4; ++e) write(j, d, i, e, acc[i][j][d][e]);
-#pragma unroll
-          for (int q = 0; q < NR; ++q) write_r(j, d, q, racc[j][d][q]);
-        }
-    }
-  }
+      write_all();
+    }
+  }
+}
+
+template <int CQ, int TM, int NR, int WPIX, bool PF, int NW = 4>
+__global__ __launch_bounds__(64 * NW, (CQ == 9 && NW == 8) ? 4 : 1) void wgrad3n_kernel(WGN p) {
+  wgrad3n_body<CQ, TM, NR, WPIX, PF, NW>(p, (int)blockIdx.x, (int)blockIdx.y);
+}
+
+struct WGNMulti {
+  WGN j[kWgnMaxJobs];
+  int nblk[kWgnMaxJobs], splits[kWgnMaxJobs];
+  int n;
+};
+
+template <int CQ, int TM, int NR, int WPIX, int NW>
+__global__ __launch_bounds__(64 * NW, (CQ == 9 && NW == 8) ? 4 : 1) void wgrad3n_multi_kernel(
+    WGNMulti m) {
+  int b = (int)blockIdx.x, r0 = 0, job = -1, local = 0;
+  while (job < 0) {
+    int active = 0, next = 0x7fffffff;
+    for (int i = 0; i < m.n; ++i)
+      if (m.nblk[i] > r0) {
+        ++active;
+        next = m.nblk[i] < next ? m.nblk[i] : next;
+      }
+    if (active == 0) return;
+    const int span = (next - r0) * active;
+    if (b < span) {
+      local = r0 + b / active;
+      int k = b % active;
+      for (int i = 0; i < m.n; ++i)
+        if (m.nblk[i] > r0 && k-- == 0) job = i;
+    } else {
+      b -= span;
+      r0 = next;
+    }
+  }
+  const int sp = m.splits[job];
+  wgrad3n_body<CQ, TM, NR, WPIX, false, NW>(m.j[job], local % sp, local / sp);
 }
 
 namespace {
@@ -379,11 +449,9 @@
   return plan(xd, dyd, pl) ? pl.splits : 0;
 }
 
-int wgrad3n_launch(const float* x, const vae2_act* xd, const float* dy, const vae2_act* dyd,
-                   float* part, const float* isave, int irelu, uint32_t x_bytes,
-                   uint32_t dy_bytes, hipStream_t s) {
-  Plan pl;
-  if (!plan(xd, dyd, pl)) return 0;
+static WGN wgn_of(const Plan& pl, const float* x, const vae2_act* xd, const float* dy,
+                  const vae2_act* dyd, float* part, const float* isave, int irelu,
+                  uint32_t x_bytes, uint32_t dy_bytes) {
   WGN p{};
   p.x = x; p.x_ps = (int)xd->ps; p.cin = (int)xd->c; p.cin4 = (int)((xd->c + 3) / 4 * 4);
   p.h = (int)xd->h; p.w = (int)xd->w;
@@ -395,6 +463,15 @@
   p.x_bytes = x_bytes; p.dy_bytes = dy_bytes;
   p.part = part;
   p.isave = isave; p.irelu = irelu ? 1 : 0;
+  return p;
+}
+
+int wgrad3n_launch(const float* x, const vae2_act* xd, const float* dy, const vae2_act* dyd,
+                   float* part, const float* isave, int irelu, uint32_t x_bytes,
+                   uint32_t dy_bytes, hipStream_t s) {
+  Plan pl;
+  if (!plan(xd, dyd, pl)) return 0;
+  const WGN p = wgn_of(pl, x, xd, dy, dyd, part, isave, irelu, x_bytes, dy_bytes);
   dim3 grid((unsigned)pl.splits, (unsigned)(pl.c.ci_slabs * pl.c.co_slabs));
   const size_t shm = lds_bytes(pl.c);
   if (pl.c.cq == 5) {
@@ -410,4 +487,30 @@
   return e == hipSuccess ? pl.splits : -(int)e;
 }
 
-}
+bool wgrad3n_shares(const vae2_act* xd, const vae2_act* dyd) {
+  Plan pl;
+  return plan(xd, dyd, pl) && pl.c.cq == 9 && pl.c.nw == 8;
+}
+
+int wgrad3n_launch_multi(int n, const WgnJob* jobs, int* splits, hipStream_t s) {
+  WGNMulti m{};
+  Cfg c{};
+  int blocks = 0;
+  for (int i = 0; i < n; ++i) {
+    const WgnJob& j = jobs[i];
+    Plan pl;
+    if (n > kWgnMaxJobs || !plan(j.xd, j.dyd, pl) || pl.c.cq != 9 || pl.c.nw != 8) return -1;
+    m.j[i] = wgn_of(pl, j.x, j.xd, j.dy, j.dyd, j.part, j.isave, j.irelu, j.x_bytes, j.dy_bytes);
+    m.splits[i] = splits[i] = pl.splits;
+    m.nblk[i] = pl.splits * pl.c.ci_slabs * pl.c.co_slabs;
+    blocks += m.nblk[i];
+    c = pl.c;
+  }
+  m.n = n;
+  VAE2_LAUNCH((wgrad3n_multi_kernel<9, 2, 4, 2, 8>), dim3((unsigned)blocks), dim3(512),
+              lds_bytes(c), s, m);
+  const hipError_t e = hipGetLastError();
+  return e == hipSuccess ? 0 : -(int)e;
+}
+
+}
diff --git a/vae-2_amd/vae2/_lib.py b/vae-2_amd/vae2/_lib.py
--- a/vae-2_amd/vae2/_lib.py
+++ b/vae-2_amd/vae2/_lib.py
@@ -189,6 +189,9 @@
     "vae2_weighted_avgpool_bwd": (c_int, [c_vp, P_ACT, c_vp, c_vp, c_f32, c_vp, P_ACT, c_f32,
                                           c_vp]),
     "vae2_conv2d_set_grouping": (c_int, [c_int]),
+    "vae2_conv2d_bwd_weight_multi": (c_int, [c_int, c_vp, c_vp]),
+    "vae2_wgrad_set_multi": (c_int, [c_int]),
+    "vae2_conv2d_bwd_weight_shares": (c_int, [c_vp, P_ACT, c_vp, P_ACT, c_int, c_int, c_int]),
 }
 
 ABI_VERSION = 15
@@ -231,6 +234,14 @@
                 ("y", c_vp), ("yd", Act), ("beta", c_f32), ("stats", c_vp)]
 
 
+class WgradJob(ctypes.Structure):
+    _fields_ = [("x", c_vp), ("xd", Act), ("dy", c_vp), ("dyd", Act), ("dw", c_vp),
+                ("dw_ld", c_i64), ("dbias", c_vp), ("k", ctypes.c_int32),
+                ("stride", ctypes.c_int32), ("pad", ctypes.c_int32),
+                ("accumulate", ctypes.c_int32), ("ws", c_vp), ("ws_size", c_i64),
+                ("bn_save", c_vp), ("relu", ctypes.c_int32), ("pad_", ctypes.c_int32)]
+
+
 class HipError(RuntimeError):
     pass
 
diff --git a/vae-2_amd/vae2/ops.py b/vae-2_amd/vae2/ops.py
--- a/vae-2_amd/vae2/ops.py
+++ b/vae-2_amd/vae2/ops.py
@@ -451,18 +451,46 @@
         return False
 
 
+class WgradGroup:
+
+    def __init__(self):
+        self.jobs, self.notes, self.single = [], [], []
+
+    def add(self, job, single):
+        self.jobs.append(job)
+        self.single.append(single)
+        self.notes.append(prof.take())
+
+    def flush(self):
+        if not self.jobs:
+            return
+        if len(self.jobs) < 2:
+            prof.put(self.notes[0])
+            self.single[0]()
+            self.jobs, self.notes, self.single = [], [], []
+            return
+        notes = [w for w in self.notes if w is not None]
+        if notes:
+            prof.note(sum(w[0] for w in notes), sum(w[1] for w in notes),
+                      " + ".join(str(w[2]) for w in notes))
+        arr = (_lib.WgradJob * len(self.jobs))(*self.jobs)
+        call("vae2_conv2d_bwd_weight_multi", len(self.jobs), arr, stream_ptr())
+        self.jobs, self.notes, self.single = [], [], []
+
+
 def _conv_bwd(x, weight, bias, dy, spec, need_dx, need_w=True, need_b=True, group=None,
-              sp=None, hold=None):
+              sp=None, hold=None, wgrad=None):
     s = stream_ptr() if sp is None else sp
     xv, dyv = act_of(x), act_of(dy)
-    wret, bret, ws = _conv_wgrad(x, xv, weight, bias, dy, dyv, spec, need_w, need_b, s=s,
-                                 lane=sp is not None, hold=hold)
+    wret, bret, ws = wgrad if wgrad is not None else _conv_wgrad(
+        x, xv, weight, bias, dy, dyv, spec, need_w, need_b, s=s, lane=sp is not None, hold=hold)
     if not need_dx or getattr(x, "_vae2_no_dx", False):
         return None, wret, bret
     return _conv_dgrad(x, xv, weight, dy, dyv, spec, group=group, s=s, hold=hold), wret, bret
 
 
-def _conv_wgrad(x, xv, weight, bias, dy, dyv, spec, need_w, need_b, *, s, lane, hold):
+def _conv_wgrad(x, xv, weight, bias, dy, dyv, spec, need_w, need_b, *, s, lane, hold,
+                queue=None):
     (xp, xa), (dyp, dya) = xv, dyv
     wsink, wret = _grad_sink(weight, need_w)
     bsink, bret = _grad_sink(bias, need_b)
@@ -479,7 +507,8 @@
     now = wret is not None or tmp_w or lane
     if lane and hold is not None:
         hold.append(ws)
-    with _defer_off(now and _WGRAD_BATCH[0] > 0):
+
+    def single():
         if lz is not None:
             call("vae2_conv2d_bwd_weight_bnin", xp, ctypes.byref(xa), ptr(lz.save),
                  int(lz.relu), dyp, ctypes.byref(dya), ptr(wsink), ptr(bsink), spec.k,
@@ -487,6 +516,19 @@
         else:
             call("vae2_conv2d_bwd_weight", xp, ctypes.byref(xa), dyp, ctypes.byref(dya),
                  ptr(wsink), ptr(bsink), spec.k, spec.stride, spec.pad, 1, ptr(ws), size, s)
+
+    if (queue is not None and _WGRAD_BATCH[0] and not now and
+            _lib.load().vae2_conv2d_bwd_weight_shares(xp, ctypes.byref(xa), dyp, ctypes.byref(dya),
+                                                      spec.k, spec.stride, spec.pad)):
+        cin_kk = xa.c * spec.k * spec.k
+        queue.add(_lib.WgradJob(xp, xa, dyp, dya, ptr(wsink), cin_kk, ptr(bsink), spec.k,
+                                spec.stride, spec.pad, 1, ptr(ws), size,
+                                ptr(lz.save) if lz is not None else None,
+                                int(lz.relu) if lz is not None else 0, 0), single)
+        _WS_HOLD.append((torch.cuda.current_stream().cuda_stream, ws))
+        return wret, bret, ws
+    with _defer_off(now and _WGRAD_BATCH[0] > 0):
+        single()
     if _WGRAD_BATCH[0] and not now:
         _WS_HOLD.append((torch.cuda.current_stream().cuda_stream, ws))
     return wret, bret, ws
@@ -892,13 +934,22 @@
         lanes.sync()
 
     with wgrad_batch():
+        wgrads = [None] * len(layers)
+        if not lanes.on:
+            wq, s = WgradGroup(), stream_ptr()
+            for i, L in enumerate(layers):
+                need = _layer_needs(ctx.needs_input_grad, i)
+                wgrads[i] = _conv_wgrad(L.x, act_of(L.x), L.weight, L.bias, L.dr, act_of(L.dr),
+                                        L.spec, need.weight, need.bias, s=s, lane=False,
+                                        hold=hold, queue=wq)
+            wq.flush()
         for i, L in enumerate(layers):
             need, dres = _layer_needs(ctx.needs_input_grad, i), L.dres
             if dres is not None and L.spec.res_link is not None:
                 dres = L.spec.res_link.hand_over(dres, settle)
             dx, wret, bret_conv = _conv_bwd(L.x, L.weight, L.bias, L.dr, L.spec, need.x,
                                             need.weight, need.bias, group=cg, sp=lanes.ptr(i),
-                                            hold=hold)
+                                            hold=hold, wgrad=wgrads[i])
             grads.append(_In(dx, wret, bret_conv, L.gret, L.bret, dres))
         if cg is not None:
             cg.flush()
```

Result: no change. 925.1 frames/s, median of 6 (+0.4%).
